# quadram-institute-bioscience/uvaia

Hardware: AMD Instinct MI355X
Metric: ref-seqs scored/sec (higher is better)
Workload: dtype u32 bit-planes / int32 counts

## Files before the change

include/uvaia_gpu.h:

```cpp
#ifndef UVAIA_GPU_H
#define UVAIA_GPU_H

#include <stddef.h>
#include <stdint.h>

#ifdef __cplusplus
extern "C" {
#endif

#define UVAIA_GPU_NSCORE 6

enum {
  UVAIA_GPU_OK         =  0,
  UVAIA_GPU_EINVAL     = -1,
  UVAIA_GPU_ENODEV     = -2,
  UVAIA_GPU_ENOMEM     = -3,
  UVAIA_GPU_EHIP       = -4,
  UVAIA_GPU_EALPHABET  = -5,
  UVAIA_GPU_ESTATE     = -6
};

typedef struct uvaia_gpu_ctx uvaia_gpu_ctx;

typedef struct {
  int n_query;
  int nchar;
  const char *const *seq;
  const char *consensus;
  const size_t *idx_c, *idx_m, *idx;
  int n_idx_c, n_idx_m, n_idx;
  size_t trim;
  int acgt;
} uvaia_gpu_query;

int uvaia_gpu_open (uvaia_gpu_ctx **ctx, const uvaia_gpu_query *query, int heap_size, int device, size_t max_pool);

enum { UVAIA_GPU_SCAN_AUTO = 0,
       UVAIA_GPU_SCAN_PACKED = 1,
       UVAIA_GPU_SCAN_COMPRESSED = 2,
       UVAIA_GPU_SCAN_WIDE = 3 };
typedef struct {
  size_t subslice_refs;
  int rare_max;
  int scan;
  int serial;
  int scan_tiles_per_wave;
  int scan_waves_per_block;
  int rederive_streams;
  int ball_gather;
  int query_tables;
  int replay_extras;
  int replay_cus;
  int scan_streams;
  int pipeline;
  int head_scan;
  int derive_waves;
} uvaia_gpu_tuning;
int uvaia_gpu_export_query_table (uvaia_gpu_ctx *ctx, int which, void *out, size_t cap, size_t *n_bytes);
int uvaia_gpu_open_tuned (uvaia_gpu_ctx **ctx, const uvaia_gpu_query *query, int heap_size, int device, size_t max_pool, const uvaia_gpu_tuning *tuning );
void uvaia_gpu_close (uvaia_gpu_ctx *ctx);
const char *uvaia_gpu_last_error (const uvaia_gpu_ctx *ctx);

int uvaia_gpu_push (uvaia_gpu_ctx *ctx, const char *const *seq, const int *non_n, int n_ref, int64_t ordinal0,
                    uint8_t *entered);

int uvaia_gpu_drain (uvaia_gpu_ctx *ctx, int *n_items, int *max_incompatible, int *scores, int64_t *ordinals);
int uvaia_gpu_heap_slots (const uvaia_gpu_ctx *ctx);
int uvaia_gpu_n_query (const uvaia_gpu_ctx *ctx);
int uvaia_gpu_reset (uvaia_gpu_ctx *ctx);

int uvaia_gpu_db_reserve (uvaia_gpu_ctx *ctx, size_t n_ref_capacity);
int uvaia_gpu_db_append (uvaia_gpu_ctx *ctx, const char *const *seq, const int *non_n, int n_ref);
int uvaia_gpu_db_append_block (uvaia_gpu_ctx *ctx, const char *rows, size_t pitch, const int *non_n, int n_ref);
size_t uvaia_gpu_db_size (const uvaia_gpu_ctx *ctx);
int uvaia_gpu_search_resident (uvaia_gpu_ctx *ctx, size_t pool, int64_t ordinal0, uint8_t *entered);
int uvaia_gpu_sync (uvaia_gpu_ctx *ctx);

size_t uvaia_gpu_state_bytes (const uvaia_gpu_ctx *ctx);
int uvaia_gpu_state_export (uvaia_gpu_ctx *ctx, void *dst);
int uvaia_gpu_state_import (uvaia_gpu_ctx *ctx, const void *src);
int uvaia_gpu_slice_scan (uvaia_gpu_ctx *ctx, size_t first, size_t n, int buf);
int uvaia_gpu_slice_replay (uvaia_gpu_ctx *ctx, int buf, int64_t ordinal0, int stripe_start);
int uvaia_gpu_slice_buffers (void);
size_t uvaia_gpu_state_range_bytes (const uvaia_gpu_ctx *ctx, int q0, int q1);
int uvaia_gpu_state_export_range (uvaia_gpu_ctx *ctx, void *dst, int q0, int q1);
int uvaia_gpu_state_import_range (uvaia_gpu_ctx *ctx, const void *src, int q0, int q1);
int uvaia_gpu_slice_replay_range (uvaia_gpu_ctx *ctx, int buf, int64_t ordinal0, int q0, int q1, int take_snapshot);
int uvaia_gpu_entered_flags (uvaia_gpu_ctx *ctx, uint8_t *out, int clear);

int uvaia_gpu_ball (uvaia_gpu_ctx *ctx, const char *const *seq, int n_ref, int radius, int *mindist);
int uvaia_gpu_ball_resident (uvaia_gpu_ctx *ctx, size_t first, size_t n, int radius, int *mindist);
int uvaia_gpu_ball_packed (uvaia_gpu_ctx *ctx, const void *planes, int n_ref, int radius, int *mindist);
int uvaia_gpu_unpack_rows (uvaia_gpu_ctx *ctx, const int *index, int n, char *rows, size_t pitch);
unsigned long long uvaia_gpu_ball_asked (uvaia_gpu_ctx *ctx, int reset);
void uvaia_gpu_ball_kernel_ms (uvaia_gpu_ctx *ctx, double out[3], int reset);

int uvaia_gpu_agree_on_polymorphic (uvaia_gpu_ctx *ctx, const char *const *seq, int n_seq, uint8_t *out);

int uvaia_gpu_query_columns (const char *const *seq, int n_query, int nchar, size_t trim, int acgt, int device, char *consensus, unsigned char *some_missing);

int uvaia_gpu_last_batch_scores (uvaia_gpu_ctx *ctx, int *out, int n_ref);
int uvaia_gpu_scan_stats (uvaia_gpu_ctx *ctx, double *ms, long long *launches, double *algorithmic_bytes, int reset);
int uvaia_gpu_replay_stats (uvaia_gpu_ctx *ctx, unsigned long long out[3], int reset);
int uvaia_gpu_replay_tiles_opened (uvaia_gpu_ctx *ctx, unsigned long long *out, int reset);
int uvaia_gpu_replay_timing (uvaia_gpu_ctx *ctx, unsigned long long out[12], int reset);
int uvaia_gpu_set_query_tile (uvaia_gpu_ctx *ctx, int qt);
int uvaia_gpu_set_active_queries (uvaia_gpu_ctx *ctx, int q0, int q1);
int uvaia_gpu_max_tolerance (uvaia_gpu_ctx *ctx, int *out);
int uvaia_gpu_search_resident_pool (uvaia_gpu_ctx *ctx, size_t first, size_t n, int64_t ordinal0, int snapshot);

int uvaia_gpu_db_set_shard (uvaia_gpu_ctx *ctx, int rank, int world, size_t piece_refs);
int uvaia_gpu_shard_rows (const uvaia_gpu_ctx *ctx);
size_t uvaia_gpu_shard_aux_bytes (const uvaia_gpu_ctx *ctx, size_t n_tiles);
int uvaia_gpu_shard_scan (uvaia_gpu_ctx *ctx, size_t first, size_t n, void *cnt, void *tmin, void *aux);
int uvaia_gpu_db_skip (uvaia_gpu_ctx *ctx, size_t n_ref);
int uvaia_gpu_shard_set_peer (uvaia_gpu_ctx *ctx, int rank, const void *planes, const void *side_rows);
const void *uvaia_gpu_shard_planes (const uvaia_gpu_ctx *ctx);
const void *uvaia_gpu_shard_side_rows (const uvaia_gpu_ctx *ctx);
int uvaia_gpu_shard_ipc_handle_bytes (void);
int uvaia_gpu_shard_ipc_handles (uvaia_gpu_ctx *ctx, void *out );
int uvaia_gpu_shard_ipc_open (uvaia_gpu_ctx *ctx, int rank, const void *handles);
int uvaia_gpu_shard_ipc_close (uvaia_gpu_ctx *ctx);
int uvaia_gpu_scan_wait (uvaia_gpu_ctx *ctx);
int uvaia_gpu_replay_wait (uvaia_gpu_ctx *ctx);
int uvaia_gpu_set_snapshot (uvaia_gpu_ctx *ctx, int snapshot);
enum { UVAIA_GPU_SCANS = 0, UVAIA_GPU_REPLAYS = 1 };
int uvaia_gpu_mark (uvaia_gpu_ctx *ctx, int what, int slot);
int uvaia_gpu_stream_wait_mark (uvaia_gpu_ctx *ctx, void *stream, int slot);
int uvaia_gpu_wait_stream (uvaia_gpu_ctx *ctx, int what, void *stream);
int uvaia_gpu_shard_replay (uvaia_gpu_ctx *ctx, const void *cnt, const void *tmin, const void *aux, int owner, size_t first, size_t n, int64_t ordinal0, int q0, int q1);

typedef struct uvaia_gpu_group uvaia_gpu_group;
int  uvaia_gpu_group_open (uvaia_gpu_group **group, const uvaia_gpu_query *query, int heap_size, const int *devices, int n_devices, size_t max_pool, size_t piece_refs);
void uvaia_gpu_group_close (uvaia_gpu_group *group);
const char *uvaia_gpu_group_last_error (const uvaia_gpu_group *group);
int  uvaia_gpu_group_size (const uvaia_gpu_group *group);
uvaia_gpu_ctx *uvaia_gpu_group_member (uvaia_gpu_group *group, int i);
int  uvaia_gpu_group_query_shard (const uvaia_gpu_group *group, int i, int *q0, int *q1);
int  uvaia_gpu_group_db_reserve (uvaia_gpu_group *group, size_t n_ref_capacity);
int  uvaia_gpu_group_db_append (uvaia_gpu_group *group, const char *const *seq, const int *non_n, int n_ref);
int  uvaia_gpu_group_db_append_packed (uvaia_gpu_group *group, const void *planes, const int *non_n, const int *side_rows, int n_ref);
int  uvaia_gpu_group_db_clear (uvaia_gpu_group *group);
int  uvaia_gpu_group_db_rederive (uvaia_gpu_group *group);
size_t uvaia_gpu_group_db_size (const uvaia_gpu_group *group);
int  uvaia_gpu_group_reset (uvaia_gpu_group *group);
int  uvaia_gpu_group_search_resident (uvaia_gpu_group *group, size_t pool, int64_t ordinal0, uint8_t *entered);
int  uvaia_gpu_group_push (uvaia_gpu_group *group, const char *const *seq, const int *non_n, int n_ref, int64_t ordinal0, uint8_t *entered);
int  uvaia_gpu_group_drain (uvaia_gpu_group *group, int *n_items, int *max_incompatible, int *scores, int64_t *ordinals);
int  uvaia_gpu_group_sync (uvaia_gpu_group *group);

size_t uvaia_gpu_db_tile_bytes (const uvaia_gpu_ctx *ctx);
int    uvaia_gpu_db_clear (uvaia_gpu_ctx *ctx);
int    uvaia_gpu_db_rederive (uvaia_gpu_ctx *ctx);
int    uvaia_gpu_db_derived_export (uvaia_gpu_ctx *ctx, size_t n_tiles, void *e, uint32_t *grp, void *poly, int *tot);
int    uvaia_gpu_db_side_row_ints (void);
int    uvaia_gpu_db_export (uvaia_gpu_ctx *ctx, size_t first_tile, size_t n_tiles, void *planes, int *non_n, int *side_rows);
int    uvaia_gpu_db_append_packed (uvaia_gpu_ctx *ctx, const void *planes, const int *non_n, const int *side_rows, int n_ref);

int uvaia_gpu_db_stage_reserve (uvaia_gpu_ctx *ctx, size_t n_tiles);
int uvaia_gpu_db_stage_packed (uvaia_gpu_ctx *ctx, int slot, const void *planes, const int *non_n, const int *side_rows, int n_tiles);
int uvaia_gpu_db_load_staged (uvaia_gpu_ctx *ctx, int slot, const int *sel, int n_ref);
int uvaia_gpu_db_stage_packed_at (uvaia_gpu_ctx *ctx, int slot, size_t tile_offset, const void *planes, const int *non_n, const int *side_rows, int n_tiles);
int uvaia_gpu_db_append_staged (uvaia_gpu_ctx *ctx, int slot, const int *sel, int n_ref);
int uvaia_gpu_db_stage_compact_at (uvaia_gpu_ctx *ctx, int slot, size_t tile_offset, const void *base, const uint64_t *head_idx, const uint32_t *heads,
                                   const uint64_t *lit_idx, const void *lits, const int *non_n, int n_tiles);
void uvaia_gpu_compact_ms (uvaia_gpu_ctx *ctx, double out[2], int reset);
int uvaia_gpu_db_unpack_rows (uvaia_gpu_ctx *ctx, const int *index, int n, char *rows, size_t pitch);
void uvaia_gpu_window_ms (uvaia_gpu_ctx *ctx, double out[3], int reset);
size_t uvaia_gpu_free_bytes (uvaia_gpu_ctx *ctx);

int uvaia_gpu_rows_census (uvaia_gpu_ctx *ctx, const void *d_rows, size_t pitch, int n, int *non_n, int *n_exc);
int uvaia_gpu_db_append_device (uvaia_gpu_ctx *ctx, const void *d_rows, size_t pitch, const int *row_index, int n_sel, const int *non_n);
int uvaia_gpu_rows_exceptions (uvaia_gpu_ctx *ctx, const void *d_rows, size_t pitch, const int *row_index, int n_sel, const uint64_t *offsets, void *exc_out);
int uvaia_gpu_db_drop_tiles (uvaia_gpu_ctx *ctx, size_t n_tiles);
void uvaia_gpu_rows_kernel_ms (uvaia_gpu_ctx *ctx, double out[3], int reset);
int uvaia_gpu_rows_set_run_cut (uvaia_gpu_ctx *ctx, unsigned cut);

size_t uvaia_gpu_scan_bytes_per_ref (const uvaia_gpu_ctx *ctx);
int uvaia_gpu_scan_variant (const uvaia_gpu_ctx *ctx);
size_t uvaia_gpu_derived_bytes_per_ref (const uvaia_gpu_ctx *ctx);
size_t uvaia_gpu_packed_bytes_per_ref (const uvaia_gpu_ctx *ctx);

#ifdef __cplusplus
}
#endif
#endif
```

uvaia_amd/capi.py:

```python
import ctypes as C
import os
import subprocess

import numpy as np

_HERE = os.path.dirname(os.path.abspath(__file__))
ROOT = os.path.dirname(_HERE)
_LIB = os.path.join(_HERE, "lib", "libuvaia_gpu.so")
NSCORE = 6

SYMBOLS = [
    "uvaia_gpu_open", "uvaia_gpu_open_tuned", "uvaia_gpu_close", "uvaia_gpu_last_error", "uvaia_gpu_push", "uvaia_gpu_drain",
    "uvaia_gpu_heap_slots", "uvaia_gpu_n_query", "uvaia_gpu_reset", "uvaia_gpu_db_reserve", "uvaia_gpu_db_append",
    "uvaia_gpu_db_append_block", "uvaia_gpu_db_size", "uvaia_gpu_search_resident", "uvaia_gpu_sync", "uvaia_gpu_ball", "uvaia_gpu_ball_resident", "uvaia_gpu_ball_packed", "uvaia_gpu_unpack_rows", "uvaia_gpu_ball_asked", "uvaia_gpu_ball_kernel_ms", "uvaia_gpu_export_query_table", "uvaia_gpu_agree_on_polymorphic", "uvaia_gpu_query_columns",
    "uvaia_gpu_last_batch_scores", "uvaia_gpu_scan_stats", "uvaia_gpu_replay_stats", "uvaia_gpu_replay_tiles_opened", "uvaia_gpu_replay_timing",
    "uvaia_gpu_state_bytes", "uvaia_gpu_state_export", "uvaia_gpu_state_import", "uvaia_gpu_slice_scan", "uvaia_gpu_slice_replay",
    "uvaia_gpu_entered_flags", "uvaia_gpu_state_range_bytes", "uvaia_gpu_state_export_range", "uvaia_gpu_state_import_range",
    "uvaia_gpu_slice_replay_range", "uvaia_gpu_slice_buffers", "uvaia_gpu_scan_bytes_per_ref", "uvaia_gpu_derived_bytes_per_ref", "uvaia_gpu_scan_variant", "uvaia_gpu_set_query_tile", "uvaia_gpu_packed_bytes_per_ref",
    "uvaia_gpu_db_tile_bytes", "uvaia_gpu_db_side_row_ints", "uvaia_gpu_db_export", "uvaia_gpu_db_append_packed", "uvaia_gpu_db_clear", "uvaia_gpu_db_rederive", "uvaia_gpu_db_derived_export",
    "uvaia_gpu_set_active_queries", "uvaia_gpu_max_tolerance", "uvaia_gpu_search_resident_pool",
    "uvaia_gpu_db_set_shard", "uvaia_gpu_shard_rows", "uvaia_gpu_shard_scan", "uvaia_gpu_scan_wait", "uvaia_gpu_replay_wait", "uvaia_gpu_set_snapshot", "uvaia_gpu_shard_replay",
    "uvaia_gpu_mark", "uvaia_gpu_stream_wait_mark", "uvaia_gpu_wait_stream",
    "uvaia_gpu_shard_aux_bytes", "uvaia_gpu_db_skip", "uvaia_gpu_shard_set_peer", "uvaia_gpu_shard_planes", "uvaia_gpu_shard_side_rows",
    "uvaia_gpu_shard_ipc_handle_bytes", "uvaia_gpu_shard_ipc_handles", "uvaia_gpu_shard_ipc_open", "uvaia_gpu_shard_ipc_close",
    "uvaia_gpu_group_open", "uvaia_gpu_group_close", "uvaia_gpu_group_last_error", "uvaia_gpu_group_size", "uvaia_gpu_group_member", "uvaia_gpu_group_query_shard",
    "uvaia_gpu_group_db_reserve", "uvaia_gpu_group_db_append", "uvaia_gpu_group_db_append_packed", "uvaia_gpu_group_db_clear", "uvaia_gpu_group_db_rederive",
    "uvaia_gpu_group_db_size", "uvaia_gpu_group_reset", "uvaia_gpu_group_search_resident", "uvaia_gpu_group_push", "uvaia_gpu_group_drain", "uvaia_gpu_group_sync",
    "uvaia_gpu_rows_census", "uvaia_gpu_db_append_device", "uvaia_gpu_rows_exceptions", "uvaia_gpu_db_drop_tiles", "uvaia_gpu_rows_kernel_ms", "uvaia_gpu_rows_set_run_cut",
    "uvaia_gpu_db_stage_reserve", "uvaia_gpu_db_stage_packed", "uvaia_gpu_db_load_staged", "uvaia_gpu_db_unpack_rows", "uvaia_gpu_window_ms", "uvaia_gpu_free_bytes",
    "uvaia_gpu_db_stage_packed_at", "uvaia_gpu_db_append_staged", "uvaia_gpu_db_stage_compact_at", "uvaia_gpu_compact_ms",
]


class GpuError(RuntimeError):
    def __init__(self, code, msg):
        super().__init__("uvaia_gpu error %d: %s" % (code, msg))
        self.code = code


class Tuning(C.Structure):
    _fields_ = [("subslice_refs", C.c_size_t), ("rare_max", C.c_int), ("scan", C.c_int), ("serial", C.c_int),
                ("scan_tiles_per_wave", C.c_int), ("scan_waves_per_block", C.c_int), ("rederive_streams", C.c_int), ("ball_gather", C.c_int), ("query_tables", C.c_int), ("replay_extras", C.c_int), ("replay_cus", C.c_int), ("scan_streams", C.c_int), ("pipeline", C.c_int), ("head_scan", C.c_int), ("derive_waves", C.c_int)]

    SCAN = {"auto": 0, "packed": 1, "compressed": 2, "wide": 3}

    @classmethod
    def make(cls, tuning):
        if tuning is None or isinstance(tuning, cls):
            return tuning
        t = cls()
        for k, v in tuning.items():
            setattr(t, k, cls.SCAN[v] if k == "scan" and isinstance(v, str) else int(v))
        return t


class _Query(C.Structure):
    _fields_ = [
        ("n_query", C.c_int), ("nchar", C.c_int),
        ("seq", C.POINTER(C.c_char_p)), ("consensus", C.c_char_p),
        ("idx_c", C.POINTER(C.c_size_t)), ("idx_m", C.POINTER(C.c_size_t)), ("idx", C.POINTER(C.c_size_t)),
        ("n_idx_c", C.c_int), ("n_idx_m", C.c_int), ("n_idx", C.c_int),
        ("trim", C.c_size_t), ("acgt", C.c_int),
    ]


def library_path():
    return _LIB


def build_library(force=False):
    csrc = os.path.join(_HERE, "csrc")
    srcs = [os.path.join(csrc, f) for f in os.listdir(csrc) if f.endswith((".hip", ".inc"))] + [os.path.join(ROOT, "include", "uvaia_gpu.h")]
    if not force and os.path.exists(_LIB) and os.path.getmtime(_LIB) >= max(os.path.getmtime(f) for f in srcs):
        return _LIB
    subprocess.check_call(["make", "-C", os.path.join(_HERE, "csrc"), "-s"])
    return _LIB


_lib = None


def load_library():
    global _lib
    if _lib is not None:
        return _lib
    if not os.path.exists(_LIB):
        raise GpuError(-2, "HIP library %s is missing: run __graft_entry__.build() (no CPU fallback exists)" % _LIB)
    L = C.CDLL(_LIB)
    vp = C.c_void_p
    pp = C.POINTER(C.c_char_p)
    pi = C.POINTER(C.c_int)
    sig = {
        "uvaia_gpu_open": (C.c_int, [C.POINTER(vp), C.POINTER(_Query), C.c_int, C.c_int, C.c_size_t]),
        "uvaia_gpu_open_tuned": (C.c_int, [C.POINTER(vp), C.POINTER(_Query), C.c_int, C.c_int, C.c_size_t, C.POINTER(Tuning)]),
        "uvaia_gpu_close": (None, [vp]),
        "uvaia_gpu_last_error": (C.c_char_p, [vp]),
        "uvaia_gpu_push": (C.c_int, [vp, pp, pi, C.c_int, C.c_int64, C.POINTER(C.c_uint8)]),
        "uvaia_gpu_drain": (C.c_int, [vp, pi, pi, pi, C.POINTER(C.c_int64)]),
        "uvaia_gpu_heap_slots": (C.c_int, [vp]),
        "uvaia_gpu_n_query": (C.c_int, [vp]),
        "uvaia_gpu_reset": (C.c_int, [vp]),
        "uvaia_gpu_db_reserve": (C.c_int, [vp, C.c_size_t]),
        "uvaia_gpu_db_append": (C.c_int, [vp, pp, pi, C.c_int]),
        "uvaia_gpu_db_append_block": (C.c_int, [vp, C.c_void_p, C.c_size_t, pi, C.c_int]),
        "uvaia_gpu_db_size": (C.c_size_t, [vp]),
        "uvaia_gpu_search_resident": (C.c_int, [vp, C.c_size_t, C.c_int64, C.POINTER(C.c_uint8)]),
        "uvaia_gpu_sync": (C.c_int, [vp]),
        "uvaia_gpu_ball": (C.c_int, [vp, pp, C.c_int, C.c_int, pi]),
        "uvaia_gpu_ball_resident": (C.c_int, [vp, C.c_size_t, C.c_size_t, C.c_int, pi]),
        "uvaia_gpu_ball_packed": (C.c_int, [vp, C.c_void_p, C.c_int, C.c_int, pi]),
        "uvaia_gpu_unpack_rows": (C.c_int, [vp, pi, C.c_int, C.c_void_p, C.c_size_t]),
        "uvaia_gpu_ball_asked": (C.c_ulonglong, [vp, C.c_int]),
        "uvaia_gpu_ball_kernel_ms": (None, [vp, C.POINTER(C.c_double), C.c_int]),
        "uvaia_gpu_export_query_table": (C.c_int, [vp, C.c_int, vp, C.c_size_t, C.POINTER(C.c_size_t)]),
        "uvaia_gpu_agree_on_polymorphic": (C.c_int, [vp, pp, C.c_int, C.POINTER(C.c_uint8)]),
        "uvaia_gpu_query_columns": (C.c_int, [pp, C.c_int, C.c_int, C.c_size_t, C.c_int, C.c_int, C.c_char_p, C.POINTER(C.c_uint8)]),
        "uvaia_gpu_last_batch_scores": (C.c_int, [vp, pi, C.c_int]),
        "uvaia_gpu_scan_stats": (C.c_int, [vp, C.POINTER(C.c_double), C.POINTER(C.c_longlong), C.POINTER(C.c_double), C.c_int]),
        "uvaia_gpu_replay_stats": (C.c_int, [vp, C.POINTER(C.c_ulonglong), C.c_int]),
        "uvaia_gpu_replay_tiles_opened": (C.c_int, [vp, C.POINTER(C.c_ulonglong), C.c_int]),
        "uvaia_gpu_replay_timing": (C.c_int, [vp, C.POINTER(C.c_ulonglong), C.c_int]),
        "uvaia_gpu_state_bytes": (C.c_size_t, [vp]),
        "uvaia_gpu_state_export": (C.c_int, [vp, C.c_void_p]),
        "uvaia_gpu_state_import": (C.c_int, [vp, C.c_void_p]),
        "uvaia_gpu_slice_scan": (C.c_int, [vp, C.c_size_t, C.c_size_t, C.c_int]),
        "uvaia_gpu_slice_replay": (C.c_int, [vp, C.c_int, C.c_int64, C.c_int]),
        "uvaia_gpu_entered_flags": (C.c_int, [vp, C.POINTER(C.c_uint8), C.c_int]),
        "uvaia_gpu_state_range_bytes": (C.c_size_t, [vp, C.c_int, C.c_int]),
        "uvaia_gpu_state_export_range": (C.c_int, [vp, C.c_void_p, C.c_int, C.c_int]),
        "uvaia_gpu_state_import_range": (C.c_int, [vp, C.c_void_p, C.c_int, C.c_int]),
        "uvaia_gpu_slice_replay_range": (C.c_int, [vp, C.c_int, C.c_int64, C.c_int, C.c_int, C.c_int]),
        "uvaia_gpu_slice_buffers": (C.c_int, []),
        "uvaia_gpu_scan_bytes_per_ref": (C.c_size_t, [vp]),
        "uvaia_gpu_derived_bytes_per_ref": (C.c_size_t, [vp]),
        "uvaia_gpu_scan_variant": (C.c_int, [vp]),
        "uvaia_gpu_set_query_tile": (C.c_int, [vp, C.c_int]),
        "uvaia_gpu_packed_bytes_per_ref": (C.c_size_t, [vp]),
        "uvaia_gpu_set_active_queries": (C.c_int, [vp, C.c_int, C.c_int]),
        "uvaia_gpu_max_tolerance": (C.c_int, [vp, pi]),
        "uvaia_gpu_search_resident_pool": (C.c_int, [vp, C.c_size_t, C.c_size_t, C.c_int64, C.c_int]),
        "uvaia_gpu_db_tile_bytes": (C.c_size_t, [vp]),
        "uvaia_gpu_db_clear": (C.c_int, [vp]),
        "uvaia_gpu_db_rederive": (C.c_int, [vp]),
        "uvaia_gpu_db_derived_export": (C.c_int, [vp, C.c_size_t, C.c_void_p, C.c_void_p, C.c_void_p, C.c_void_p]),
        "uvaia_gpu_db_side_row_ints": (C.c_int, []),
        "uvaia_gpu_db_export": (C.c_int, [vp, C.c_size_t, C.c_size_t, C.c_void_p, pi, pi]),
        "uvaia_gpu_db_append_packed": (C.c_int, [vp, C.c_void_p, pi, pi, C.c_int]),
        "uvaia_gpu_db_set_shard": (C.c_int, [vp, C.c_int, C.c_int, C.c_size_t]),
        "uvaia_gpu_shard_rows": (C.c_int, [vp]),
        "uvaia_gpu_shard_scan": (C.c_int, [vp, C.c_size_t, C.c_size_t, C.c_void_p, C.c_void_p, C.c_void_p]),
        "uvaia_gpu_shard_aux_bytes": (C.c_size_t, [vp, C.c_size_t]), "uvaia_gpu_db_skip": (C.c_int, [vp, C.c_size_t]),
        "uvaia_gpu_shard_set_peer": (C.c_int, [vp, C.c_int, C.c_void_p, C.c_void_p]),
        "uvaia_gpu_shard_planes": (C.c_void_p, [vp]), "uvaia_gpu_shard_side_rows": (C.c_void_p, [vp]),
        "uvaia_gpu_shard_ipc_handle_bytes": (C.c_int, []), "uvaia_gpu_shard_ipc_handles": (C.c_int, [vp, C.c_void_p]),
        "uvaia_gpu_shard_ipc_open": (C.c_int, [vp, C.c_int, C.c_void_p]), "uvaia_gpu_shard_ipc_close": (C.c_int, [vp]),
        "uvaia_gpu_scan_wait": (C.c_int, [vp]),
        "uvaia_gpu_replay_wait": (C.c_int, [vp]),
        "uvaia_gpu_set_snapshot": (C.c_int, [vp, C.c_int]),
        "uvaia_gpu_shard_replay": (C.c_int, [vp, C.c_void_p, C.c_void_p, C.c_void_p, C.c_int, C.c_size_t, C.c_size_t, C.c_int64, C.c_int, C.c_int]),
        "uvaia_gpu_mark": (C.c_int, [vp, C.c_int, C.c_int]), "uvaia_gpu_stream_wait_mark": (C.c_int, [vp, C.c_void_p, C.c_int]),
        "uvaia_gpu_wait_stream": (C.c_int, [vp, C.c_int, C.c_void_p]),
        "uvaia_gpu_group_open": (C.c_int, [C.POINTER(vp), C.POINTER(_Query), C.c_int, pi, C.c_int, C.c_size_t, C.c_size_t]),
        "uvaia_gpu_group_close": (None, [vp]),
        "uvaia_gpu_group_last_error": (C.c_char_p, [vp]),
        "uvaia_gpu_group_size": (C.c_int, [vp]),
        "uvaia_gpu_group_member": (vp, [vp, C.c_int]),
        "uvaia_gpu_group_query_shard": (C.c_int, [vp, C.c_int, pi, pi]),
        "uvaia_gpu_group_db_reserve": (C.c_int, [vp, C.c_size_t]),
        "uvaia_gpu_group_db_append": (C.c_int, [vp, pp, pi, C.c_int]),
        "uvaia_gpu_group_db_append_packed": (C.c_int, [vp, C.c_void_p, pi, pi, C.c_int]),
        "uvaia_gpu_group_db_clear": (C.c_int, [vp]),
        "uvaia_gpu_group_db_rederive": (C.c_int, [vp]),
        "uvaia_gpu_group_db_size": (C.c_size_t, [vp]),
        "uvaia_gpu_group_reset": (C.c_int, [vp]),
        "uvaia_gpu_group_search_resident": (C.c_int, [vp, C.c_size_t, C.c_int64, C.POINTER(C.c_uint8)]),
        "uvaia_gpu_group_push": (C.c_int, [vp, pp, pi, C.c_int, C.c_int64, C.POINTER(C.c_uint8)]),
        "uvaia_gpu_group_drain": (C.c_int, [vp, pi, pi, pi, C.POINTER(C.c_int64)]),
        "uvaia_gpu_group_sync": (C.c_int, [vp]),
        "uvaia_gpu_rows_census": (C.c_int, [vp, C.c_void_p, C.c_size_t, C.c_int, pi, pi]),
        "uvaia_gpu_db_append_device": (C.c_int, [vp, C.c_void_p, C.c_size_t, pi, C.c_int, pi]),
        "uvaia_gpu_rows_exceptions": (C.c_int, [vp, C.c_void_p, C.c_size_t, pi, C.c_int, C.POINTER(C.c_uint64), C.c_void_p]),
        "uvaia_gpu_db_drop_tiles": (C.c_int, [vp, C.c_size_t]),
        "uvaia_gpu_rows_kernel_ms": (None, [vp, C.POINTER(C.c_double), C.c_int]),
        "uvaia_gpu_rows_set_run_cut": (C.c_int, [vp, C.c_uint]),
        "uvaia_gpu_db_stage_reserve": (C.c_int, [vp, C.c_size_t]),
        "uvaia_gpu_db_stage_packed": (C.c_int, [vp, C.c_int, C.c_void_p, pi, pi, C.c_int]),
        "uvaia_gpu_db_load_staged": (C.c_int, [vp, C.c_int, pi, C.c_int]),
        "uvaia_gpu_db_stage_packed_at": (C.c_int, [vp, C.c_int, C.c_size_t, C.c_void_p, pi, pi, C.c_int]),
        "uvaia_gpu_db_append_staged": (C.c_int, [vp, C.c_int, pi, C.c_int]),
        "uvaia_gpu_db_stage_compact_at": (C.c_int, [vp, C.c_int, C.c_size_t, C.c_void_p, C.c_void_p, C.c_void_p, C.c_void_p, C.c_void_p, pi, C.c_int]),
        "uvaia_gpu_compact_ms": (None, [vp, C.POINTER(C.c_double), C.c_int]),
        "uvaia_gpu_db_unpack_rows": (C.c_int, [vp, pi, C.c_int, C.c_void_p, C.c_size_t]),
        "uvaia_gpu_window_ms": (None, [vp, C.POINTER(C.c_double), C.c_int]),
        "uvaia_gpu_free_bytes": (C.c_size_t, [vp]),
    }
    for name, (res, args) in sig.items():
        fn = getattr(L, name)
        fn.restype, fn.argtypes = res, args
    _lib = L
    return L


def _cstrs(strs):
    arr = (C.c_char_p * len(strs))()
    for i, s in enumerate(strs):
        arr[i] = s
    return arr


def _int_ptr(a):
    if a is None:
        return None, None
    arr = np.ascontiguousarray(a, dtype=np.int32)
    return arr, arr.ctypes.data_as(C.POINTER(C.c_int))


class Engine:

    def __init__(self, seqs, consensus, idx_c, idx_m, idx, trim=0, acgt=False, nbest=100, max_pool=4096, device=-1, tuning=None):
        self.L = load_library()
        self.nq, self.nchar = len(seqs), len(consensus)
        self._keep = [_cstrs(seqs), consensus,
                      (C.c_size_t * len(idx_c))(*[int(x) for x in idx_c]),
                      (C.c_size_t * len(idx_m))(*[int(x) for x in idx_m]),
                      (C.c_size_t * len(idx))(*[int(x) for x in idx])]
        q = _Query(self.nq, self.nchar, self._keep[0], consensus, self._keep[2], self._keep[3], self._keep[4],
                   len(idx_c), len(idx_m), len(idx), int(trim), int(bool(acgt)))
        self.ctx = C.c_void_p()
        tn = Tuning.make(tuning)
        rc = self.L.uvaia_gpu_open_tuned(C.byref(self.ctx), C.byref(q), int(nbest), int(device), int(max_pool), C.byref(tn) if tn is not None else None)
        if rc != 0:
            msg = self.L.uvaia_gpu_last_error(None)
            self.ctx = None
            raise GpuError(rc, msg.decode() if msg else "?")
        self.slots = self.L.uvaia_gpu_heap_slots(self.ctx)
        self.ordinal = 0

    @classmethod
    def from_query(cls, q, **kw):
        return cls(q.seqs, q.consensus, q.idx_c, q.idx_m, q.idx, trim=q.trim, acgt=q.acgt, **kw)

    def _chk(self, rc):
        if rc != 0:
            msg = self.L.uvaia_gpu_last_error(self.ctx)
            raise GpuError(rc, msg.decode() if msg else "?")

    def close(self):
        if getattr(self, "ctx", None):
            self.L.uvaia_gpu_close(self.ctx)
            self.ctx = None

    def __del__(self):
        try:
            self.close()
        except Exception:
            pass

    def __enter__(self):
        return self

    def __exit__(self, *a):
        self.close()

    def push(self, refs, non_n=None, ordinal0=None):
        n = len(refs)
        if ordinal0 is None:
            ordinal0 = self.ordinal
        self.ordinal = ordinal0 + n
        entered = np.zeros(n, dtype=np.uint8)
        if n == 0:
            return entered
        _k, nn = _int_ptr(non_n)
        self._chk(self.L.uvaia_gpu_push(self.ctx, _cstrs(refs), nn, n, ordinal0, entered.ctypes.data_as(C.POINTER(C.c_uint8))))
        return entered

    def last_batch_scores(self, n):
        out = np.zeros((n, self.nq, NSCORE), dtype=np.int32)
        self._chk(self.L.uvaia_gpu_last_batch_scores(self.ctx, out.ctypes.data_as(C.POINTER(C.c_int)), n))
        return out

    def drain(self):
        n = np.zeros(self.nq, dtype=np.int32)
        T = np.zeros(self.nq, dtype=np.int32)
        sc = np.zeros((self.nq, self.slots + 1, NSCORE), dtype=np.int32)
        od = np.zeros((self.nq, self.slots + 1), dtype=np.int64)
        pi = C.POINTER(C.c_int)
        self._chk(self.L.uvaia_gpu_drain(self.ctx, n.ctypes.data_as(pi), T.ctypes.data_as(pi), sc.ctypes.data_as(pi),
                                         od.ctypes.data_as(C.POINTER(C.c_int64))))
        return n, T, sc, od

    def reset(self):
        self.ordinal = 0
        self._chk(self.L.uvaia_gpu_reset(self.ctx))

    def db_reserve(self, n):
        self._chk(self.L.uvaia_gpu_db_reserve(self.ctx, int(n)))

    def db_append(self, refs, non_n=None):
        _k, nn = _int_ptr(non_n)
        self._chk(self.L.uvaia_gpu_db_append(self.ctx, _cstrs(refs), nn, len(refs)))

    def db_append_block(self, block, non_n=None):
        block = np.ascontiguousarray(block, dtype=np.uint8)
        _k, nn = _int_ptr(non_n)
        self._chk(self.L.uvaia_gpu_db_append_block(self.ctx, block.ctypes.data, block.shape[1], nn, block.shape[0]))

    def db_size(self):
        return self.L.uvaia_gpu_db_size(self.ctx)

    @staticmethod
    def _device_block(rows, pitch=None, n=None):
        if hasattr(rows, "data_ptr"):
            import torch
            if rows.dtype != torch.uint8 or rows.dim() != 2 or not rows.is_cuda or (rows.shape[0] > 0 and rows.shape[1] > 1 and rows.stride(1) != 1):
                raise GpuError(-1, "rows must be a 2-d torch.uint8 tensor in device memory with contiguous rows")
            torch.cuda.current_stream(rows.device).synchronize()
            return rows.data_ptr(), (rows.stride(0) if rows.shape[0] > 1 else rows.shape[1]), rows.shape[0], rows
        if pitch is None:
            raise GpuError(-1, "a raw device pointer needs its pitch")
        return int(rows), int(pitch), n, None

    def rows_census(self, rows, pitch=None, n=None):
        ptr, pitch, n, _keep = self._device_block(rows, pitch, n)
        non_n, n_exc = np.zeros(n, dtype=np.int32), np.zeros(n, dtype=np.int32)
        self._chk(self.L.uvaia_gpu_rows_census(self.ctx, ptr, pitch, n, non_n.ctypes.data_as(C.POINTER(C.c_int)), n_exc.ctypes.data_as(C.POINTER(C.c_int))))
        return non_n, n_exc

    def db_append_device(self, rows, row_index=None, non_n=None, pitch=None, n=None):
        ptr, pitch, n, _keep = self._device_block(rows, pitch, n)
        _k1, ri = _int_ptr(row_index)
        _k2, nn = _int_ptr(non_n)
        self._chk(self.L.uvaia_gpu_db_append_device(self.ctx, ptr, pitch, ri, n if row_index is None else len(row_index), nn))

    def rows_exceptions(self, rows, n_exc, row_index=None, pitch=None, n=None):
        ptr, pitch, n, _keep = self._device_block(rows, pitch, n)
        n_sel = n if row_index is None else len(row_index)
        off = np.zeros(n_sel + 1, dtype=np.uint64)
        off[1:] = np.cumsum(np.asarray(n_exc, dtype=np.uint64))
        out = np.zeros((int(off[-1]), 2), dtype=np.uint32)
        _k1, ri = _int_ptr(row_index)
        self._chk(self.L.uvaia_gpu_rows_exceptions(self.ctx, ptr, pitch, ri, n_sel, off.ctypes.data_as(C.POINTER(C.c_uint64)), out.ctypes.data))
        return off, out

    def db_drop_tiles(self, n_tiles):
        self._chk(self.L.uvaia_gpu_db_drop_tiles(self.ctx, int(n_tiles)))

    def rows_kernel_ms(self, reset=False):
        out = (C.c_double * 3)()
        self.L.uvaia_gpu_rows_kernel_ms(self.ctx, out, int(reset))
        return {"census": out[0], "gather": out[1], "exceptions": out[2]}

    def rows_set_run_cut(self, cut):
        self._chk(self.L.uvaia_gpu_rows_set_run_cut(self.ctx, int(cut)))

    def set_active_queries(self, q0, q1):
        self._chk(self.L.uvaia_gpu_set_active_queries(self.ctx, int(q0), int(q1)))

    def max_tolerance(self):
        v = C.c_int(0)
        self._chk(self.L.uvaia_gpu_max_tolerance(self.ctx, C.byref(v)))
        return v.value

    def search_resident_pool(self, first, n, ordinal0, snapshot=-1):
        self._chk(self.L.uvaia_gpu_search_resident_pool(self.ctx, int(first), int(n), int(ordinal0), int(snapshot)))

    def db_clear(self):
        self._chk(self.L.uvaia_gpu_db_clear(self.ctx))

    def db_set_shard(self, rank, world, piece_refs):
        self._chk(self.L.uvaia_gpu_db_set_shard(self.ctx, int(rank), int(world), int(piece_refs)))

    def shard_rows(self):
        return self.L.uvaia_gpu_shard_rows(self.ctx)

    def shard_scan(self, first, n, cnt_ptr, tmin_ptr, aux_ptr):
        self._chk(self.L.uvaia_gpu_shard_scan(self.ctx, int(first), int(n), C.c_void_p(cnt_ptr), C.c_void_p(tmin_ptr), C.c_void_p(aux_ptr)))

    def shard_aux_bytes(self, n_tiles):
        return int(self.L.uvaia_gpu_shard_aux_bytes(self.ctx, int(n_tiles)))

    def db_skip(self, n_ref):
        self._chk(self.L.uvaia_gpu_db_skip(self.ctx, int(n_ref)))

    def shard_ipc_handles(self):
        buf = C.create_string_buffer(self.L.uvaia_gpu_shard_ipc_handle_bytes())
        self._chk(self.L.uvaia_gpu_shard_ipc_handles(self.ctx, buf))
        return buf.raw

    def shard_ipc_close(self):
        self._chk(self.L.uvaia_gpu_shard_ipc_close(self.ctx))

    def shard_ipc_open(self, rank, handles):
        self._chk(self.L.uvaia_gpu_shard_ipc_open(self.ctx, int(rank), C.c_char_p(bytes(handles))))

    def scan_wait(self):
        self._chk(self.L.uvaia_gpu_scan_wait(self.ctx))

    def replay_wait(self):
        self._chk(self.L.uvaia_gpu_replay_wait(self.ctx))

    def set_snapshot(self, v):
        self._chk(self.L.uvaia_gpu_set_snapshot(self.ctx, int(v)))

    SCANS, REPLAYS = 0, 1

    def mark(self, what, slot):
        self._chk(self.L.uvaia_gpu_mark(self.ctx, int(what), int(slot)))

    def stream_wait_mark(self, stream, slot):
        self._chk(self.L.uvaia_gpu_stream_wait_mark(self.ctx, C.c_void_p(stream), int(slot)))

    def wait_stream(self, what, stream):
        self._chk(self.L.uvaia_gpu_wait_stream(self.ctx, int(what), C.c_void_p(stream)))

    def shard_replay(self, cnt_ptr, tmin_ptr, aux_ptr, owner, first, n, ordinal0, q0, q1):
        self._chk(self.L.uvaia_gpu_shard_replay(self.ctx, C.c_void_p(cnt_ptr), C.c_void_p(tmin_ptr), C.c_void_p(aux_ptr), int(owner), int(first), int(n), int(ordinal0), int(q0), int(q1)))

    def db_rederive(self):
        self._chk(self.L.uvaia_gpu_db_rederive(self.ctx))

    def db_export(self, first_tile=0, n_tiles=None):
        if n_tiles is None:
            n_tiles = (self.db_size() + 63) // 64 - first_tile
        tb, ri = self.L.uvaia_gpu_db_tile_bytes(self.ctx), self.L.uvaia_gpu_db_side_row_ints()
        planes = np.zeros((n_tiles, tb), dtype=np.uint8)
        non_n = np.zeros(n_tiles * 64, dtype=np.int32)
        side = np.zeros((n_tiles * 64, ri), dtype=np.int32)
        self._chk(self.L.uvaia_gpu_db_export(self.ctx, first_tile, n_tiles, planes.ctypes.data, non_n.ctypes.data_as(C.POINTER(C.c_int)),
                                             side.ctypes.data_as(C.POINTER(C.c_int))))
        return planes, non_n, side

    def db_append_packed(self, planes, non_n, side_rows, n_ref):
        planes = np.ascontiguousarray(planes, dtype=np.uint8)
        non_n = np.ascontiguousarray(non_n, dtype=np.int32)
        side_rows = np.ascontiguousarray(side_rows, dtype=np.int32)
        self._chk(self.L.uvaia_gpu_db_append_packed(self.ctx, planes.ctypes.data, non_n.ctypes.data_as(C.POINTER(C.c_int)),
                                                    side_rows.ctypes.data_as(C.POINTER(C.c_int)), int(n_ref)))

    def search_resident(self, pool, ordinal0=0, want_entered=True):
        ent, p = None, None
        if want_entered:
            ent = np.zeros(self.db_size(), dtype=np.uint8)
            p = ent.ctypes.data_as(C.POINTER(C.c_uint8))
        self._chk(self.L.uvaia_gpu_search_resident(self.ctx, int(pool), int(ordinal0), p))
        return ent

    def sync(self):
        self._chk(self.L.uvaia_gpu_sync(self.ctx))

    def scan_stats(self, reset=False):
        ms, n, b = C.c_double(), C.c_longlong(), C.c_double()
        self._chk(self.L.uvaia_gpu_scan_stats(self.ctx, C.byref(ms), C.byref(n), C.byref(b), int(reset)))
        return ms.value, n.value, b.value

    def state_bytes(self):
        return self.L.uvaia_gpu_state_bytes(self.ctx)

    def state_export(self, ptr):
        self._chk(self.L.uvaia_gpu_state_export(self.ctx, C.c_void_p(ptr)))

    def state_import(self, ptr):
        self._chk(self.L.uvaia_gpu_state_import(self.ctx, C.c_void_p(ptr)))

    def slice_scan(self, first, n, buf):
        self._chk(self.L.uvaia_gpu_slice_scan(self.ctx, int(first), int(n), int(buf)))

    def slice_replay(self, buf, ordinal0, stripe_start):
        self._chk(self.L.uvaia_gpu_slice_replay(self.ctx, int(buf), int(ordinal0), int(bool(stripe_start))))

    def state_range_bytes(self, q0, q1):
        return self.L.uvaia_gpu_state_range_bytes(self.ctx, int(q0), int(q1))

    def state_export_range(self, ptr, q0, q1):
        self._chk(self.L.uvaia_gpu_state_export_range(self.ctx, C.c_void_p(ptr), int(q0), int(q1)))

    def state_import_range(self, ptr, q0, q1):
        self._chk(self.L.uvaia_gpu_state_import_range(self.ctx, C.c_void_p(ptr), int(q0), int(q1)))

    def slice_replay_range(self, buf, ordinal0, q0, q1, take_snapshot):
        self._chk(self.L.uvaia_gpu_slice_replay_range(self.ctx, int(buf), int(ordinal0), int(q0), int(q1), int(bool(take_snapshot))))

    def entered_flags(self, clear=False):
        ent = np.zeros(self.db_size(), dtype=np.uint8)
        self._chk(self.L.uvaia_gpu_entered_flags(self.ctx, ent.ctypes.data_as(C.POINTER(C.c_uint8)), int(clear)))
        return ent

    def replay_stats(self, reset=False):
        out = (C.c_ulonglong * 3)()
        self._chk(self.L.uvaia_gpu_replay_stats(self.ctx, out, int(reset)))
        return int(out[0]), int(out[1]), int(out[2])

    def replay_timing(self, reset=False):
        out = (C.c_ulonglong * 12)()
        self._chk(self.L.uvaia_gpu_replay_timing(self.ctx, out, int(reset)))
        return [int(x) for x in out]

    def replay_tiles_opened(self, reset=False):
        out = C.c_ulonglong(0)
        self._chk(self.L.uvaia_gpu_replay_tiles_opened(self.ctx, C.byref(out), int(reset)))
        return int(out.value)

    def set_query_tile(self, qt):
        self._chk(self.L.uvaia_gpu_set_query_tile(self.ctx, int(qt)))

    def scan_bytes_per_ref(self):
        return self.L.uvaia_gpu_scan_bytes_per_ref(self.ctx)

    def derived_bytes_per_ref(self):
        return self.L.uvaia_gpu_derived_bytes_per_ref(self.ctx)

    def scan_variant(self):
        return self.L.uvaia_gpu_scan_variant(self.ctx)

    def packed_bytes_per_ref(self):
        return self.L.uvaia_gpu_packed_bytes_per_ref(self.ctx)

    def agree_on_polymorphic(self, seqs):
        out = np.zeros((len(seqs), self.nq), dtype=np.uint8)
        self._chk(self.L.uvaia_gpu_agree_on_polymorphic(self.ctx, _cstrs(seqs), len(seqs), out.ctypes.data_as(C.POINTER(C.c_uint8))))
        return out

    def ball(self, refs, radius):
        md = np.zeros(len(refs), dtype=np.int32)
        self._chk(self.L.uvaia_gpu_ball(self.ctx, _cstrs(refs), len(refs), int(radius), md.ctypes.data_as(C.POINTER(C.c_int))))
        return md

    def ball_resident(self, radius, first=0, n=None, want=True):
        n = self.db_size() - first if n is None else n
        md = np.zeros(n, dtype=np.int32) if want else None
        self._chk(self.L.uvaia_gpu_ball_resident(self.ctx, int(first), int(n), int(radius), md.ctypes.data_as(C.POINTER(C.c_int)) if want else None))
        return md

    def ball_packed(self, planes, n_ref, radius):
        planes = np.ascontiguousarray(planes, dtype=np.uint8)
        tb = self.L.uvaia_gpu_db_tile_bytes(self.ctx)
        if planes.size < (int(n_ref) + 63) // 64 * tb:
            raise ValueError("%d references need %d bytes of tiles, got %d" % (n_ref, (int(n_ref) + 63) // 64 * tb, planes.size))
        md = np.zeros(int(n_ref), dtype=np.int32)
        self._chk(self.L.uvaia_gpu_ball_packed(self.ctx, planes.ctypes.data, int(n_ref), int(radius), md.ctypes.data_as(C.POINTER(C.c_int))))
        return md

    def unpack_rows(self, index):
        idx = np.ascontiguousarray(index, dtype=np.int32)
        pitch = (self.nchar + 15) // 16 * 16
        rows = np.zeros((max(len(idx), 1), pitch), dtype=np.uint8)
        self._chk(self.L.uvaia_gpu_unpack_rows(self.ctx, idx.ctypes.data_as(C.POINTER(C.c_int)), len(idx), rows.ctypes.data, pitch))
        return [rows[k, :self.nchar].tobytes() for k in range(len(idx))]

    def db_stage_reserve(self, n_tiles):
        self._chk(self.L.uvaia_gpu_db_stage_reserve(self.ctx, int(n_tiles)))

    def db_stage_packed(self, slot, planes, non_n, side_rows, n_tiles):
        planes = np.ascontiguousarray(planes, dtype=np.uint8)
        non_n = np.ascontiguousarray(non_n, dtype=np.int32)
        side_rows = np.ascontiguousarray(side_rows, dtype=np.int32)
        tb = self.L.uvaia_gpu_db_tile_bytes(self.ctx)
        if planes.size < int(n_tiles) * tb or non_n.size < int(n_tiles) * 64 or side_rows.size < int(n_tiles) * 64 * self.L.uvaia_gpu_db_side_row_ints():
            raise ValueError("arrays shorter than %d tiles" % n_tiles)
        if not hasattr(self, "_staged"):
            self._staged = {}
        self._staged[int(slot)] = (planes, non_n, side_rows)
        self._chk(self.L.uvaia_gpu_db_stage_packed(self.ctx, int(slot), planes.ctypes.data, non_n.ctypes.data_as(C.POINTER(C.c_int)),
                                                   side_rows.ctypes.data_as(C.POINTER(C.c_int)), int(n_tiles)))

    def db_load_staged(self, slot, sel, n_ref):
        _k, sp = _int_ptr(sel)
        self._chk(self.L.uvaia_gpu_db_load_staged(self.ctx, int(slot), sp, int(n_ref)))

    def db_stage_packed_at(self, slot, tile_offset, planes, non_n, side_rows, n_tiles):
        planes = np.ascontiguousarray(planes, dtype=np.uint8)
        non_n = np.ascontiguousarray(non_n, dtype=np.int32)
        side_rows = np.ascontiguousarray(side_rows, dtype=np.int32)
        tb = self.L.uvaia_gpu_db_tile_bytes(self.ctx)
        if planes.size < int(n_tiles) * tb or non_n.size < int(n_tiles) * 64 or side_rows.size < int(n_tiles) * 64 * self.L.uvaia_gpu_db_side_row_ints():
            raise ValueError("arrays shorter than %d tiles" % n_tiles)
        if not hasattr(self, "_staged_at"):
            self._staged_at = {}
        if int(tile_offset) == 0:
            self._staged_at[int(slot)] = []
        self._staged_at.setdefault(int(slot), []).append((planes, non_n, side_rows))
        self._chk(self.L.uvaia_gpu_db_stage_packed_at(self.ctx, int(slot), int(tile_offset), planes.ctypes.data, non_n.ctypes.data_as(C.POINTER(C.c_int)),
                                                      side_rows.ctypes.data_as(C.POINTER(C.c_int)), int(n_tiles)))

    def db_stage_compact_at(self, slot, tile_offset, base, head_idx, heads, lit_idx, lits, non_n, n_tiles):
        base = np.ascontiguousarray(base, dtype=np.uint32)
        head_idx = np.ascontiguousarray(head_idx, dtype=np.uint64)
        lit_idx = np.ascontiguousarray(lit_idx, dtype=np.uint64)
        heads = np.ascontiguousarray(heads, dtype=np.uint32)
        lits = np.ascontiguousarray(lits, dtype=np.uint32)
        non_n = np.ascontiguousarray(non_n, dtype=np.int32)
        lanes = int(n_tiles) * 64
        if base.size * 4 * 64 != self.L.uvaia_gpu_db_tile_bytes(self.ctx) or head_idx.size < lanes + 1 or lit_idx.size < lanes + 1 or non_n.size < lanes:
            raise ValueError("arrays shorter than %d tiles" % n_tiles)
        if lanes and (heads.size < int(head_idx[lanes]) or lits.size < int(lit_idx[lanes]) * 4):
            raise ValueError("records shorter than the index says")
        if not hasattr(self, "_staged_at"):
            self._staged_at = {}
        if int(tile_offset) == 0:
            self._staged_at[int(slot)] = []
        self._staged_at.setdefault(int(slot), []).append((base, head_idx, heads, lit_idx, lits, non_n))
        self._chk(self.L.uvaia_gpu_db_stage_compact_at(self.ctx, int(slot), int(tile_offset), base.ctypes.data, head_idx.ctypes.data, heads.ctypes.data,
                                                       lit_idx.ctypes.data, lits.ctypes.data, non_n.ctypes.data_as(C.POINTER(C.c_int)), int(n_tiles)))

    def compact_ms(self, reset=False):
        out = (C.c_double * 2)()
        self.L.uvaia_gpu_compact_ms(self.ctx, out, int(reset))
        return tuple(out)

    def db_append_staged(self, slot, sel, n_ref):
        _k, sp = _int_ptr(sel)
        self._chk(self.L.uvaia_gpu_db_append_staged(self.ctx, int(slot), sp, int(n_ref)))

    def db_unpack_rows(self, index, pitch=None):
        idx = np.ascontiguousarray(index, dtype=np.int32)
        pitch = (self.nchar + 15) // 16 * 16 if pitch is None else int(pitch)
        rows = np.zeros((max(len(idx), 1), pitch), dtype=np.uint8)
        self._chk(self.L.uvaia_gpu_db_unpack_rows(self.ctx, idx.ctypes.data_as(C.POINTER(C.c_int)), len(idx), rows.ctypes.data, pitch))
        return [rows[k, :self.nchar].tobytes() for k in range(len(idx))]

    def window_ms(self, reset=False):
        out = (C.c_double * 3)()
        self.L.uvaia_gpu_window_ms(self.ctx, out, int(reset))
        return tuple(out)

    def free_bytes(self):
        return int(self.L.uvaia_gpu_free_bytes(self.ctx))

    def ball_asked(self, reset=False):
        return int(self.L.uvaia_gpu_ball_asked(self.ctx, int(reset)))

    def query_table(self, which):
        n = C.c_size_t(0)
        self._chk(self.L.uvaia_gpu_export_query_table(self.ctx, int(which), None, 0, C.byref(n)))
        out = np.zeros(n.value, dtype=np.uint8)
        if n.value:
            self._chk(self.L.uvaia_gpu_export_query_table(self.ctx, int(which), out.ctypes.data_as(C.c_void_p), n.value, C.byref(n)))
        return out

    def db_derived(self, n_tiles):
        W4 = ((self.nchar + 31) // 32 + 3) // 4
        counts = self.query_table(10).view(np.int32)
        NG = int(counts[2]) + int(counts[3])
        e = np.zeros((n_tiles, W4, 64, 4), dtype=np.uint32)
        grp = np.zeros((n_tiles, W4, 64), dtype=np.uint32)
        poly = np.zeros((n_tiles, NG, 3, 64, 4), dtype=np.uint32)
        tot = np.zeros(n_tiles * 64, dtype=np.int32)
        self._chk(self.L.uvaia_gpu_db_derived_export(self.ctx, int(n_tiles), e.ctypes.data, grp.ctypes.data, poly.ctypes.data, tot.ctypes.data))
        return e, grp, poly, tot

    def ball_kernel_ms(self, reset=False):
        out = (C.c_double * 3)()
        self.L.uvaia_gpu_ball_kernel_ms(self.ctx, out, int(reset))
        return tuple(out)


def finalise_heaps(n, scores, ordinals):
    out = []
    for q in range(len(n)):
        k = int(n[q])
        order = ([k] + list(range(1, k))) if k else []
        rows = [(tuple(int(x) for x in scores[q, s]), int(ordinals[q, s])) for s in order]
        rows.sort(key=lambda r: tuple(-v for v in r[0]))
        out.append(rows)
    return out


class Group:

    def __init__(self, q, devices, nbest=100, max_pool=4096, piece_refs=0):
        self.L = load_library()
        self.nq, self.nchar = len(q.seqs), len(q.consensus)
        self._keep = [_cstrs(q.seqs), q.consensus,
                      (C.c_size_t * len(q.idx_c))(*[int(x) for x in q.idx_c]),
                      (C.c_size_t * len(q.idx_m))(*[int(x) for x in q.idx_m]),
                      (C.c_size_t * len(q.idx))(*[int(x) for x in q.idx])]
        qq = _Query(self.nq, self.nchar, self._keep[0], q.consensus, self._keep[2], self._keep[3], self._keep[4],
                    len(q.idx_c), len(q.idx_m), len(q.idx), int(q.trim), int(bool(q.acgt)))
        self.g = C.c_void_p()
        dev = (C.c_int * len(devices))(*[int(d) for d in devices])
        rc = self.L.uvaia_gpu_group_open(C.byref(self.g), C.byref(qq), int(nbest), dev, len(devices), int(max_pool), int(piece_refs))
        if rc != 0:
            msg = self.L.uvaia_gpu_group_last_error(None)
            self.g = None
            raise GpuError(rc, msg.decode() if msg else "?")
        self.slots = self.L.uvaia_gpu_heap_slots(self.L.uvaia_gpu_group_member(self.g, 0))

    def _chk(self, rc):
        if rc != 0:
            msg = self.L.uvaia_gpu_group_last_error(self.g)
            raise GpuError(rc, msg.decode() if msg else "?")

    def close(self):
        if getattr(self, "g", None):
            self.L.uvaia_gpu_group_close(self.g)
            self.g = None

    def __enter__(self):
        return self

    def __exit__(self, *a):
        self.close()

    def __del__(self):
        try:
            self.close()
        except Exception:
            pass

    def query_shard(self, i):
        a, b = C.c_int(), C.c_int()
        self._chk(self.L.uvaia_gpu_group_query_shard(self.g, i, C.byref(a), C.byref(b)))
        return a.value, b.value

    def member_bytes_per_ref(self):
        self.L.uvaia_gpu_packed_bytes_per_ref.restype = C.c_size_t
        self.L.uvaia_gpu_derived_bytes_per_ref.restype = C.c_size_t
        m0 = C.c_void_p(self.L.uvaia_gpu_group_member(self.g, 0))
        return int(self.L.uvaia_gpu_packed_bytes_per_ref(m0)), int(self.L.uvaia_gpu_derived_bytes_per_ref(m0))

    def db_reserve(self, n):
        self._chk(self.L.uvaia_gpu_group_db_reserve(self.g, int(n)))

    def db_append(self, refs, non_n=None):
        _k, nn = _int_ptr(non_n)
        self._chk(self.L.uvaia_gpu_group_db_append(self.g, _cstrs(refs), nn, len(refs)))

    def db_rederive(self):
        self._chk(self.L.uvaia_gpu_group_db_rederive(self.g))

    def reset(self):
        self._chk(self.L.uvaia_gpu_group_reset(self.g))

    def sync(self):
        self._chk(self.L.uvaia_gpu_group_sync(self.g))

    def search_resident(self, pool, ordinal0=0, want_entered=True):
        ent, p = None, None
        if want_entered:
            ent = np.zeros(self.L.uvaia_gpu_group_db_size(self.g), dtype=np.uint8)
            p = ent.ctypes.data_as(C.POINTER(C.c_uint8))
        self._chk(self.L.uvaia_gpu_group_search_resident(self.g, int(pool), int(ordinal0), p))
        return ent

    def push(self, refs, non_n=None, ordinal0=0):
        entered = np.zeros(len(refs), dtype=np.uint8)
        _k, nn = _int_ptr(non_n)
        self._chk(self.L.uvaia_gpu_group_push(self.g, _cstrs(refs), nn, len(refs), int(ordinal0), entered.ctypes.data_as(C.POINTER(C.c_uint8))))
        return entered

    def drain(self):
        n = np.zeros(self.nq, dtype=np.int32)
        T = np.zeros(self.nq, dtype=np.int32)
        sc = np.zeros((self.nq, self.slots + 1, NSCORE), dtype=np.int32)
        od = np.zeros((self.nq, self.slots + 1), dtype=np.int64)
        pi = C.POINTER(C.c_int)
        self._chk(self.L.uvaia_gpu_group_drain(self.g, n.ctypes.data_as(pi), T.ctypes.data_as(pi), sc.ctypes.data_as(pi), od.ctypes.data_as(C.POINTER(C.c_int64))))
        return n, T, sc, od


def query_columns(seqs, trim=0, acgt=False, device=-1):
    L = load_library()
    n, nchar = len(seqs), len(seqs[0])
    arr = (C.c_char_p * n)(*seqs)
    cons = C.create_string_buffer(nchar)
    miss = np.zeros(nchar, dtype=np.uint8)
    rc = L.uvaia_gpu_query_columns(arr, n, nchar, int(trim), int(bool(acgt)), int(device), cons, miss.ctypes.data_as(C.POINTER(C.c_uint8)))
    if rc:
        raise GpuError(rc, (L.uvaia_gpu_last_error(None) or b"").decode())
    return cons.raw[:nchar], miss
```

uvaia_amd/csrc/host_ctx.inc:

```

struct uvaia_gpu_ctx;

namespace {

thread_local std::string g_open_error;

int fail(uvaia_gpu_ctx *c, int code, const char *fmt, ...);

#define HIP_TRY(call, on_fail) do { hipError_t e_ = (call); if (e_ != hipSuccess) { const int code_ = e_ == hipErrorOutOfMemory ? UVAIA_GPU_ENOMEM : UVAIA_GPU_EHIP; (void)code_; on_fail; } } while (0)
#define HIPCHK(c, call) HIP_TRY(call, return fail((c), code_, "%s failed: %s (%s:%d)", #call, hipGetErrorString(e_), __FILE__, __LINE__))

template <class T> struct DevBuf {
  T *p = nullptr; size_t cap = 0;
  DevBuf() = default;
  DevBuf(const DevBuf &) = delete; DevBuf &operator=(const DevBuf &) = delete;
  DevBuf(DevBuf &&o) noexcept : p(o.p), cap(o.cap) { o.p = nullptr; o.cap = 0; }
  DevBuf &operator=(DevBuf &&o) noexcept { if (this != &o) { release(); p = o.p; cap = o.cap; o.p = nullptr; o.cap = 0; } return *this; }
  ~DevBuf() { release(); }
  void release() { if (p) hipFree(p); p = nullptr; cap = 0; }
  int reserve(uvaia_gpu_ctx *c, size_t n)
  {
    if (n <= cap) return 0;
    release();
    HIPCHK(c, hipMalloc(&p, n * sizeof(T)));
    cap = n;
    return 0;
  }
  operator T *() const { return p; }
};

struct PinnedBuf {
  uint8_t *p = nullptr;
  PinnedBuf() = default;
  PinnedBuf(const PinnedBuf &) = delete; PinnedBuf &operator=(const PinnedBuf &) = delete;
  ~PinnedBuf() { if (p) hipHostFree(p); }
  int alloc(uvaia_gpu_ctx *c, size_t bytes) { HIPCHK(c, hipHostMalloc(&p, bytes, hipHostMallocDefault)); return 0; }
  operator uint8_t *() const { return p; }
};

struct Event {
  hipEvent_t e = nullptr;
  Event() = default;
  Event(const Event &) = delete; Event &operator=(const Event &) = delete;
  Event(Event &&o) noexcept : e(o.e) { o.e = nullptr; }
  Event &operator=(Event &&o) noexcept { if (this != &o) { if (e) hipEventDestroy(e); e = o.e; o.e = nullptr; } return *this; }
  ~Event() { if (e) hipEventDestroy(e); }
  int make(uvaia_gpu_ctx *c, unsigned flags = 0)
  {
    if (e) return 0;
    if (flags) HIPCHK(c, hipEventCreateWithFlags(&e, flags)); else HIPCHK(c, hipEventCreate(&e));
    return 0;
  }
  operator hipEvent_t() const { return e; }
};

struct Stream {
  hipStream_t s = nullptr;
  Stream() = default;
  Stream(const Stream &) = delete; Stream &operator=(const Stream &) = delete;
  ~Stream() { if (s) hipStreamDestroy(s); }
  operator hipStream_t() const { return s; }
};

struct ScanEvt { Event a, b; double bytes = 0; };

struct TileStore {
  DevBuf<uint4> planes;
  DevBuf<int> nonn;
  DevBuf<int> amb;
  DevBuf<int> tot;
  DevBuf<uint4> ev, poly;
  DevBuf<uint32_t> grp;
  DevBuf<int> tote;
};

struct SliceBuf {
  DevBuf<uint32_t> cnt;
  DevBuf<int2> tmin;
  DevBuf<uint32_t> ext;
  DevBuf<uint32_t> rtp;
  DevBuf<uint4> tb8;
  DevBuf<int4> rt;
  int tiles = 0, rb = 0, re = 0; long long tf = 0;
  bool scanned = false, cons_done = false;
  Event scan_done, replay_done;
  bool replay_recorded = false;
};

}

struct uvaia_gpu_ctx {
  int device = 0;
  struct Streams {
    Stream stream;
    Stream scan_streams[3];
    unsigned scan_rr = 0;
    int scan_nstreams = 1;
    int scan_nstreams_forced = 0;
    struct DeriveChunk { long long t0, t1; Event done; };
    Stream derive_streams[3];
    int derive_nstreams = 3; bool derive_forced = false;
    std::vector<DeriveChunk> derive_chunks;
    Event derive_fence[4];
    size_t derive_pending = 0;
    bool planes_busy[4] = {}; hipEvent_t planes_ev[4] = {};
    Stream rep_stream; Event rep_ev[2];
    Event order_ev[16]; unsigned order_rr = 0;
    Event mark_ev[8][3]; bool mark_set[8][3] = {};
  } st;
  SliceBuf slice[NBUF];
  bool use_ext = false;
  size_t subslice = 25088;
  bool subslice_forced = false;
  int first_slice_pct = 70;
  int nq = 0, nq_pad = 0, nchar = 0, W = 0, W4 = 0, P = 4, NQ = 6, acgt = 0, k = 2, qt = 16, n_idx_c = 0, n_idx_m = 0;
  size_t trim = 0;
  size_t max_pool = 0, pool_pad = 0;
  int scan_variant = 2;
  int derive_waves = 0;
  int act_q0 = 0, act_q1 = 0;
  bool serial = false;
  int replay_lq = -1;
  int replay_prio = 1;
  int replay_half = 32;
  int replay_cus = 0;
  int scan_R = 2;
  int scan_NW = 8;
  bool fullscan = false;
  struct QueryTables {
    DevBuf<uint32_t> d_qp;
    DevBuf<uint32_t> d_qp2;
    DevBuf<uint32_t> d_cls;
    DevBuf<uint32_t> d_qpl;
    DevBuf<uint32_t> d_stream;
    DevBuf<uint32_t> d_sdir;
    int NP = 0, NP4 = 0;
    int NR = 0, NR4 = 0, rare_max = -1;
    DevBuf<uint32_t> d_rmask;
    DevBuf<int> d_split;
    DevBuf<uint32_t> d_qrare;
    int need_e_groups = 0, need_v_groups = 0, need_g_groups = 0, need_r_groups = 0;
    DevBuf<int> d_amb_q;
    struct { const void *p; size_t n; } qtab[10] = {};
    DevBuf<uint32_t> d_cp;
    DevBuf<uint32_t> d_cpm;
    DevBuf<uint32_t> d_qpoly;
    DevBuf<uint32_t> d_pmask;
  } tab;
  struct SearchState {
    DevBuf<int> d_heap, d_n, d_T, d_snap, d_err;
    DevBuf<int4> d_cnt;
    DevBuf<int4> d_rt, d_tr;
    DevBuf<uint8_t> d_entered;
    size_t entered_clean = 0;
  } state;
  struct Ball {
    DevBuf<int> d_mindist, d_list, d_cdist, d_n;
    DevBuf<uint4> d_tiles; unsigned long long asked = 0;
    bool fused = true; DevBuf<uint4> d_ga;
    Event ev[4]; double ms[3] = {0., 0., 0.};
    DevBuf<int> d_idx_cols; int n_idx = 0, NG4 = 0;
    std::vector<int> idx_cols; DevBuf<uint32_t> d_masks; int NH4 = 0;
    DevBuf<uint32_t> d_qg;
    DevBuf<unsigned long long> d_key;
    DevBuf<uint4> d_pk; int pk_n = 0;
    DevBuf<uint8_t> d_rows;
    DevBuf<int> d_row_idx;
  } ball;
  struct Rows {
    DevBuf<int> d_sel, d_cnt; DevBuf<unsigned long long> d_off; DevBuf<uint2> d_exc;
    std::vector<int> host; std::vector<uint2> exc_host;
    uint32_t run_cut = 0xFFFFFFu;
    std::vector<Event> evs; double ms[3] = {0., 0., 0.};
  } rows;
  struct Window {
    Stream copy_stream;
    struct StageSlot { DevBuf<uint4> planes; DevBuf<int> nonn, side; int n_tiles = 0; Event copied, read; bool read_recorded = false; };
    StageSlot stage[2];
    DevBuf<int> d_sel;
    DevBuf<uint4> d_four; int n = 0;
    Event ev[5]; double ms[3] = {0., 0., 0.};
    struct Compact { DevBuf<uint4> base; DevBuf<unsigned long long> hidx, lidx; DevBuf<uint32_t> heads, lits; Event ev[3]; bool timed = false; double ms[2] = {0., 0.}; } compact;
  } win;
  struct Shard {
    int rank = 0, world = 1; long long pt = 0;
    const uint4 *peer_db[64] = {}; const int *peer_amb[64] = {};
    void *ipc_opened[64][2] = {};
  } shard;
  TileStore batch;
  DevBuf<uint8_t> d_stage;
  PinnedBuf h_stage;
  Event stage_free[2]; bool stage_busy[2] = {};
  size_t pitch = 0;
  TileStore db;
  size_t db_cap = 0, db_n = 0, db_local_tiles = 0;
  struct { const TileStore *store = nullptr; long long tile_first = 0; int n_tiles = 0, n = 0, rbegin = 0, ppad = 0; const int4 *rt = nullptr; } last;
  struct Stats {
    DevBuf<unsigned long long> d_stats;
    std::vector<ScanEvt> evts;
    std::vector<Event> ev_pool;
    double scan_ms = 0, scan_bytes = 0; long long scan_launches = 0;
    bool profile = true;
  } stats;
  std::string err;
};

namespace {

int fail(uvaia_gpu_ctx *c, int code, const char *fmt, ...)
{
  char buf[512];
  va_list ap; va_start(ap, fmt); vsnprintf(buf, sizeof buf, fmt, ap); va_end(ap);
  if (c) c->err = buf; else g_open_error = buf;
  return code;
}

inline bool owns_tile(const uvaia_gpu_ctx *c, long long t) { return c->shard.world == 1 || (t / c->shard.pt) % c->shard.world == c->shard.rank; }
inline long long dtile_of(const uvaia_gpu_ctx *c, long long t)
{ return c->shard.world == 1 ? t : (t / (c->shard.pt * c->shard.world)) * c->shard.pt + t % c->shard.pt; }
template <class F> inline int for_owned_tiles(const uvaia_gpu_ctx *c, long long gt0, long long gt1, F f)
{
  if (c->shard.world == 1) return gt1 > gt0 ? f(gt0, gt0, gt1 - gt0) : 0;
  for (long long a = gt0; a < gt1;) {
    const long long b = std::min(gt1, (a / c->shard.pt + 1) * c->shard.pt);
    if (owns_tile(c, a)) { const int rc = f(a, dtile_of(c, a), b - a); if (rc) return rc; }
    a = b;
  }
  return 0;
}
inline size_t derived_tiles(const uvaia_gpu_ctx *c, size_t tiles)
{ return c->shard.world == 1 ? tiles : (size_t)((tiles + (size_t)(c->shard.pt * c->shard.world) - 1) / (size_t)(c->shard.pt * c->shard.world)) * (size_t)c->shard.pt; }

void fill_code_table(uint8_t *t)
{
  memset(t, 0xFF, 256);
  const char *inv = "NnXx-?Oo.";
  for (const char *p = inv; *p; p++) t[(unsigned char)*p] = 0;
  static const struct { char c; uint8_t m; } iu[] = {
    {'A',1},{'C',2},{'G',4},{'T',8},{'M',3},{'R',5},{'W',9},{'S',6},{'Y',10},{'K',12},{'V',7},{'H',11},{'D',13},{'B',14}};
  for (auto &e : iu) { t[(unsigned char)e.c] = e.m; t[(unsigned char)(e.c + 32)] = e.m; }
}

}
```

uvaia_amd/csrc/host_launch.inc:

```

namespace {

template <class F>
static void parallel_for(int n, F f)
{
  const unsigned nt = std::min<unsigned>(std::max(1u, std::thread::hardware_concurrency()), 64u);
  if (n < 32 || nt < 2) { for (int i = 0; i < n; i++) f(i); return; }
  std::atomic<int> next(0);
  std::vector<std::thread> th;
  for (unsigned t = 0; t < nt; t++) th.emplace_back([&]() { for (;;) { const int a = next.fetch_add(4); if (a >= n) break; for (int i = a; i < std::min(n, a + 4); i++) f(i); } });
  for (auto &x : th) x.join();
}

__global__ void mask_query_planes_kernel(const uint32_t *__restrict__ qp, const uint32_t *__restrict__ pmask, uint32_t *__restrict__ out, size_t n_words_total, int words_per_row, int nq_planes)
{
  const size_t i = (size_t)blockIdx.x * blockDim.x + threadIdx.x;
  if (i >= n_words_total) return;
  const int w = (int)((i / (size_t)nq_planes) % (size_t)words_per_row);
  out[i] = qp[i] & pmask[w];
}

int ensure_qpoly(uvaia_gpu_ctx *c)
{
  if (c->tab.d_qpoly) return 0;
  HIPCHK(c, hipSetDevice(c->device));
  const size_t n = (size_t)c->nq_pad * c->W4 * 4 * c->NQ;
  DevBuf<uint32_t> d;
  if (int rc = d.reserve(c, n)) return rc;
  hipLaunchKernelGGL(mask_query_planes_kernel, dim3((unsigned)((n + 255) / 256)), dim3(256), 0, c->st.stream, c->tab.d_qp, c->tab.d_pmask, d, n, c->W4 * 4, c->NQ);
  hipError_t e = hipGetLastError();
  if (e == hipSuccess) e = hipStreamSynchronize(c->st.stream);
  if (e != hipSuccess) return fail(c, UVAIA_GPU_EHIP, "query planes on the polymorphic columns: %s", hipGetErrorString(e));
  c->tab.d_qpoly = std::move(d);
  return 0;
}

int ensure_qgather(uvaia_gpu_ctx *c)
{
  if (c->ball.d_qg) return 0;
  HIPCHK(c, hipSetDevice(c->device));
  const int NG = c->acgt ? 3 : 5, W = c->W4 * 4, n_idx = c->ball.n_idx;
  constexpr int BALL_HOT_COLS = 256;
  std::vector<int> cols(c->ball.idx_cols.begin(), c->ball.idx_cols.begin() + n_idx), order;
  std::vector<uint32_t> masks((size_t)2 * W, 0u);
  int n_hot = 0;
  if (n_idx >= 2 * BALL_HOT_COLS) {
    DevBuf<int> d_score;
    std::vector<int> score((size_t)n_idx);
    if (int rc = d_score.reserve(c, (size_t)n_idx)) return rc;
    if (c->acgt) hipLaunchKernelGGL((ball_column_diversity_kernel<true>), dim3((n_idx + 63) / 64), dim3(64), 0, c->st.stream, c->tab.d_qp, c->nq, c->W4, c->ball.d_idx_cols, n_idx, d_score);
    else         hipLaunchKernelGGL((ball_column_diversity_kernel<false>), dim3((n_idx + 63) / 64), dim3(64), 0, c->st.stream, c->tab.d_qp, c->nq, c->W4, c->ball.d_idx_cols, n_idx, d_score);
    hipError_t e = hipGetLastError();
    if (e == hipSuccess) e = hipMemcpyAsync(score.data(), d_score, (size_t)n_idx * sizeof(int), hipMemcpyDeviceToHost, c->st.stream);
    if (e == hipSuccess) e = hipStreamSynchronize(c->st.stream);
    if (e != hipSuccess) return fail(c, UVAIA_GPU_EHIP, "diversity of the polymorphic columns: %s", hipGetErrorString(e));
    std::vector<int> by_score((size_t)n_idx);
    for (int i = 0; i < n_idx; i++) by_score[(size_t)i] = i;
    std::stable_sort(by_score.begin(), by_score.end(), [&](int a, int b) { return score[(size_t)a] > score[(size_t)b]; });
    n_hot = BALL_HOT_COLS;
    std::vector<uint8_t> is_hot((size_t)n_idx, 0);
    for (int i = 0; i < n_hot; i++) is_hot[(size_t)by_score[(size_t)i]] = 1;
    for (int i = 0; i < n_idx; i++) if (is_hot[(size_t)i]) order.push_back(cols[(size_t)i]);
    for (int i = 0; i < n_idx; i++) if (!is_hot[(size_t)i]) order.push_back(cols[(size_t)i]);
  } else order = cols;
  c->ball.NH4 = n_hot / 128;
  c->ball.NG4 = std::max(1, c->ball.NH4 + (n_idx - n_hot + 127) / 128);
  for (int i = 0; i < n_idx; i++) { const int col = order[(size_t)i]; masks[(size_t)(col >> 7) * 8 + (i < n_hot ? 0 : 4) + ((col >> 5) & 3)] |= 1u << (col & 31); }
  order.resize(order.size() + 1, 0);
  DevBuf<uint32_t> d, dm; DevBuf<int> dc;
  const size_t n = (size_t)c->nq_pad * c->ball.NG4 * 4 * NG;
  if (int rc = d.reserve(c, n)) return rc;
  if (int rc = dm.reserve(c, masks.size())) return rc;
  if (int rc = dc.reserve(c, order.size())) return rc;
  hipError_t e = hipMemcpyAsync(dm, masks.data(), masks.size() * 4, hipMemcpyHostToDevice, c->st.stream);
  if (e == hipSuccess) e = hipMemcpyAsync(dc, order.data(), order.size() * sizeof(int), hipMemcpyHostToDevice, c->st.stream);
  if (e == hipSuccess) e = hipMemsetAsync(d, 0, n * 4, c->st.stream);
  dim3 grid((unsigned)((c->ball.NG4 * 4 + 63) / 64), (unsigned)c->nq);
  if (e == hipSuccess) {
    if (c->acgt) hipLaunchKernelGGL((ball_gather_queries_kernel<true>), grid, dim3(64), 0, c->st.stream, c->tab.d_qp, c->nq, c->W4, dc, n_idx, c->ball.NG4, d);
    else         hipLaunchKernelGGL((ball_gather_queries_kernel<false>), grid, dim3(64), 0, c->st.stream, c->tab.d_qp, c->nq, c->W4, dc, n_idx, c->ball.NG4, d);
    e = hipGetLastError();
  }
  if (e == hipSuccess) e = hipStreamSynchronize(c->st.stream);
  if (e != hipSuccess) return fail(c, UVAIA_GPU_EHIP, "query planes on the polymorphic columns: %s", hipGetErrorString(e));
  c->ball.d_qg = std::move(d); c->ball.d_masks = std::move(dm);
  return 0;
}

int store_alloc(uvaia_gpu_ctx *c, TileStore &s, size_t tiles)
{
  s = TileStore();
  DevBuf<uint4> planes;
  const size_t refs = tiles * 64, tile_u4 = (size_t)c->W4 * c->P * 64;
  if (int rc = s.nonn.reserve(c, refs)) return rc;
  HIPCHK(c, hipMemset(s.nonn, 0, refs * sizeof(int)));
  if (int rc = s.ev.reserve(c, tiles * (size_t)c->W4 * 2 * 64)) return rc;
  if (int rc = s.grp.reserve(c, tiles * (size_t)c->W4 * 64)) return rc;
  if (int rc = s.poly.reserve(c, tiles * (size_t)std::max(c->tab.NP4 + c->tab.NR4, 1) * 3 * 64)) return rc;
  if (int rc = s.tote.reserve(c, refs)) return rc;
  if (int rc = s.tot.reserve(c, refs)) return rc;
  HIPCHK(c, hipMemset(s.tot, 0, refs * sizeof(int)));
  if (int rc = s.amb.reserve(c, refs * AMB_ROW)) return rc;
  HIPCHK(c, hipMemset(s.amb, 0, refs * AMB_ROW * sizeof(int)));
  if (int rc = planes.reserve(c, tiles * tile_u4)) return rc;
  HIPCHK(c, hipMemset(planes, 0, tiles * tile_u4 * sizeof(uint4)));
  s.planes = std::move(planes);
  return 0;
}

int ensure_batch_buffers(uvaia_gpu_ctx *c)
{
  if (c->batch.planes) return 0;
  HIPCHK(c, hipSetDevice(c->device));
  return store_alloc(c, c->batch, c->pool_pad / 64);
}

int pack_query_row(const uint8_t *code_tab, const char *row, int nchar, int lo, int hi, const uint8_t *keep, const uint8_t *is_poly,
                   bool acgt, int NQ, uint32_t *dst, int *bad_byte)
{
  for (int s = lo; s < hi; s++) {
    if (keep && !keep[s]) continue;
    const uint8_t code = code_tab[(unsigned char)row[s]];
    if (code == 0xFF) { *bad_byte = (unsigned char)row[s]; return -1; }
    if (!code) continue;
    const int w = s >> 5, b = s & 31;
    uint32_t *d = dst + (size_t)w * NQ;
    const bool one = (code & (code - 1)) == 0;
    if (acgt) {
      if (!one) continue;
      const uint32_t two = code == 2 ? 1u : code == 4 ? 2u : code == 8 ? 3u : 0u;
      d[0] |= (two & 1u) << b; d[1] |= (two >> 1) << b; d[2] |= 1u << b;
      if (is_poly && is_poly[s]) d[3] |= 1u << b;
    } else {
      for (int p = 0; p < 4; p++) d[p] |= (uint32_t)((code >> p) & 1u) << b;
      d[4] |= 1u << b;
      if (one) d[5] |= 1u << b;
    }
  }
  return 0;
}

constexpr int DERIVE_SPLIT_INTS = 3 * (5 + 9 + 17);
inline int derive_split_offset(int nwv) { return nwv == 4 ? 0 : nwv == 8 ? 3 * 5 : 3 * (5 + 9); }
inline void build_derive_split(const uint32_t *cls, const uint32_t *rmask, int W4, int *split)
{
  for (int nwv : {4, 8, 16}) {
    int *s = split + derive_split_offset(nwv);
    for (int v = 0; v <= nwv; v++) s[v] = (int)((long long)W4 * v / nwv);
    int nd = 0, nr = 0, w = 0;
    for (int v = 0; v <= nwv; v++) {
      for (; w < s[v] * 4; w++) { nd += __builtin_popcount(cls[(size_t)w * 4 + 3]); nr += __builtin_popcount(rmask[(size_t)w]); }
      s[nwv + 1 + v] = nd; s[2 * (nwv + 1) + v] = nr;
    }
  }
}

inline int planes_slot(const uvaia_gpu_ctx *c, hipStream_t st) { for (int i = 0; i < 3; i++) if (st && st == c->st.scan_streams[i]) return 1 + i; return 0; }
inline void planes_touch(uvaia_gpu_ctx *c, hipStream_t st) { const int i = planes_slot(c, st); c->st.planes_busy[i] = true; c->st.planes_ev[i] = nullptr; }
inline void planes_fenced(uvaia_gpu_ctx *c, hipStream_t st, hipEvent_t ev)
{
  const int i = planes_slot(c, st);
  for (int j = 0; j < 4; j++) if (j != i && c->st.planes_ev[j] == ev) c->st.planes_ev[j] = nullptr;
  if (c->st.planes_busy[i]) c->st.planes_ev[i] = ev;
}
inline void planes_idle(uvaia_gpu_ctx *c, bool main, bool scans)
{ for (int i = 0; i < 4; i++) if (i == 0 ? main : scans) { c->st.planes_busy[i] = false; c->st.planes_ev[i] = nullptr; } }

int take_scan_events(uvaia_gpu_ctx *c, ScanEvt &ev)
{
  for (Event *e : {&ev.a, &ev.b}) {
    if (!c->stats.ev_pool.empty()) { *e = std::move(c->stats.ev_pool.back()); c->stats.ev_pool.pop_back(); }
    else if (int rc = e->make(c)) return rc;
  }
  return 0;
}

int launch_scan(uvaia_gpu_ctx *c, const TileStore &s, long long tile_first, int n_tiles, const uint32_t *qp, int n_rows, int4 *out, int ppad, double bytes)
{
  if (n_tiles <= 0) return 0;
  dim3 grid((unsigned)((n_rows + c->qt - 1) / c->qt), (unsigned)((n_tiles + 3) / 4)), block(256);
  ScanEvt ev{};
  if (c->stats.profile) {
    { int rc_ = take_scan_events(c, ev); if (rc_) return rc_; }
    HIPCHK(c, hipEventRecord(ev.a, c->st.stream));
  }
#define LAUNCH(K, QT) hipLaunchKernelGGL((K<QT>), grid, block, 0, c->st.stream, s.planes, tile_first, n_tiles, c->W4, qp, out, ppad)
  if (c->acgt) { switch (c->qt) { case 8: LAUNCH(scan_acgt_kernel, 8); break; case 32: LAUNCH(scan_acgt_kernel, 32); break; default: LAUNCH(scan_acgt_kernel, 16); } }
  else         { switch (c->qt) { case 8: LAUNCH(scan_iupac_kernel, 8); break; case 32: LAUNCH(scan_iupac_kernel, 32); break; default: LAUNCH(scan_iupac_kernel, 16); } }
#undef LAUNCH
  HIPCHK(c, hipGetLastError());
  if (c->stats.profile) { HIPCHK(c, hipEventRecord(ev.b, c->st.stream)); ev.bytes = bytes; c->stats.evts.push_back(std::move(ev)); }
  return 0;
}

int launch_pair_extras(uvaia_gpu_ctx *c, const TileStore &s, long long tile_first, int n_tiles, uint32_t *ext, int ppad, hipStream_t stream)
{
  if (n_tiles <= 0) return 0;
  hipLaunchKernelGGL(pair_extras_kernel, dim3((unsigned)n_tiles, (unsigned)((c->nq + 15) / 16)), dim3(256), 0, stream, s.planes, tile_first, n_tiles, c->W4,
                     s.amb, c->tab.d_qp, c->tab.d_amb_q, c->nq, ext, ppad);
  HIPCHK(c, hipGetLastError());
  return 0;
}

int launch_scan2(uvaia_gpu_ctx *c, const TileStore &s, long long tile_first, int n_tiles, uint32_t *out, int ppad, double bytes, hipStream_t stream,
                 int2 *tmin, int r_lo, int r_hi, int4 *rt, uint32_t *ext = nullptr , uint32_t *rtp = nullptr, uint4 *tb8 = nullptr)
{
  if (n_tiles <= 0) return 0;
  if (!stream) stream = c->st.stream;
  const bool cons = c->n_idx_c > 0;
  if (cons && !rt) return fail(c, UVAIA_GPU_ESTATE, "no buffer for the consensus pre-score");
  const uint4 *tiles = s.planes; const int *tot_tile0 = s.tot + tile_first * 64;
  const long long ptile_first = tile_first;
  auto consensus_rt = [&]() {
    if (!cons) return;
    if (c->acgt) hipLaunchKernelGGL((consensus_rt_kernel<true>), dim3((n_tiles + 3) / 4), dim3(256), 0, stream, tiles, ptile_first, n_tiles, c->W4, c->tab.d_cp, rt);
    else         hipLaunchKernelGGL((consensus_rt_kernel<false>), dim3((n_tiles + 3) / 4), dim3(256), 0, stream, tiles, ptile_first, n_tiles, c->W4, c->tab.d_cp, rt);
  };
  const int qt2 = c->qt != 8 ? 16 : c->nq <= 1 ? 1 : c->nq <= 2 ? 2 : c->nq <= 4 ? 4 : 8;
  const int n_qtiles = (c->nq + qt2 - 1) / qt2;
  dim3 grid(scan_grid_size(n_qtiles, n_tiles)), block(256);
  ScanEvt ev_{};
  if (c->stats.profile) {
    { int rc_ = take_scan_events(c, ev_); if (rc_) return rc_; }
    HIPCHK(c, hipEventRecord(ev_.a, stream));
  }
  const uint32_t *qp = c->acgt ? c->tab.d_qp : c->tab.d_qp2;
  if (c->scan_variant == 2) {
    planes_touch(c, stream);
    const int *tote = s.tote + tile_first * 64;
    constexpr int QS = 64;
    if (c->act_q0 % QS) return fail(c, UVAIA_GPU_ESTATE, "the scan works on super-tiles of %d queries: active queries start at a multiple of that", QS);
    const int st_first = c->act_q0 / QS, n_st = (c->act_q1 + QS - 1) / QS - st_first;
    const int R = c->scan_R;
    dim3 grid3(scan_grid_size(n_st, (n_tiles + R - 1) / R));
#define SCAN3_LAUNCH(NWW, A, RR) hipLaunchKernelGGL((scan3_kernel<NWW, A, RR>), grid3, dim3(64 * NWW), 0, stream, s.ev, s.poly, tile_first, n_tiles, c->W4, c->tab.NP4, c->tab.NP4 + c->tab.NR4, c->tab.d_qpl, c->tab.d_stream, c->tab.d_sdir, s.grp, tote, tot_tile0, out, ppad, n_st, tmin, r_lo, r_hi, st_first)
#define SCAN3_NW(A, RR) { if (c->scan_NW == 8) SCAN3_LAUNCH(8, A, RR); else SCAN3_LAUNCH(4, A, RR); }
    if (R == 4)      { if (c->acgt) SCAN3_LAUNCH(8, true, 4); else SCAN3_LAUNCH(8, false, 4); }
    else if (R == 2) { if (c->acgt) SCAN3_NW(true, 2) else SCAN3_NW(false, 2) }
    else             { if (c->acgt) SCAN3_NW(true, 1) else SCAN3_NW(false, 1) }
#undef SCAN3_NW
#undef SCAN3_LAUNCH
    HIPCHK(c, hipGetLastError());
    if (c->stats.profile) { HIPCHK(c, hipEventRecord(ev_.b, stream)); ev_.bytes = bytes; c->stats.evts.push_back(std::move(ev_)); }
    consensus_rt();
    HIPCHK(c, hipGetLastError());
    if (tb8 && !c->acgt) {
      hipLaunchKernelGGL(tile_bounds_kernel, dim3((unsigned)n_tiles), dim3(256), 0, stream, out, ppad, n_tiles, c->nq, r_lo, r_hi, tb8, cons ? rt : (const int4 *)nullptr, rtp);
      HIPCHK(c, hipGetLastError());
      if (ext) { int rc_ = launch_pair_extras(c, s, ptile_first, n_tiles, ext, ppad, stream); if (rc_) return rc_; }
    }
    return 0;
  }
  const int *amb0 = s.amb;
#define LAUNCH(K, QT, CN) hipLaunchKernelGGL((K<QT, CN>), grid, block, 0, stream, tiles, tile_first, n_tiles, c->W4, qp, out, ppad, n_qtiles, tot_tile0, tmin, r_lo, r_hi, c->tab.d_cp, rt)
#define LAUNCHX(K, QT, CN) hipLaunchKernelGGL((K<QT, CN>), grid, block, 0, stream, tiles, tile_first, n_tiles, c->W4, qp, out, ppad, n_qtiles, tot_tile0, tmin, r_lo, r_hi, c->tab.d_cp, rt, ext, rtp, tb8, amb0, c->tab.d_qp, c->tab.d_amb_q, c->nq)
#define LAUNCH_QT(L, K, CN) switch (qt2) { case 1: L(K, 1, CN); break; case 2: L(K, 2, CN); break; case 4: L(K, 4, CN); break; case 8: L(K, 8, CN); break; default: L(K, 16, CN); }
  if (c->acgt) { if (cons) { LAUNCH_QT(LAUNCH, scan2_acgt_kernel, true) } else { LAUNCH_QT(LAUNCH, scan2_acgt_kernel, false) } }
  else         { if (cons) { LAUNCH_QT(LAUNCHX, scan2_iupac_kernel, true) } else { LAUNCH_QT(LAUNCHX, scan2_iupac_kernel, false) } }
#undef LAUNCH_QT
#undef LAUNCHX
#undef LAUNCH
  HIPCHK(c, hipGetLastError());
  if (c->stats.profile) { HIPCHK(c, hipEventRecord(ev_.b, stream)); ev_.bytes = bytes; c->stats.evts.push_back(std::move(ev_)); }
  return 0;
}

size_t replay3_lds_bytes(const uvaia_gpu_ctx *c)
{ return (size_t)(c->k + 1) * HEAP_ENTRY * sizeof(int) + 128 + (size_t)16 * 1024 + (size_t)2 * c->replay_half * (c->n_idx_c > 0 ? 4 : 3) * 256; }
int ensure_cnt4(uvaia_gpu_ctx *c, size_t elems) { return c->state.d_cnt.reserve(c, elems); }

int collect_events(uvaia_gpu_ctx *c)
{
  for (auto &e : c->stats.evts) {
    HIPCHK(c, hipEventSynchronize(e.b));
    float ms = 0; HIPCHK(c, hipEventElapsedTime(&ms, e.a, e.b));
    c->stats.scan_ms += ms; c->stats.scan_bytes += e.bytes; c->stats.scan_launches++;
    c->stats.ev_pool.push_back(std::move(e.a)); c->stats.ev_pool.push_back(std::move(e.b));
  }
  c->stats.evts.clear();
  return 0;
}

struct ReplayLaunch {
  hipStream_t stream; int q0, q1;
  const uint32_t *cnt, *ext; int ppad; const int4 *rt; const uint32_t *rtp; const int2 *tmin; const uint4 *tb8;
  const uint4 *planes; long long tile_first; const int *nonn, *amb; uint8_t *entered;
  int rb, re; long long ord_base;
  const uint32_t *qpl; const uint4 *poly; int nr4; const uint32_t *qrare;
  int prefetch;
};
int launch_replay(uvaia_gpu_ctx *c, const ReplayLaunch &L)
{
  const dim3 grid(L.q1 - L.q0), block(64);
  const size_t lds = (size_t)(c->k + 1) * HEAP_ENTRY * sizeof(int);
  c->state.entered_clean = 0;
  if (L.poly) planes_touch(c, L.stream);
  if (c->fullscan) {
#define REPLAY(A) hipLaunchKernelGGL((replay_kernel<A>), grid, block, lds, L.stream, c->state.d_cnt, L.ppad, c->state.d_rt, c->state.d_tr, L.nonn, L.rb, L.re, L.ord_base, c->state.d_heap, c->state.d_n, c->state.d_T, c->state.d_snap, L.entered, c->k)
    if (c->acgt) REPLAY(true); else REPLAY(false);
#undef REPLAY
  } else if (L.ext) {
#define REPLAY3(B, H) hipLaunchKernelGGL((replay3_kernel<B, H>), grid, block, replay3_lds_bytes(c), L.stream, L.cnt, L.ext, L.ppad, L.rt, L.rtp, c->tab.d_cp, L.nonn, L.amb, L.rb, L.re, L.ord_base, \
                                         c->state.d_heap, c->state.d_n, c->state.d_T, c->state.d_snap, L.entered, c->k, L.planes, L.tile_first, c->W4, c->tab.d_qp, c->tab.d_amb_q, c->stats.d_stats, L.q0, L.tb8, c->replay_prio)
#define REPLAY3_HALF(B) { if (c->replay_half == 32) REPLAY3(B, 32); else if (c->replay_half == 16) REPLAY3(B, 16); else REPLAY3(B, 8); }
    if (c->n_idx_c > 0) REPLAY3_HALF(true) else REPLAY3_HALF(false)
#undef REPLAY3_HALF
#undef REPLAY3
  } else {
    const int lq_words = (c->replay_lq && !c->acgt && lds + (size_t)c->W4 * 4 * 6 * 4 + 128 <= 64 * 1024) ? c->W4 * 4 * 6 : 0;
#define REPLAY2(A, B, PF_) hipLaunchKernelGGL((replay2_kernel<A, B, PF_>), grid, block, lds + (size_t)lq_words * 4 + 128, L.stream, L.cnt, L.ppad, L.rt, c->tab.d_cp, L.nonn, L.amb, L.rb, L.re, L.ord_base, \
                                              c->state.d_heap, c->state.d_n, c->state.d_T, c->state.d_snap, L.entered, c->k, L.planes, L.tile_first, c->W4, c->tab.d_qp, c->tab.d_amb_q, c->stats.d_stats, L.q0, L.tmin, L.qpl, lq_words, c->replay_prio, \
                                              L.poly, c->tab.NP4 + c->tab.NR4, c->tab.NP4, L.nr4, L.qrare)
#define REPLAY2_PF(A, B) { if (L.prefetch == 1) REPLAY2(A, B, 1); else if (L.prefetch == 2) REPLAY2(A, B, 2); else REPLAY2(A, B, 3); }
    if (c->acgt) { if (c->n_idx_c > 0) REPLAY2_PF(true, true) else REPLAY2_PF(true, false) }
    else         { if (c->n_idx_c > 0) REPLAY2_PF(false, true) else REPLAY2_PF(false, false) }
#undef REPLAY2_PF
#undef REPLAY2
  }
  HIPCHK(c, hipGetLastError());
  return 0;
}

int run_batch(uvaia_gpu_ctx *c, const TileStore &s, long long tile_first, int n_tiles, int r_begin, int r_end,
              long long ord_base)
{
  if (r_end <= r_begin) return 0;
  const int ppad = n_tiles * 64;
  const SliceBuf &b = c->slice[0];
  hipLaunchKernelGGL(snapshot_kernel, dim3(1), dim3(256), 0, c->st.stream, c->state.d_T, c->nq, c->state.d_snap);
  if (c->n_idx_c > 0 && c->fullscan) {
    if (c->acgt) hipLaunchKernelGGL((consensus_kernel<true>), dim3((n_tiles + 3) / 4), dim3(256), 0, c->st.stream, s.planes, tile_first, n_tiles, c->W4, c->tab.d_cp, c->state.d_snap, c->state.d_rt, c->state.d_tr);
    else         hipLaunchKernelGGL((consensus_kernel<false>), dim3((n_tiles + 3) / 4), dim3(256), 0, c->st.stream, s.planes, tile_first, n_tiles, c->W4, c->tab.d_cp, c->state.d_snap, c->state.d_rt, c->state.d_tr);
  }
  HIPCHK(c, hipGetLastError());
  const double bytes = (double)(r_end - r_begin) * (double)c->W4 * 16.0 * c->P + (double)c->nq * (double)c->W4 * 16.0 * c->P;
  uint32_t *ext = c->use_ext ? b.ext : nullptr;
  int rc = 0;
  if (c->fullscan) {
    rc = ensure_cnt4(c, (size_t)c->nq_pad * c->pool_pad); if (rc) return rc;
    rc = launch_scan(c, s, tile_first, n_tiles, c->tab.d_qp, c->nq, c->state.d_cnt, ppad, bytes);
  } else rc = launch_scan2(c, s, tile_first, n_tiles, b.cnt, ppad, bytes, nullptr, b.tmin, r_begin, r_end, b.rt, ext, b.rtp, b.tb8);
  if (rc) return rc;
  rc = launch_replay(c, {c->st.stream, 0, c->nq, b.cnt, ext, ppad, b.rt, b.rtp, b.tmin, b.tb8,
                             s.planes, tile_first, s.nonn + tile_first * 64, s.amb + tile_first * 64 * AMB_ROW, c->state.d_entered + tile_first * 64, r_begin, r_end, ord_base,
                             c->scan_variant == 2 ? c->tab.d_qpl : nullptr, s.poly, c->tab.NR4, c->tab.d_qrare, 3});
  if (rc) return rc;
  c->last = {&s, tile_first, n_tiles, r_end - r_begin, r_begin, ppad, c->fullscan ? c->state.d_rt : b.rt};
  return 0;
}

int derive_rows(uvaia_gpu_ctx *c, const TileStore &s, long long slot0, int n_ref, hipStream_t st = nullptr, bool v_in_place = false)
{
  if (!st) st = c->st.stream;
  if (c->fullscan || c->scan_variant != 2 || n_ref <= 0 || !c->tab.d_split) return 0;
  if (st == c->st.stream) planes_touch(c, st);
  const long long a = slot0 / 64, t1 = (slot0 + n_ref - 1) / 64;
  const int nblk = (int)(t1 - a + 1);
  const int waves = c->derive_waves ? c->derive_waves : 4;
#define DERIVE_ALL_W(A, V, N) hipLaunchKernelGGL((derive_all_kernel<A, V, N>), dim3(nblk), dim3(64 * N), 0, st, s.planes, a, a, c->W4, c->tab.d_cls, c->tab.d_rmask, c->tab.d_split + derive_split_offset(N), c->tab.NP4, c->tab.NR4, s.ev, s.tote, s.grp, s.poly)
#define DERIVE_ALL(A, V) { if (waves == 8) DERIVE_ALL_W(A, V, 8); else if (waves == 16) DERIVE_ALL_W(A, V, 16); else DERIVE_ALL_W(A, V, 4); }
  if (c->acgt) { if (v_in_place) DERIVE_ALL(true, false) else DERIVE_ALL(true, true) }
  else         { if (v_in_place) DERIVE_ALL(false, false) else DERIVE_ALL(false, true) }
#undef DERIVE_ALL
#undef DERIVE_ALL_W
  HIPCHK(c, hipGetLastError());
  return 0;
}

int sync_scan_streams(uvaia_gpu_ctx *c) { for (hipStream_t st : c->st.scan_streams) if (st) HIPCHK(c, hipStreamSynchronize(st)); planes_idle(c, false, true); return 0; }
int sync_derive_streams(uvaia_gpu_ctx *c) { for (hipStream_t st : c->st.derive_streams) if (st) HIPCHK(c, hipStreamSynchronize(st)); return 0; }

int slice_reserve(uvaia_gpu_ctx *c, SliceBuf &b, size_t need, size_t ppad)
{
  need = std::max(need, b.cnt.cap);
  if (need <= b.cnt.cap && b.tmin) return 0;
  if (int rc = sync_scan_streams(c)) return rc;
  HIPCHK(c, hipStreamSynchronize(c->st.stream));
  const size_t cap = std::max(need, (size_t)c->nq_pad * c->pool_pad), refs = std::max(cap / (size_t)c->nq_pad, ppad) + 64;
  if (int rc = b.cnt.reserve(c, cap)) return rc;
  if (int rc = b.tmin.reserve(c, cap / 64)) return rc;
  if (c->use_ext) {
    if (int rc = b.ext.reserve(c, cap)) return rc;
    if (int rc = b.tb8.reserve(c, cap / 64)) return rc;
    if (int rc = b.rtp.reserve(c, refs)) return rc;
  }
  return b.rt.reserve(c, refs);
}

static int settle_derive(uvaia_gpu_ctx *c)
{
  if (c->st.derive_pending) { if (int rc = sync_derive_streams(c)) return rc; c->st.derive_pending = 0; }
  return 0;
}


int db_refuse_full(uvaia_gpu_ctx *c) { return fail(c, UVAIA_GPU_ESTATE, "database capacity %zu exceeded: call uvaia_gpu_db_reserve first", c->db_cap); }

int db_make_room(uvaia_gpu_ctx *c, size_t n)
{
  if (int rc = settle_derive(c)) return rc;
  if (c->db_n + n <= c->db_cap) return 0;
  return c->db_n ? db_refuse_full(c) : uvaia_gpu_db_reserve(c, n);
}

int launch_pack_chunk(uvaia_gpu_ctx *c, const uint8_t *ds, int m, const TileStore &s, long long s0, const int *non_n)
{
  const long long t0 = s0 / 64, t1 = (s0 + m - 1) / 64;
  const int nblk = (int)(t1 - t0 + 1);
  int *nn_out = non_n ? nullptr : s.nonn.p;
  if (c->acgt) hipLaunchKernelGGL((pack_refs_kernel<3>), dim3(nblk), dim3(256), 0, c->st.stream, ds, c->pitch, c->nchar, s0, m, c->W4, s.planes, t0, nn_out, (int *)nullptr, s.tot, c->state.d_err);
  else         hipLaunchKernelGGL((pack_refs_kernel<4>), dim3(nblk), dim3(256), 0, c->st.stream, ds, c->pitch, c->nchar, s0, m, c->W4, s.planes, t0, nn_out, s.amb, s.tot, c->state.d_err);
  HIPCHK(c, hipGetLastError());
  if (non_n) HIPCHK(c, hipMemcpyAsync(s.nonn + s0, non_n, (size_t)m * sizeof(int), hipMemcpyHostToDevice, c->st.stream));
  return 0;
}

int take_pack_error(uvaia_gpu_ctx *c)
{
  int bad = 0;
  HIPCHK(c, hipMemcpy(&bad, c->state.d_err, sizeof(int), hipMemcpyDeviceToHost));
  if (!bad) return 0;
  HIPCHK(c, hipMemset(c->state.d_err, 0, sizeof(int)));
  return fail(c, UVAIA_GPU_EALPHABET, "a reference sequence holds a byte outside ACGT / MRWSYKVHDB / NX-?O.");
}

int db_import_tiles(uvaia_gpu_ctx *c, const uint4 *four, long long t0, size_t n_tiles)
{
  if (c->acgt) hipLaunchKernelGGL((import_tiles_kernel<3>), dim3((unsigned)n_tiles), dim3(256), 0, c->st.stream, four, c->W4, c->db.planes, t0, c->db.tot);
  else         hipLaunchKernelGGL((import_tiles_kernel<4>), dim3((unsigned)n_tiles), dim3(256), 0, c->st.stream, c->db.planes + (size_t)t0 * c->W4 * 4 * 64, c->W4, (uint4 *)nullptr, t0, c->db.tot);
  HIPCHK(c, hipGetLastError());
  return 0;
}

int db_sanitise_import(uvaia_gpu_ctx *c, size_t slot0, size_t n)
{
  hipLaunchKernelGGL(sanitise_import_kernel, dim3((unsigned)((n + 255) / 256)), dim3(256), 0, c->st.stream, c->acgt ? (int *)nullptr : c->db.amb + slot0 * AMB_ROW, c->db.nonn + slot0,
                     (long long)n, c->W4 * 4, c->nchar);
  HIPCHK(c, hipGetLastError());
  return 0;
}

int db_canonical_side_rows(uvaia_gpu_ctx *c, long long slot0, int n_ref, bool wait)
{
  if (c->acgt || n_ref <= 0 || !c->db.amb) return 0;
  const long long t0 = slot0 / 64, t1 = (slot0 + n_ref - 1) / 64;
  hipLaunchKernelGGL(side_rows_canonical_kernel, dim3((unsigned)(t1 - t0 + 1)), dim3(64), 0, c->st.stream, c->db.planes, c->W4, t0, slot0, n_ref, c->db.amb);
  HIPCHK(c, hipGetLastError());
  if (wait) HIPCHK(c, hipStreamSynchronize(c->st.stream));
  return 0;
}

int win_image_room(uvaia_gpu_ctx *c, size_t tiles, bool *grown)
{
  const size_t tile_u4 = (size_t)c->W4 * 4 * 64;
  if (!c->acgt || c->win.d_four.cap >= tiles * tile_u4) return 0;
  *grown = true;
  return c->win.d_four.reserve(c, std::max(tiles, c->db_cap / 64 + 1) * tile_u4);
}

void db_commit(uvaia_gpu_ctx *c, size_t db_n, int win_n) { c->db_n = db_n; c->win.n = win_n; }

int pack_rows(uvaia_gpu_ctx *c, const char *const *seq, const char *rows, size_t rows_pitch, const int *non_n, int n_ref, const TileStore &s, long long slot0)
{
  for (int done = 0, k = 0; done < n_ref; done += PACK_CHUNK, k ^= 1) {
    const int m = std::min(PACK_CHUNK, n_ref - done);
    if (c->stage_busy[k]) { HIPCHK(c, hipEventSynchronize(c->stage_free[k])); c->stage_busy[k] = false; }
    uint8_t *hs = c->h_stage + (size_t)k * PACK_CHUNK * c->pitch, *ds = c->d_stage + (size_t)k * PACK_CHUNK * c->pitch;
    for (int i = 0; i < m; i++) if (!(seq ? seq[done + i] : rows)) return fail(c, UVAIA_GPU_EINVAL, "NULL sequence at position %d", done + i);
    parallel_for(m, [&](int i) {
      const char *src = seq ? seq[done + i] : rows + (size_t)(done + i) * rows_pitch;
      memcpy(hs + (size_t)i * c->pitch, src, (size_t)c->nchar);
    });
    HIPCHK(c, hipMemcpyAsync(ds, hs, (size_t)m * c->pitch, hipMemcpyHostToDevice, c->st.stream));
    if (int rc = launch_pack_chunk(c, ds, m, s, slot0 + done, non_n ? non_n + done : nullptr)) return rc;
    HIPCHK(c, hipEventRecord(c->stage_free[k], c->st.stream)); c->stage_busy[k] = true;
  }
  { int rc = derive_rows(c, s, slot0, n_ref); if (rc) return rc; }
  HIPCHK(c, hipStreamSynchronize(c->st.stream));
  planes_idle(c, true, false);
  return take_pack_error(c);
}

}
```

uvaia_amd/csrc/host_open.inc:

```

extern "C" {

const char *uvaia_gpu_last_error(const uvaia_gpu_ctx *ctx) { return ctx ? ctx->err.c_str() : g_open_error.c_str(); }

void uvaia_gpu_close(uvaia_gpu_ctx *c)
{
  if (!c) return;
  if (c->st.stream) hipStreamSynchronize(c->st.stream);
  if (c->win.copy_stream) hipStreamSynchronize(c->win.copy_stream);
  for (hipStream_t st : c->st.derive_streams) if (st) hipStreamSynchronize(st);
  if (c->st.rep_stream) hipStreamSynchronize(c->st.rep_stream);
  for (auto &rank : c->shard.ipc_opened) for (void *p : rank) if (p) hipIpcCloseMemHandle(p);
  delete c;
}

int uvaia_gpu_open(uvaia_gpu_ctx **out, const uvaia_gpu_query *q, int heap_size, int device, size_t max_pool)
{ return uvaia_gpu_open_tuned(out, q, heap_size, device, max_pool, nullptr); }

int uvaia_gpu_open_tuned(uvaia_gpu_ctx **out, const uvaia_gpu_query *q, int heap_size, int device, size_t max_pool, const uvaia_gpu_tuning *tune)
{
  uvaia_gpu_tuning tn;
  memset(&tn, 0, sizeof tn);
  if (tune) tn = *tune;
  if (tn.scan < 0 || tn.scan > UVAIA_GPU_SCAN_WIDE || tn.query_tables < 0 || tn.query_tables > 2 || (tn.scan_tiles_per_wave != 0 && tn.scan_tiles_per_wave != 1 && tn.scan_tiles_per_wave != 2 && tn.scan_tiles_per_wave != 4) ||
      (tn.scan_waves_per_block != 0 && tn.scan_waves_per_block != 4 && tn.scan_waves_per_block != 8) || (tn.subslice_refs != 0 && tn.subslice_refs < 64) ||
      (tn.derive_waves != 0 && tn.derive_waves != 4 && tn.derive_waves != 8 && tn.derive_waves != 16))
    return fail(nullptr, UVAIA_GPU_EINVAL, "bad tuning values");
  if (!out) return fail(nullptr, UVAIA_GPU_EINVAL, "ctx is NULL");
  *out = nullptr;
  if (!q || q->n_query < 1 || q->nchar < 1 || !q->seq || !q->consensus) return fail(nullptr, UVAIA_GPU_EINVAL, "empty or incomplete query set");
  if ((q->n_idx_c && !q->idx_c) || (q->n_idx_m && !q->idx_m) || (q->n_idx && !q->idx)) return fail(nullptr, UVAIA_GPU_EINVAL, "index arrays missing");
  if (max_pool < 1) return fail(nullptr, UVAIA_GPU_EINVAL, "max_pool must be >= 1");
  int ndev = 0;
  if (hipGetDeviceCount(&ndev) != hipSuccess || ndev < 1) return fail(nullptr, UVAIA_GPU_ENODEV, "no HIP device available: the MI355X engine has no CPU fallback");
  if (device < 0) { if (hipGetDevice(&device) != hipSuccess) device = 0; }
  if (device >= ndev) return fail(nullptr, UVAIA_GPU_ENODEV, "device %d out of range (%d devices)", device, ndev);
  if (hipSetDevice(device) != hipSuccess) return fail(nullptr, UVAIA_GPU_ENODEV, "hipSetDevice(%d) failed", device);

  uvaia_gpu_ctx *c = new uvaia_gpu_ctx();
  c->device = device;
  c->nq = q->n_query; c->act_q0 = 0; c->act_q1 = q->n_query; c->nchar = q->nchar; c->acgt = q->acgt ? 1 : 0; c->trim = q->trim; c->n_idx_c = q->n_idx_c; c->n_idx_m = q->n_idx_m;
  c->P = c->acgt ? 3 : 4; c->NQ = c->acgt ? 4 : 6;
  c->W = (c->nchar + 31) / 32; c->W4 = (c->W + 3) / 4;
  c->k = heap_size < 2 ? 2 : heap_size;
  c->qt = c->nq <= 8 ? 8 : 16;
  c->scan_variant = tn.scan == UVAIA_GPU_SCAN_PACKED ? 0 : tn.scan == UVAIA_GPU_SCAN_COMPRESSED ? 2 : (c->nq <= 32 ? 0 : 2);
  c->fullscan = tn.scan == UVAIA_GPU_SCAN_WIDE;
  c->serial = tn.serial != 0;
  if (tn.scan_tiles_per_wave) c->scan_R = tn.scan_tiles_per_wave;
  if (tn.scan_waves_per_block) c->scan_NW = tn.scan_waves_per_block;
  if (c->scan_R == 4 && c->scan_NW != 8) { delete c; return fail(nullptr, UVAIA_GPU_EINVAL, "four reference tiles per wave go with eight waves per block"); }
  if (tn.subslice_refs) { c->subslice = tn.subslice_refs; c->subslice_forced = true; }
  if (tn.scan_streams >= 1 && tn.scan_streams <= 3) c->st.scan_nstreams_forced = tn.scan_streams;
  if (tn.scan_streams > 100 && tn.scan_streams < 200) c->first_slice_pct = tn.scan_streams == 199 ? 0 : tn.scan_streams - 100;
  c->derive_waves = tn.derive_waves;
  if (tn.ball_gather == 1 || tn.ball_gather == 2) c->ball.fused = tn.ball_gather == 2;
  if (tn.rederive_streams >= 1 && tn.rederive_streams <= 3) { c->st.derive_nstreams = tn.rederive_streams; c->st.derive_forced = true; }
  if (c->nchar > 49000) c->fullscan = true;
  c->nq_pad = ((c->nq + 127) / 128) * 128;
  c->max_pool = max_pool; c->pool_pad = ((max_pool + 63) / 64) * 64 + 64;
  c->pitch = ((size_t)c->nchar + 63) / 64 * 64;
  if ((size_t)(c->k + 1) * HEAP_ENTRY * sizeof(int) + 128 > 160 * 1024) { delete c; return fail(nullptr, UVAIA_GPU_EINVAL, "nbest=%d does not fit the per-query LDS heap (max 5115)", heap_size); }

#define OPENCHK(call) HIP_TRY(call, { const int rc_ = fail(nullptr, code_, "%s failed: %s", #call, hipGetErrorString(e_)); uvaia_gpu_close(c); return rc_; })
#define OPENBUF(buf, n) do { if (const int rc_ = (buf).reserve(nullptr, (n))) { uvaia_gpu_close(c); return rc_; } } while (0)
  c->use_ext = !c->fullscan && !c->acgt && tn.replay_extras != 1 && (c->scan_variant == 0 || (c->scan_variant == 2 && c->nq <= 128 && tn.replay_extras == 2));
  {
    int prio_least = 0, prio_greatest = 0;
    OPENCHK(hipDeviceGetStreamPriorityRange(&prio_least, &prio_greatest));
    bool split = false;
    const int want_half = tn.replay_cus >= 1000 ? tn.replay_cus / 1000 : 0, want_cus = tn.replay_cus >= 1000 ? tn.replay_cus % 1000 : tn.replay_cus;
    c->replay_half = (want_half == 32 || want_half == 16 || want_half == 8) ? want_half : c->nq <= 8 ? 32 : c->nq <= 24 ? 16 : 8;
    int per_cu = (int)std::min<size_t>(4, (size_t)160 * 1024 / replay3_lds_bytes(c));
    while (c->use_ext && c->replay_half > 8 && per_cu * 8 < std::min(c->nq, 32)) { c->replay_half /= 2; per_cu = (int)std::min<size_t>(4, (size_t)160 * 1024 / replay3_lds_bytes(c)); }
    if (c->use_ext && replay3_lds_bytes(c) > (size_t)160 * 1024) c->use_ext = false;
    const int rep_cus = want_cus < 0 ? 0 : want_cus > 0 ? want_cus : (c->use_ext && per_cu > 0 ? std::max(8, ((c->nq + per_cu - 1) / per_cu + 7) / 8 * 8) : 0);
    hipDeviceProp_t prop;
    if (rep_cus > 0 && hipGetDeviceProperties(&prop, device) == hipSuccess && prop.multiProcessorCount >= 4 * rep_cus) {
      const int ncu = prop.multiProcessorCount, words = (ncu + 31) / 32;
      std::vector<uint32_t> m_rep((size_t)words, 0u), m_scan((size_t)words, 0u);
      for (int b = 0; b < ncu; b++) (b < rep_cus ? m_rep : m_scan)[(size_t)b >> 5] |= 1u << (b & 31);
      hipStream_t st[7] = {};
      bool ok = hipExtStreamCreateWithCUMask(&st[0], (uint32_t)words, m_rep.data()) == hipSuccess;
      for (int i = 1; i < 7 && ok; i++) ok = hipExtStreamCreateWithCUMask(&st[i], (uint32_t)words, m_scan.data()) == hipSuccess;
      if (ok) ok = hipEventCreateWithFlags(&c->st.rep_ev[0].e, hipEventDisableTiming) == hipSuccess && hipEventCreateWithFlags(&c->st.rep_ev[1].e, hipEventDisableTiming) == hipSuccess;
      if (ok) {
        c->st.rep_stream.s = st[0];
        for (int i = 0; i < 3; i++) { c->st.scan_streams[i].s = st[1 + i]; c->st.derive_streams[i].s = st[4 + i]; }
        split = true; c->replay_cus = rep_cus;
      } else { (void)hipGetLastError(); for (int i = 0; i < 7; i++) if (st[i]) hipStreamDestroy(st[i]); }
    }
    OPENCHK(hipStreamCreateWithPriority(&c->st.stream.s, hipStreamNonBlocking, prio_greatest));
    if (!split) {
      for (int i = 0; i < 3; i++) OPENCHK(hipStreamCreateWithPriority(&c->st.scan_streams[i].s, hipStreamNonBlocking, prio_least));
      for (int i = 0; i < 3; i++) OPENCHK(hipStreamCreateWithPriority(&c->st.derive_streams[i].s, hipStreamNonBlocking, (prio_least + prio_greatest) / 2));
    }
    for (SliceBuf &b : c->slice) { OPENCHK(hipEventCreateWithFlags(&b.scan_done.e, hipEventDisableTiming)); OPENCHK(hipEventCreateWithFlags(&b.replay_done.e, hipEventDisableTiming)); }
  }
  uint8_t code_tab[256]; fill_code_table(code_tab);
  OPENCHK(hipMemcpyToSymbol(HIP_SYMBOL(c_code), code_tab, 256));

  const int lo = (int)std::min<size_t>(c->trim, (size_t)c->nchar), hi = std::max(lo, c->nchar - (int)c->trim);
  const size_t row_words = (size_t)c->W4 * 4 * c->NQ;
  std::vector<uint8_t> in_c(c->nchar, 0), in_m(c->nchar, 0), in_p(c->nchar, 0);
  for (int i = 0; i < q->n_idx_c; i++) if (q->idx_c[i] < (size_t)c->nchar) in_c[q->idx_c[i]] = 1;
  for (int i = 0; i < q->n_idx_m; i++) if (q->idx_m[i] < (size_t)c->nchar) in_m[q->idx_m[i]] = 1;
  for (int i = 0; i < q->n_idx; i++)   if (q->idx[i]   < (size_t)c->nchar) in_p[q->idx[i]] = 1;
  std::vector<uint32_t> cp(row_words, 0u), cpm(row_words, 0u);
  int bad = 0;
  for (int i = 0; i < c->nq; i++) if (!q->seq[i]) { uvaia_gpu_close(c); return fail(nullptr, UVAIA_GPU_EINVAL, "query %d is NULL", i); }
  if (pack_query_row(code_tab, q->consensus, c->nchar, 0, c->nchar, in_c.data(), nullptr, c->acgt, c->NQ, cp.data(), &bad) ||
      pack_query_row(code_tab, q->consensus, c->nchar, 0, c->nchar, in_m.data(), nullptr, c->acgt, c->NQ, cpm.data(), &bad)) {
    uvaia_gpu_close(c); return fail(nullptr, UVAIA_GPU_EALPHABET, "consensus holds byte 0x%02x outside the supported alphabet", bad);
  }
  {
    std::vector<uint32_t> pmask((size_t)c->W4 * 4, 0u);
    for (int sidx = lo; sidx < hi; sidx++) if (in_p[(size_t)sidx]) pmask[(size_t)sidx >> 5] |= 1u << (sidx & 31);
    OPENBUF(c->tab.d_pmask, pmask.size()); OPENCHK(hipMemcpy(c->tab.d_pmask, pmask.data(), pmask.size() * 4, hipMemcpyHostToDevice));
    std::vector<int> cols;
    for (int sidx = lo; sidx < hi; sidx++) if (in_p[(size_t)sidx]) cols.push_back(sidx);
    c->ball.n_idx = (int)cols.size(); c->ball.NG4 = std::max(1, ((c->ball.n_idx + 31) / 32 + 3) / 4);
    c->ball.idx_cols = cols;
    cols.resize(cols.size() + 1, 0);
    OPENBUF(c->ball.d_idx_cols, cols.size()); OPENCHK(hipMemcpy(c->ball.d_idx_cols, cols.data(), cols.size() * sizeof(int), hipMemcpyHostToDevice));
  }
  OPENBUF(c->d_stage, (size_t)2 * PACK_CHUNK * c->pitch);
  if (const int rc_ = c->h_stage.alloc(nullptr, (size_t)2 * PACK_CHUNK * c->pitch)) { uvaia_gpu_close(c); return rc_; }
  memset(c->h_stage, 'N', (size_t)2 * PACK_CHUNK * c->pitch);
  for (int i = 0; i < 2; i++) OPENCHK(hipEventCreateWithFlags(&c->stage_free[i].e, hipEventDisableTiming));
  if (tn.query_tables == 1) { const int rc_ = build_query_tables_host(c, q, tn, code_tab, lo, hi, in_p); if (rc_) { uvaia_gpu_close(c); return rc_; } }
  else                      { const int rc_ = build_query_tables_device(c, q, tn, lo, hi);               if (rc_) { uvaia_gpu_close(c); return rc_; } }
  OPENBUF(c->tab.d_cp, cp.size()); OPENCHK(hipMemcpy(c->tab.d_cp, cp.data(), cp.size() * 4, hipMemcpyHostToDevice));
  OPENBUF(c->tab.d_cpm, cpm.size()); OPENCHK(hipMemcpy(c->tab.d_cpm, cpm.data(), cpm.size() * 4, hipMemcpyHostToDevice));

  OPENBUF(c->state.d_heap, (size_t)c->nq * (c->k + 1) * HEAP_ENTRY);
  OPENBUF(c->state.d_n, (size_t)c->nq);
  OPENBUF(c->state.d_T, (size_t)c->nq);
  OPENBUF(c->state.d_snap, 1);
  OPENBUF(c->state.d_err, 1);
  OPENCHK(hipMemset(c->state.d_err, 0, sizeof(int)));
  SliceBuf &b0 = c->slice[0];
  if (!c->fullscan) OPENBUF(b0.cnt, (size_t)c->nq_pad * c->pool_pad);
  if (c->use_ext) {
    OPENBUF(b0.ext, (size_t)c->nq_pad * c->pool_pad);
    OPENBUF(b0.tb8, (size_t)c->nq_pad * (c->pool_pad / 64));
    OPENBUF(b0.rtp, c->pool_pad);
    OPENCHK(hipMemset(b0.rtp, 0, c->pool_pad * sizeof(uint32_t)));
    const size_t l3 = replay3_lds_bytes(c);
#define BIGLDS(K, N) OPENCHK(hipFuncSetAttribute(reinterpret_cast<const void *>(&K), hipFuncAttributeMaxDynamicSharedMemorySize, (int)(N)))
    BIGLDS((replay3_kernel<true, 32>), l3); BIGLDS((replay3_kernel<false, 32>), l3); BIGLDS((replay3_kernel<true, 16>), l3);
    BIGLDS((replay3_kernel<false, 16>), l3); BIGLDS((replay3_kernel<true, 8>), l3); BIGLDS((replay3_kernel<false, 8>), l3);
  }
  OPENBUF(b0.tmin, (size_t)c->nq_pad * (c->pool_pad / 64));
  OPENBUF(b0.rt, c->pool_pad);
  OPENCHK(hipMemset(b0.rt, 0, c->pool_pad * sizeof(int4)));
  OPENBUF(c->stats.d_stats, 16);
  OPENCHK(hipMemset(c->stats.d_stats, 0, 16 * sizeof(unsigned long long)));
  OPENBUF(c->state.d_rt, c->pool_pad);
  OPENBUF(c->state.d_tr, c->pool_pad);
  OPENCHK(hipMemset(c->state.d_rt, 0, c->pool_pad * sizeof(int4)));
  OPENCHK(hipMemset(c->state.d_tr, 0, c->pool_pad * sizeof(int4)));
  OPENBUF(c->state.d_entered, c->pool_pad);
  OPENCHK(hipMemset(c->state.d_entered, 0, c->pool_pad));
  const size_t lds = (size_t)(c->k + 1) * HEAP_ENTRY * sizeof(int) + 128;
  if (lds > 64 * 1024) {
    BIGLDS(replay_kernel<true>, lds); BIGLDS(replay_kernel<false>, lds);
#define BIGHEAP(PF_) BIGLDS((replay2_kernel<true, true, PF_>), lds); BIGLDS((replay2_kernel<true, false, PF_>), lds); BIGLDS((replay2_kernel<false, true, PF_>), lds); BIGLDS((replay2_kernel<false, false, PF_>), lds)
    BIGHEAP(1); BIGHEAP(2); BIGHEAP(3);
#undef BIGHEAP
  }
#undef BIGLDS
#undef OPENBUF
#undef OPENCHK
  int rc = uvaia_gpu_reset(c);
  if (rc) { g_open_error = c->err; uvaia_gpu_close(c); return rc; }
  *out = c;
  return UVAIA_GPU_OK;
}

int uvaia_gpu_export_query_table(uvaia_gpu_ctx *c, int which, void *out, size_t cap, size_t *n_bytes)
{
  if (!c || !n_bytes || which < 0 || which > 10) return UVAIA_GPU_EINVAL;
  if (which == 10) {
    const int v[11] = {c->tab.NP, c->tab.NR, c->tab.NP4, c->tab.NR4, c->tab.rare_max, c->scan_variant, c->tab.need_e_groups, c->tab.need_v_groups, c->tab.need_g_groups, c->tab.need_r_groups, c->replay_lq};
    *n_bytes = sizeof v;
    if (out && cap >= sizeof v) memcpy(out, v, sizeof v);
    return UVAIA_GPU_OK;
  }
  *n_bytes = c->tab.qtab[which].p ? c->tab.qtab[which].n : 0;
  if (out && *n_bytes && cap >= *n_bytes) {
    HIPCHK(c, hipSetDevice(c->device));
    HIPCHK(c, hipStreamSynchronize(c->st.stream));
    HIPCHK(c, hipMemcpy(out, c->tab.qtab[which].p, *n_bytes, hipMemcpyDeviceToHost));
  }
  return UVAIA_GPU_OK;
}

int uvaia_gpu_reset(uvaia_gpu_ctx *c)
{
  if (!c) return UVAIA_GPU_EINVAL;
  const size_t heap16 = (size_t)c->nq * (c->k + 1) * HEAP_ENTRY * sizeof(int) / 16;
  const size_t ent = (c->state.d_entered && c->db_n) ? std::min(c->state.d_entered.cap / 64 * 64, ((c->db_n + 63) / 64) * 64) : 0;
  const size_t work = std::max(std::max(heap16, ent / 16), (size_t)c->nq);
  hipLaunchKernelGGL(reset_state_kernel, dim3((unsigned)std::min<size_t>(1024, (work + 255) / 256)), dim3(256), 0, c->st.stream,
                     reinterpret_cast<uint4 *>(c->state.d_heap.p), heap16, c->state.d_T, c->state.d_n, c->nq, c->nchar, c->state.d_snap, reinterpret_cast<uint4 *>(c->state.d_entered.p), ent / 16);
  HIPCHK(c, hipGetLastError());
  c->state.entered_clean = ent;
  return 0;
}

int uvaia_gpu_heap_slots(const uvaia_gpu_ctx *c) { return c ? c->k : 0; }
int uvaia_gpu_n_query(const uvaia_gpu_ctx *c) { return c ? c->nq : 0; }
size_t uvaia_gpu_packed_bytes_per_ref(const uvaia_gpu_ctx *c) { return c ? (size_t)c->W4 * 16 * c->P : 0; }
size_t uvaia_gpu_scan_bytes_per_ref(const uvaia_gpu_ctx *c)
{
  if (!c) return 0;
  return (c->fullscan || c->scan_variant != 2) ? (size_t)c->W4 * 16 * c->P
                                                : (size_t)(c->tab.need_e_groups + c->tab.need_v_groups) * 16 + (size_t)c->tab.need_g_groups * 4 + (size_t)(c->tab.NP4 + c->tab.need_r_groups) * 16 * 3;
}

int uvaia_gpu_scan_variant(const uvaia_gpu_ctx *c)
{
  return !c ? -2 : c->fullscan ? -1 : c->scan_variant;
}

size_t uvaia_gpu_derived_bytes_per_ref(const uvaia_gpu_ctx *c)
{
  if (!c || c->fullscan || c->scan_variant != 2) return 0;
  return (size_t)c->W4 * 16 + (size_t)c->W4 * 4 + (size_t)(c->tab.NP4 + c->tab.NR4) * 48 + 4;
}

int uvaia_gpu_set_query_tile(uvaia_gpu_ctx *c, int qt)
{
  if (!c) return UVAIA_GPU_EINVAL;
  if (qt == 0) qt = 16;
  if (qt != 8 && qt != 16 && qt != 32) return fail(c, UVAIA_GPU_EINVAL, "query tile must be 8, 16 or 32");
  c->qt = qt;
  return 0;
}


}
```

uvaia_amd/csrc/host_resident.inc:

```

extern "C" {

int uvaia_gpu_db_reserve(uvaia_gpu_ctx *c, size_t cap)
{
  if (!c) return UVAIA_GPU_EINVAL;
  if (cap <= c->db_cap) return 0;
  if (c->db_n) return fail(c, UVAIA_GPU_ESTATE, "reserve the database before appending to it");
  const size_t tiles = (cap + 63) / 64 + 1;
  const size_t dtiles = derived_tiles(c, tiles) + (c->shard.world > 1 ? 1 : 0);
  if (int rc = store_alloc(c, c->db, dtiles)) return rc;
  c->db_local_tiles = dtiles;
  c->shard.peer_db[c->shard.rank] = c->db.planes; c->shard.peer_amb[c->shard.rank] = c->db.amb;
  c->db_cap = tiles * 64 - 64;
  c->state.entered_clean = 0;
  if (int rc = c->state.d_entered.reserve(c, tiles * 64)) return rc;
  HIPCHK(c, hipMemset(c->state.d_entered, 0, c->state.d_entered.cap));
  return 0;
}

static int db_append_common(uvaia_gpu_ctx *c, const char *const *seq, const char *rows, size_t pitch, const int *non_n, int n_ref)
{
  if (!c) return UVAIA_GPU_EINVAL;
  if (n_ref < 0) return fail(c, UVAIA_GPU_EINVAL, "negative count");
  if (n_ref == 0) return 0;
  if (int rc = db_make_room(c, (size_t)n_ref)) return rc;
  const long long s0 = (long long)c->db_n, s1 = s0 + n_ref;
  for (long long a = s0; a < s1;) {
    const long long pe = c->shard.world == 1 ? s1 : std::min(s1, (a / (c->shard.pt * 64) + 1) * c->shard.pt * 64);
    if (owns_tile(c, a / 64)) {
      const long long off = a - s0, local = dtile_of(c, a / 64) * 64 + a % 64;
      int rc = pack_rows(c, seq ? seq + off : nullptr, rows ? rows + (size_t)off * pitch : nullptr, pitch, non_n ? non_n + off : nullptr, (int)(pe - a), c->db, local);
      if (rc) return rc;
      rc = db_canonical_side_rows(c, local, (int)(pe - a), true);
      if (rc) return rc;
    }
    a = pe;
  }
  db_commit(c, c->db_n + (size_t)n_ref, 0);
  return 0;
}

int uvaia_gpu_db_skip(uvaia_gpu_ctx *c, size_t n_ref)
{
  if (!c) return UVAIA_GPU_EINVAL;
  if (!n_ref) return 0;
  if (c->db_n + n_ref > c->db_cap) return db_refuse_full(c);
  for (size_t a = c->db_n; a < c->db_n + n_ref; a = (a / 64 + 1) * 64)
    if (owns_tile(c, (long long)(a / 64))) return fail(c, UVAIA_GPU_EINVAL, "reference %zu belongs to a piece of this context: it cannot be skipped", a);
  c->db_n += n_ref;
  return 0;
}

int uvaia_gpu_db_append(uvaia_gpu_ctx *c, const char *const *seq, const int *non_n, int n_ref)
{ if (c && n_ref > 0 && !seq) return fail(c, UVAIA_GPU_EINVAL, "NULL seq"); return db_append_common(c, seq, nullptr, 0, non_n, n_ref); }

int uvaia_gpu_db_append_block(uvaia_gpu_ctx *c, const char *rows, size_t pitch, const int *non_n, int n_ref)
{
  if (c && n_ref > 0 && (!rows || pitch < (size_t)c->nchar)) return fail(c, UVAIA_GPU_EINVAL, "bad block");
  return db_append_common(c, nullptr, rows, pitch, non_n, n_ref);
}

size_t uvaia_gpu_db_size(const uvaia_gpu_ctx *c) { return c ? c->db_n : 0; }

int uvaia_gpu_db_clear(uvaia_gpu_ctx *c)
{
  if (!c) return UVAIA_GPU_EINVAL;
  c->win.n = 0;
  if (!c->db.planes || !c->db_n) { c->db_n = 0; return 0; }
  { int rc = settle_derive(c); if (rc) return rc; }
  HIPCHK(c, hipStreamSynchronize(c->st.stream));
  if (int rc = sync_scan_streams(c)) return rc;
  const size_t tiles = c->shard.world == 1 ? (c->db_n + 63) / 64 : c->db_local_tiles;
  HIPCHK(c, hipMemsetAsync(c->db.planes, 0, tiles * (size_t)c->W4 * c->P * 64 * sizeof(uint4), c->st.stream));
  HIPCHK(c, hipMemsetAsync(c->db.nonn, 0, tiles * 64 * sizeof(int), c->st.stream));
  HIPCHK(c, hipMemsetAsync(c->db.tot, 0, tiles * 64 * sizeof(int), c->st.stream));
  HIPCHK(c, hipMemsetAsync(c->db.amb, 0, tiles * 64 * AMB_ROW * sizeof(int), c->st.stream));
  HIPCHK(c, hipStreamSynchronize(c->st.stream));
  c->db_n = 0;
  return 0;
}

size_t uvaia_gpu_db_tile_bytes(const uvaia_gpu_ctx *c) { return c ? (size_t)c->W4 * 4 * 64 * sizeof(uint4) : 0; }
int uvaia_gpu_db_side_row_ints(void) { return AMB_ROW; }

int uvaia_gpu_db_export(uvaia_gpu_ctx *c, size_t first_tile, size_t n_tiles, void *planes, int *non_n, int *side_rows)
{
  if (!c || !planes || !non_n || !side_rows) return UVAIA_GPU_EINVAL;
  if (c->acgt) return fail(c, UVAIA_GPU_ESTATE, "the interchange form is the four IUPAC planes: export from a default-mode context");
  if (c->shard.world > 1) return fail(c, UVAIA_GPU_ESTATE, "a context of a reference shard holds its own pieces only: export from a plain context");
  if ((first_tile + n_tiles) * 64 > ((c->db_n + 63) / 64) * 64) return fail(c, UVAIA_GPU_EINVAL, "tiles %zu..%zu lie outside the database", first_tile, first_tile + n_tiles);
  if (!n_tiles) return 0;
  HIPCHK(c, hipStreamSynchronize(c->st.stream));
  const size_t tb = uvaia_gpu_db_tile_bytes(c);
  HIPCHK(c, hipMemcpy(planes, reinterpret_cast<const char *>(c->db.planes.p) + first_tile * tb, n_tiles * tb, hipMemcpyDeviceToHost));
  HIPCHK(c, hipMemcpy(non_n, c->db.nonn + first_tile * 64, n_tiles * 64 * sizeof(int), hipMemcpyDeviceToHost));
  HIPCHK(c, hipMemcpy(side_rows, c->db.amb + first_tile * 64 * AMB_ROW, n_tiles * 64 * AMB_ROW * sizeof(int), hipMemcpyDeviceToHost));
  return 0;
}

int uvaia_gpu_db_derived_export(uvaia_gpu_ctx *c, size_t n_tiles, void *e, uint32_t *grp, void *poly, int *tot)
{
  if (!c || !e || !grp || !poly || !tot) return UVAIA_GPU_EINVAL;
  if (c->fullscan || c->scan_variant != 2 || !c->db.ev) return fail(c, UVAIA_GPU_ESTATE, "only the column-compressed scan keeps planes derived for the query set");
  if (c->shard.world > 1) return fail(c, UVAIA_GPU_ESTATE, "a context of a reference shard numbers its derived tiles by piece: read them from a plain context");
  if (n_tiles * 64 > ((c->db_n + 63) / 64) * 64) return fail(c, UVAIA_GPU_EINVAL, "tiles 0..%zu lie outside the database", n_tiles);
  if (!n_tiles) return 0;
  { int rc = settle_derive(c); if (rc) return rc; }
  HIPCHK(c, hipStreamSynchronize(c->st.stream));
  const size_t W4 = (size_t)c->W4, NG = (size_t)(c->tab.NP4 + c->tab.NR4);
  HIPCHK(c, hipMemcpy2D(e, 1024, c->db.ev, 2048, 1024, n_tiles * W4, hipMemcpyDeviceToHost));
  HIPCHK(c, hipMemcpy(grp, c->db.grp, n_tiles * W4 * 64 * sizeof(uint32_t), hipMemcpyDeviceToHost));
  if (NG) HIPCHK(c, hipMemcpy(poly, c->db.poly, n_tiles * NG * 3 * 64 * sizeof(uint4), hipMemcpyDeviceToHost));
  HIPCHK(c, hipMemcpy(tot, c->db.tote, n_tiles * 64 * sizeof(int), hipMemcpyDeviceToHost));
  return 0;
}

int uvaia_gpu_db_append_packed(uvaia_gpu_ctx *c, const void *planes, const int *non_n, const int *side_rows, int n_ref)
{
  if (!c) return UVAIA_GPU_EINVAL;
  if (n_ref < 0) return fail(c, UVAIA_GPU_EINVAL, "negative count");
  if (n_ref == 0) return 0;
  if (!planes || !non_n || (!c->acgt && !side_rows)) return fail(c, UVAIA_GPU_EINVAL, "NULL packed arrays");
  if (c->db_n % 64) return fail(c, UVAIA_GPU_ESTATE, "packed tiles can only follow a whole number of tiles (database holds %zu references)", c->db_n);
  if (int rc = db_make_room(c, (size_t)n_ref)) return rc;
  const size_t tb = uvaia_gpu_db_tile_bytes(c), n_tiles_all = ((size_t)n_ref + 63) / 64;
  const long long t0g = (long long)(c->db_n / 64);
  int rc = for_owned_tiles(c, t0g, t0g + (long long)n_tiles_all, [&](long long gt, long long t0, long long nt) -> int {
    const size_t n_tiles = (size_t)nt, off = (size_t)(gt - t0g);
    const char *pl = reinterpret_cast<const char *>(planes) + off * tb;
    if (!c->acgt) {
      HIPCHK(c, hipMemcpyAsync(reinterpret_cast<char *>(c->db.planes.p) + (size_t)t0 * tb, pl, n_tiles * tb, hipMemcpyHostToDevice, c->st.stream));
      if (int rc = db_import_tiles(c, nullptr, t0, n_tiles)) return rc;
      HIPCHK(c, hipMemcpyAsync(c->db.amb + (size_t)t0 * 64 * AMB_ROW, side_rows + off * 64 * AMB_ROW, n_tiles * 64 * AMB_ROW * sizeof(int), hipMemcpyHostToDevice, c->st.stream));
    } else {
      const size_t chunk = 64;
      DevBuf<uint4> d_tmp;
      if (int rc = d_tmp.reserve(c, chunk * tb / sizeof(uint4))) return rc;
      for (size_t a = 0; a < n_tiles; a += chunk) {
        const size_t m = std::min(chunk, n_tiles - a);
        HIPCHK(c, hipMemcpyAsync(d_tmp, pl + a * tb, m * tb, hipMemcpyHostToDevice, c->st.stream));
        if (int rc = db_import_tiles(c, d_tmp, t0 + (long long)a, m)) return rc;
        HIPCHK(c, hipStreamSynchronize(c->st.stream));
      }
    }
    HIPCHK(c, hipMemcpyAsync(c->db.nonn + (size_t)t0 * 64, non_n + off * 64, n_tiles * 64 * sizeof(int), hipMemcpyHostToDevice, c->st.stream));
    if (int rc = db_sanitise_import(c, (size_t)t0 * 64, n_tiles * 64)) return rc;
    return derive_rows(c, c->db, t0 * 64, (int)(n_tiles * 64));
  });
  if (rc) return rc;
  HIPCHK(c, hipStreamSynchronize(c->st.stream));
  db_commit(c, c->db_n + (size_t)n_ref, 0);
  return 0;
}

struct SubSlice { size_t first, n; bool pool_start; };
#ifndef HEAD_TAIL_NQT
#define HEAD_TAIL_NQT 17
#endif
static std::vector<SubSlice> plan_subslices(const uvaia_gpu_ctx *c, size_t first, size_t n, size_t pool)
{
  std::vector<SubSlice> subs;
  const int nqt = (c->act_q1 + 15) / 16 - c->act_q0 / 16;
  if (c->n_idx_c == 0) pool = std::max<size_t>(n, 1);
  size_t sub = c->subslice;
  if (nqt <= 32) sub /= 2;
  if (nqt < 63) sub = std::min(pool, (sub * 63 / (size_t)std::max(nqt, 1) + 63) / 64 * 64);
  if (nqt < 4) sub = std::min(pool, std::max<size_t>(65536, ((pool + 3) / 4 + 63) / 64 * 64));
  if (c->subslice_forced) sub = std::min(pool, c->subslice);
  for (size_t a = first; a < first + n; a += pool) {
    const size_t pe = std::min(first + n, a + pool);
    if (nqt < HEAD_TAIL_NQT && !c->subslice_forced && pe - a >= 8 * 65536) {
      const size_t head = 65536, tail = 65536, pre = (nqt < 4 && pe - a >= 12 * 65536) ? 131072 : 0, mid = pe - a - head - tail - pre, nm = std::max<size_t>(1, (mid + sub / 2) / sub);
      const size_t each = ((mid + nm - 1) / nm + 63) / 64 * 64;
      subs.push_back({a, head, true});
      for (size_t x = a + head; x < pe - tail - pre; x += each) subs.push_back({x, std::min(each, pe - tail - pre - x), false});
      if (pre) subs.push_back({pe - tail - pre, pre, false});
      subs.push_back({pe - tail, tail, false});
      continue;
    }
    const size_t len = pe - a, ns = std::max<size_t>(1, (len + sub / 2) / sub);
    const size_t each = ((len + ns - 1) / ns + 63) / 64 * 64;
    if (c->first_slice_pct > 0 && c->first_slice_pct < 100 && ns >= 3 && !c->subslice_forced) {
      const size_t first_n = std::max<size_t>(64, each * (size_t)c->first_slice_pct / 100 / 64 * 64), rest = len - first_n;
      const size_t each2 = ((rest + (ns - 1) - 1) / (ns - 1) + 63) / 64 * 64;
      subs.push_back({a, first_n, true});
      for (size_t x = a + first_n; x < pe; x += each2) subs.push_back({x, std::min(each2, pe - x), false});
      continue;
    }
    for (size_t x = a; x < pe; x += each) subs.push_back({x, std::min(each, pe - x), x == a});
  }
  return subs;
}

int uvaia_gpu_db_rederive(uvaia_gpu_ctx *c)
{
  if (!c) return UVAIA_GPU_EINVAL;
  if (!c->db.planes || !c->db_n || c->fullscan || c->scan_variant != 2) return 0;
  HIPCHK(c, hipSetDevice(c->device));
  std::vector<SubSlice> plan;
  if (c->shard.world == 1) plan = plan_subslices(c, 0, c->db_n, c->max_pool);
  else {
    const size_t piece = (size_t)c->shard.pt * 64;
    for (size_t a = (size_t)c->shard.rank * piece; a < c->db_n; a += piece * (size_t)c->shard.world) plan.push_back({a, std::min(piece, c->db_n - a), false});
  }
  const int n_derive_streams = (c->st.derive_forced || plan.size() <= 3) ? c->st.derive_nstreams : 1;
  {
    hipStream_t busy[4] = {c->st.stream, c->st.scan_streams[0], c->st.scan_streams[1], c->st.scan_streams[2]};
    for (int i = 0; i < 4; i++) {
      if (!busy[i] || !c->st.planes_busy[i]) continue;
      hipEvent_t e = c->st.planes_ev[i];
      if (!e) {
        if (int rc = c->st.derive_fence[i].make(c, hipEventDisableTiming)) return rc;
        HIPCHK(c, hipEventRecord(c->st.derive_fence[i], busy[i]));
        planes_fenced(c, busy[i], e = c->st.derive_fence[i]);
      }
      for (int j = 0; j < n_derive_streams; j++) HIPCHK(c, hipStreamWaitEvent(c->st.derive_streams[j], e, 0));
    }
  }
  size_t k = 0;
  long long t_done = 0;
  for (const SubSlice &sl : plan) {
    const long long t0 = std::max(t_done, (long long)(sl.first / 64)), t1 = (long long)((sl.first + sl.n + 63) / 64);
    if (t0 >= t1) continue;
    t_done = t1;
    hipStream_t ds = c->st.derive_streams[k % (size_t)n_derive_streams];
    int rc = for_owned_tiles(c, t0, t1, [&](long long, long long lt, long long nt) -> int { return derive_rows(c, c->db, lt * 64, (int)(nt * 64), ds, true); });
    if (rc) return rc;
    if (k == c->st.derive_chunks.size()) {
      c->st.derive_chunks.emplace_back();
      if (int rc = c->st.derive_chunks.back().done.make(c, hipEventDisableTiming)) { c->st.derive_chunks.pop_back(); return rc; }
    }
    c->st.derive_chunks[k].t0 = t0; c->st.derive_chunks[k].t1 = t1;
    HIPCHK(c, hipEventRecord(c->st.derive_chunks[k].done, ds));
    k++;
  }
  c->st.derive_pending = k;
  return 0;
}

static int run_subslices(uvaia_gpu_ctx *c, const std::vector<SubSlice> &subs, int64_t ordinal_of_db0, int snapshot)
{
  const size_t ns = subs.size();
  size_t issued = 0;
  {
    const int nqt = (c->act_q1 + 15) / 16 - c->act_q0 / 16;
    size_t longest = 0;
    for (const SubSlice &sl : subs) longest = std::max(longest, sl.n);
    const size_t waves = ns ? (size_t)nqt * ((longest + 63) / 64) : 0;
    c->st.scan_nstreams = (waves && waves < 16000 && nqt >= 4 && !c->use_ext) ? 3 : 1;
    if (c->st.scan_nstreams_forced) c->st.scan_nstreams = c->st.scan_nstreams_forced;
  }
  for (size_t i = 0; i < ns; i++) {
    const bool serial_ = c->serial;
    while (issued < ns && issued < i + (serial_ ? 1 : NBUF)) {
      int rc = uvaia_gpu_slice_scan(c, subs[issued].first, subs[issued].n, (int)(issued % NBUF));
      if (rc) return rc;
      issued++;
      if (serial_) (void)sync_scan_streams(c);
    }
    int take = subs[i].pool_start ? 1 : 0;
    if (take && snapshot >= 0) { HIPCHK(c, hipMemcpyAsync(c->state.d_snap, &snapshot, sizeof(int), hipMemcpyHostToDevice, c->st.stream)); HIPCHK(c, hipStreamSynchronize(c->st.stream)); take = 0; }
    int rc = uvaia_gpu_slice_replay(c, (int)(i % NBUF), ordinal_of_db0 + (long long)subs[i].first, take);
    if (rc) return rc;
    if (serial_) hipStreamSynchronize(c->st.stream);
  }
  return 0;
}

int uvaia_gpu_search_resident(uvaia_gpu_ctx *c, size_t pool, int64_t ordinal0, uint8_t *entered)
{
  if (!c) return UVAIA_GPU_EINVAL;
  if (c->shard.world > 1) return fail(c, UVAIA_GPU_ESTATE, "a context of a reference shard keeps its own pieces only: use uvaia_gpu_shard_scan / uvaia_gpu_shard_replay (or a group)");
  if (pool < 1 || pool > c->max_pool) return fail(c, UVAIA_GPU_EINVAL, "pool must be in [1, max_pool=%zu]", c->max_pool);
  if (!c->db_n) return 0;
  if (c->state.entered_clean < ((c->db_n + 63) / 64) * 64) HIPCHK(c, hipMemsetAsync(c->state.d_entered, 0, ((c->db_n + 63) / 64) * 64, c->st.stream));
  c->state.entered_clean = 0;
  if (!c->fullscan) {
    int rc = run_subslices(c, plan_subslices(c, 0, c->db_n, pool), ordinal0, -1);
    if (rc) return rc;
  } else
  for (size_t a = 0; a < c->db_n; a += pool) {
    const size_t b = std::min(c->db_n, a + pool);
    const long long tf = (long long)(a / 64);
    const int n_tiles = (int)((b + 63) / 64 - a / 64);
    const int rb = (int)(a - (size_t)tf * 64), re = (int)(b - (size_t)tf * 64);
    int rc = run_batch(c, c->db, tf, n_tiles, rb, re, ordinal0 + (long long)a);
    if (rc) return rc;
  }
  if (entered) {
    HIPCHK(c, hipMemcpyAsync(entered, c->state.d_entered, c->db_n, hipMemcpyDeviceToHost, c->st.stream));
    HIPCHK(c, hipStreamSynchronize(c->st.stream));
    return collect_events(c);
  }
  return 0;
}

int uvaia_gpu_search_resident_pool(uvaia_gpu_ctx *c, size_t first, size_t n, int64_t ordinal0, int snapshot)
{
  if (!c) return UVAIA_GPU_EINVAL;
  if (c->fullscan) return fail(c, UVAIA_GPU_ESTATE, "per-pool search needs the default scan");
  if (n < 1 || n > c->max_pool || first + n > c->db_n) return fail(c, UVAIA_GPU_EINVAL, "pool [%zu,+%zu) outside the database or above max_pool=%zu", first, n, c->max_pool);
  return run_subslices(c, plan_subslices(c, first, n, n), ordinal0 - (int64_t)first, snapshot);
}

int uvaia_gpu_sync(uvaia_gpu_ctx *c)
{
  if (!c) return UVAIA_GPU_EINVAL;
  if (int rc = sync_derive_streams(c)) return rc;
  c->st.derive_pending = 0;
  if (int rc = sync_scan_streams(c)) return rc;
  HIPCHK(c, hipStreamSynchronize(c->st.stream));
  if (c->st.rep_stream) HIPCHK(c, hipStreamSynchronize(c->st.rep_stream));
  planes_idle(c, true, true);
  return collect_events(c);
}

int uvaia_gpu_last_batch_scores(uvaia_gpu_ctx *c, int *out, int n_ref)
{
  if (!c || !out) return UVAIA_GPU_EINVAL;
  if (n_ref != c->last.n || !c->last.store) return fail(c, UVAIA_GPU_ESTATE, "last batch held %d references, not %d", c->last.n, n_ref);
  const int *nonn = c->last.store->nonn + c->last.tile_first * 64;
  DevBuf<int> d_out;
  const size_t bytes = (size_t)n_ref * c->nq * 6 * sizeof(int);
  if (!c->fullscan) {
    int rc = ensure_cnt4(c, (size_t)c->nq_pad * c->last.ppad); if (rc) return rc;
    const bool prof = c->stats.profile; c->stats.profile = false;
    rc = launch_scan(c, *c->last.store, c->last.tile_first, c->last.n_tiles, c->tab.d_qp, c->nq, c->state.d_cnt, c->last.ppad, 0.0);
    c->stats.profile = prof;
    if (rc) return rc;
  }
  if (int rc = d_out.reserve(c, bytes / sizeof(int))) return rc;
  dim3 grid((n_ref + 255) / 256, c->nq);
  if (c->acgt) hipLaunchKernelGGL((batch_scores_kernel<true>), grid, dim3(256), 0, c->st.stream, c->state.d_cnt, c->last.ppad, c->last.rt, nonn, c->last.rbegin, n_ref, c->nq, d_out);
  else         hipLaunchKernelGGL((batch_scores_kernel<false>), grid, dim3(256), 0, c->st.stream, c->state.d_cnt, c->last.ppad, c->last.rt, nonn, c->last.rbegin, n_ref, c->nq, d_out);
  hipError_t e = hipGetLastError();
  if (e == hipSuccess) e = hipMemcpyAsync(out, d_out, bytes, hipMemcpyDeviceToHost, c->st.stream);
  if (e == hipSuccess) e = hipStreamSynchronize(c->st.stream);
  if (e != hipSuccess) return fail(c, UVAIA_GPU_EHIP, "batch_scores: %s", hipGetErrorString(e));
  return 0;
}

int uvaia_gpu_scan_stats(uvaia_gpu_ctx *c, double *ms, long long *launches, double *bytes, int reset)
{
  if (!c) return UVAIA_GPU_EINVAL;
  int rc = collect_events(c); if (rc) return rc;
  if (ms) *ms = c->stats.scan_ms;
  if (launches) *launches = c->stats.scan_launches;
  if (bytes) *bytes = c->stats.scan_bytes;
  if (reset) { c->stats.scan_ms = 0; c->stats.scan_bytes = 0; c->stats.scan_launches = 0; }
  return 0;
}

int uvaia_gpu_replay_stats(uvaia_gpu_ctx *c, unsigned long long out[3], int reset)
{
  if (!c || !out) return UVAIA_GPU_EINVAL;
  HIPCHK(c, hipStreamSynchronize(c->st.stream));
  unsigned long long h[3] = {0, 0, 0};
  HIPCHK(c, hipMemcpy(h, c->stats.d_stats, sizeof h, hipMemcpyDeviceToHost));
  out[0] = h[0]; out[1] = h[1]; out[2] = h[2];
  if (reset) HIPCHK(c, hipMemset(c->stats.d_stats, 0, sizeof h));
  return 0;
}

int uvaia_gpu_replay_timing(uvaia_gpu_ctx *c, unsigned long long out[12], int reset)
{
  if (!c || !out) return UVAIA_GPU_EINVAL;
  HIPCHK(c, hipStreamSynchronize(c->st.stream));
  HIPCHK(c, hipMemcpy(out, c->stats.d_stats + 4, 12 * sizeof(unsigned long long), hipMemcpyDeviceToHost));
  if (reset) HIPCHK(c, hipMemset(c->stats.d_stats + 4, 0, 12 * sizeof(unsigned long long)));
  return 0;
}

int uvaia_gpu_replay_tiles_opened(uvaia_gpu_ctx *c, unsigned long long *out, int reset)
{
  if (!c || !out) return UVAIA_GPU_EINVAL;
  HIPCHK(c, hipStreamSynchronize(c->st.stream));
  unsigned long long h3 = 0;
  HIPCHK(c, hipMemcpy(&h3, c->stats.d_stats + 3, sizeof h3, hipMemcpyDeviceToHost));
  *out = h3;
  if (reset) HIPCHK(c, hipMemset(c->stats.d_stats + 3, 0, sizeof h3));
  return 0;
}

size_t uvaia_gpu_state_range_bytes(const uvaia_gpu_ctx *c, int q0, int q1)
{
  if (!c || q0 < 0 || q1 > c->nq || q1 < q0) return 0;
  const size_t nqr = (size_t)(q1 - q0);
  return sizeof(int) * (4 + 2 * nqr + nqr * (c->k + 1) * HEAP_ENTRY);
}
size_t uvaia_gpu_state_bytes(const uvaia_gpu_ctx *c) { return c ? uvaia_gpu_state_range_bytes(c, 0, c->nq) : 0; }

int uvaia_gpu_state_export_range(uvaia_gpu_ctx *c, void *dst, int q0, int q1)
{
  if (!c || !dst || q0 < 0 || q1 > c->nq || q1 < q0) return UVAIA_GPU_EINVAL;
  int *d = (int *)dst;
  const size_t nqr = (size_t)(q1 - q0), he = (size_t)(c->k + 1) * HEAP_ENTRY;
  HIPCHK(c, hipMemcpyAsync(d, c->state.d_snap, sizeof(int), hipMemcpyDefault, c->st.stream));
  if (nqr) {
    HIPCHK(c, hipMemcpyAsync(d + 4, c->state.d_n + q0, nqr * sizeof(int), hipMemcpyDefault, c->st.stream));
    HIPCHK(c, hipMemcpyAsync(d + 4 + nqr, c->state.d_T + q0, nqr * sizeof(int), hipMemcpyDefault, c->st.stream));
    HIPCHK(c, hipMemcpyAsync(d + 4 + 2 * nqr, c->state.d_heap + (size_t)q0 * he, nqr * he * sizeof(int), hipMemcpyDefault, c->st.stream));
  }
  HIPCHK(c, hipStreamSynchronize(c->st.stream));
  return 0;
}

int uvaia_gpu_state_import_range(uvaia_gpu_ctx *c, const void *src, int q0, int q1)
{
  if (!c || !src || q0 < 0 || q1 > c->nq || q1 < q0) return UVAIA_GPU_EINVAL;
  const int *d = (const int *)src;
  const size_t nqr = (size_t)(q1 - q0), he = (size_t)(c->k + 1) * HEAP_ENTRY;
  HIPCHK(c, hipMemcpyAsync(c->state.d_snap, d, sizeof(int), hipMemcpyDefault, c->st.stream));
  if (nqr) {
    HIPCHK(c, hipMemcpyAsync(c->state.d_n + q0, d + 4, nqr * sizeof(int), hipMemcpyDefault, c->st.stream));
    HIPCHK(c, hipMemcpyAsync(c->state.d_T + q0, d + 4 + nqr, nqr * sizeof(int), hipMemcpyDefault, c->st.stream));
    HIPCHK(c, hipMemcpyAsync(c->state.d_heap + (size_t)q0 * he, d + 4 + 2 * nqr, nqr * he * sizeof(int), hipMemcpyDefault, c->st.stream));
  }
  HIPCHK(c, hipStreamSynchronize(c->st.stream));
  return 0;
}

int uvaia_gpu_state_export(uvaia_gpu_ctx *c, void *dst) { return c ? uvaia_gpu_state_export_range(c, dst, 0, c->nq) : UVAIA_GPU_EINVAL; }
int uvaia_gpu_state_import(uvaia_gpu_ctx *c, const void *src) { return c ? uvaia_gpu_state_import_range(c, src, 0, c->nq) : UVAIA_GPU_EINVAL; }

int uvaia_gpu_slice_scan(uvaia_gpu_ctx *c, size_t first, size_t n, int buf)
{
  if (!c || buf < 0 || buf >= NBUF) return UVAIA_GPU_EINVAL;
  if (c->fullscan) return fail(c, UVAIA_GPU_ESTATE, "ring mode needs the two-counter scan");
  if (c->shard.world > 1) return fail(c, UVAIA_GPU_ESTATE, "a context of a reference shard keeps its own pieces only: use uvaia_gpu_shard_scan / uvaia_gpu_shard_replay");
  if (first + n > c->db_n) return fail(c, UVAIA_GPU_EINVAL, "slice [%zu,+%zu) outside the database", first, n);
  if (n > c->max_pool && c->n_idx_c > 0) return fail(c, UVAIA_GPU_EINVAL, "slice of %zu references above max_pool %zu", n, c->max_pool);
  SliceBuf &b = c->slice[buf];
  const size_t ppad_ = ((first + n + 63) / 64 - first / 64) * 64;
  const size_t qtile = c->scan_variant == 2 ? 64 : 16;
  const size_t rows = std::min<size_t>((size_t)c->nq_pad, ((size_t)c->act_q1 + qtile - 1) / qtile * qtile);
  if (int rc = slice_reserve(c, b, rows * ppad_, ppad_)) return rc;
  hipStream_t ss = c->st.scan_streams[c->st.scan_nstreams > 1 ? (c->st.scan_rr++ % c->st.scan_nstreams) : 0];
  if (b.replay_recorded) HIPCHK(c, hipStreamWaitEvent(ss, b.replay_done, 0));
  for (size_t k = 0; k < c->st.derive_pending; k++) {
    const auto &d = c->st.derive_chunks[k];
    if (d.t0 < (long long)((first + n + 63) / 64) && d.t1 > (long long)(first / 64)) HIPCHK(c, hipStreamWaitEvent(ss, d.done, 0));
  }
  b.tf = (long long)(first / 64);
  b.tiles = n ? (int)((first + n + 63) / 64 - first / 64) : 0;
  b.rb = (int)(first - (size_t)b.tf * 64); b.re = b.rb + (int)n;
  b.scanned = true; b.cons_done = false;
  const double bytes = (double)n * (double)c->W4 * 16.0 * c->P + (double)c->nq * (double)c->W4 * 16.0 * c->P;
  int rc = launch_scan2(c, c->db, b.tf, b.tiles, b.cnt, b.tiles * 64, bytes, ss, b.tmin, b.rb, b.re, b.rt, c->use_ext ? b.ext : nullptr, b.rtp, b.tb8);
  if (rc) return rc;
  HIPCHK(c, hipEventRecord(b.scan_done, ss));
  planes_fenced(c, ss, b.scan_done);
  return 0;
}

int uvaia_gpu_slice_replay_range(uvaia_gpu_ctx *c, int buf, int64_t ordinal0, int q0, int q1, int take_snapshot)
{
  if (!c || buf < 0 || buf >= NBUF) return UVAIA_GPU_EINVAL;
  SliceBuf &b = c->slice[buf];
  if (!b.scanned) return fail(c, UVAIA_GPU_ESTATE, "slice_replay without slice_scan");
  if (q0 < 0 || q1 > c->nq || q1 < q0) return fail(c, UVAIA_GPU_EINVAL, "bad query range [%d,%d)", q0, q1);
  if (take_snapshot) { hipLaunchKernelGGL(snapshot_kernel, dim3(1), dim3(256), 0, c->st.stream, c->state.d_T + c->act_q0, c->act_q1 - c->act_q0, c->state.d_snap); b.cons_done = false; }
  if (b.re <= b.rb || q1 == q0) return 0;
  HIPCHK(c, hipStreamWaitEvent(c->st.stream, b.scan_done, 0));
  const int ppad = b.tiles * 64;
  const uint32_t *ext = c->use_ext ? b.ext : nullptr;
  hipStream_t rs = (c->st.rep_stream && ext) ? c->st.rep_stream : c->st.stream;
  if (rs != c->st.stream) { HIPCHK(c, hipEventRecord(c->st.rep_ev[0], c->st.stream)); HIPCHK(c, hipStreamWaitEvent(rs, c->st.rep_ev[0], 0)); }
  const int pf = (q1 - q0) <= 64 ? 1 : 2;
  int rc = launch_replay(c, {rs, q0, q1, b.cnt, ext, ppad, b.rt, b.rtp, b.tmin, b.tb8,
                             c->db.planes, b.tf, c->db.nonn + b.tf * 64, c->db.amb + b.tf * 64 * AMB_ROW, c->state.d_entered + b.tf * 64, b.rb, b.re, (long long)ordinal0,
                             (c->scan_variant == 2 && c->shard.world == 1) ? c->tab.d_qpl : nullptr, c->db.poly, c->tab.NR4, c->tab.d_qrare, pf});
  if (rc) return rc;
  if (rs != c->st.stream) { HIPCHK(c, hipEventRecord(c->st.rep_ev[1], rs)); HIPCHK(c, hipStreamWaitEvent(c->st.stream, c->st.rep_ev[1], 0)); }
  HIPCHK(c, hipEventRecord(b.replay_done, c->st.stream));
  planes_fenced(c, c->st.stream, b.replay_done);
  b.replay_recorded = true;
  c->last = {&c->db, b.tf, b.tiles, b.re - b.rb, b.rb, ppad, b.rt};
  return 0;
}

int uvaia_gpu_slice_buffers(void) { return NBUF; }

int uvaia_gpu_slice_replay(uvaia_gpu_ctx *c, int buf, int64_t ordinal0, int stripe_start)
{ return c ? uvaia_gpu_slice_replay_range(c, buf, ordinal0, c->act_q0, c->act_q1, stripe_start) : UVAIA_GPU_EINVAL; }

int uvaia_gpu_set_active_queries(uvaia_gpu_ctx *c, int q0, int q1)
{
  if (!c) return UVAIA_GPU_EINVAL;
  if (q0 < 0 || q1 > c->nq || q1 <= q0 || ((q0 % 64) && c->shard.world == 1))
    return fail(c, UVAIA_GPU_EINVAL, "active queries [%d,%d): need 0 <= q0 < q1 <= %d and q0 a multiple of 64", q0, q1, c->nq);
  if ((c->fullscan || c->scan_variant != 2) && c->shard.world == 1) { if (q0 != 0 || q1 != c->nq) return fail(c, UVAIA_GPU_ESTATE, "query shards need the default scan"); }
  c->act_q0 = q0; c->act_q1 = q1;
  return 0;
}

int uvaia_gpu_max_tolerance(uvaia_gpu_ctx *c, int *out)
{
  if (!c || !out) return UVAIA_GPU_EINVAL;
  DevBuf<int> d_tmp;
  if (int rc = d_tmp.reserve(c, 1)) return rc;
  hipLaunchKernelGGL(snapshot_kernel, dim3(1), dim3(256), 0, c->st.stream, c->state.d_T + c->act_q0, c->act_q1 - c->act_q0, d_tmp);
  hipError_t e = hipGetLastError();
  if (e == hipSuccess) e = hipMemcpyAsync(out, d_tmp, sizeof(int), hipMemcpyDeviceToHost, c->st.stream);
  if (e == hipSuccess) e = hipStreamSynchronize(c->st.stream);
  if (e != hipSuccess) return fail(c, UVAIA_GPU_EHIP, "max_tolerance: %s", hipGetErrorString(e));
  return 0;
}

int uvaia_gpu_entered_flags(uvaia_gpu_ctx *c, uint8_t *out, int clear)
{
  if (!c) return UVAIA_GPU_EINVAL;
  HIPCHK(c, hipStreamSynchronize(c->st.stream));
  if (out && c->db_n) HIPCHK(c, hipMemcpy(out, c->state.d_entered, c->db_n, hipMemcpyDeviceToHost));
  if (clear && c->db_n) HIPCHK(c, hipMemset(c->state.d_entered, 0, ((c->db_n + 63) / 64) * 64));
  return 0;
}


}
```

uvaia_amd/csrc/kernels_scan3.inc:

```


typedef uint32_t u32x4_nt __attribute__((ext_vector_type(4)));
static __device__ __forceinline__ void st_stream(uint4 *p, const uint4 &v)
{
  const u32x4_nt x = {v.x, v.y, v.z, v.w};
  __builtin_nontemporal_store(x, reinterpret_cast<u32x4_nt *>(p));
}
struct GatherStage { uint32_t bL, bH, bI; int fill, ow; };

template <int NWV>
static __device__ __forceinline__ int shared_slot(const int *__restrict__ bit, int word)
{
  for (int k = 1; k < NWV; k++) if ((bit[k] & 31) != 0 && (bit[k] >> 5) == word) return k;
  return 0;
}
static __device__ __forceinline__ uint32_t take_bit(uint32_t x, int b, int at, uint32_t acc)
{
  return (__builtin_amdgcn_ubfe(x, (uint32_t)b, 1u) << at) | acc;
}

template <bool ACGT, bool WRITE_V, int NWV>
__global__ __launch_bounds__(64 * NWV) __attribute__((amdgpu_waves_per_eu(8, 8)))
void derive_all_kernel(const uint4 *__restrict__ tiles, long long tile_base, long long dtile_base, int W4,
                       const uint32_t *__restrict__ cls, const uint32_t *__restrict__ rmask,
                       const int *__restrict__ split, int NP4, int NR4,
                       uint4 *__restrict__ ev, int *__restrict__ tot_e, uint32_t *__restrict__ grp, uint4 *__restrict__ poly)
{
  constexpr int P = ACGT ? 3 : 4;
  __shared__ int partial[NWV][64];
  __shared__ uint32_t shr[2 * (NWV - 1)][3][64];
  for (int i = threadIdx.x; i < 2 * (NWV - 1) * 3 * 64; i += 64 * NWV) (&shr[0][0][0])[i] = 0u;
  __syncthreads();
  const int lane = threadIdx.x & 63, wv = __builtin_amdgcn_readfirstlane(threadIdx.x >> 6);
  const long long ptile = tile_base + blockIdx.x, tile = dtile_base + blockIdx.x;
  const uint4 *t = tiles + (size_t)ptile * W4 * P * 64 + lane;
  uint4 *o = ev + (size_t)tile * W4 * 2 * 64 + lane;
  const int NG = NP4 + NR4;
  uint32_t *po = reinterpret_cast<uint32_t *>(poly + (size_t)tile * NG * 3 * 64 + lane);
  const int lo = split[wv], hi = split[wv + 1];
  const int *dbit = split + (NWV + 1), *rbit = split + 2 * (NWV + 1);

  GatherStage D, R;
  D.bL = D.bH = D.bI = 0u; D.fill = dbit[wv] & 31; D.ow = dbit[wv] >> 5;
  R.bL = R.bH = R.bI = 0u; R.fill = rbit[wv] & 31; R.ow = rbit[wv] >> 5;
  int sw[2][2], sk[2][2];
#pragma unroll
  for (int sec = 0; sec < 2; sec++) {
    const int *bit = sec ? rbit : dbit;
    sw[sec][0] = (bit[wv] & 31) != 0 ? (bit[wv] >> 5) : -1;
    sw[sec][1] = (wv + 1 < NWV && (bit[wv + 1] & 31) != 0) ? (bit[wv + 1] >> 5) : -1;
#pragma unroll
    for (int e = 0; e < 2; e++) sk[sec][e] = sw[sec][e] >= 0 ? shared_slot<NWV>(bit, sw[sec][e]) : 0;
  }
  auto push_word = [&](GatherStage &g, int sec) {
    const int k = (sw[sec][0] == g.ow) ? sk[sec][0] : (sw[sec][1] == g.ow) ? sk[sec][1] : 0;
    if (k) {
      uint32_t (*dst)[64] = shr[sec * (NWV - 1) + k - 1];
      if (g.bL) atomicOr(&dst[0][lane], g.bL);
      if (g.bH) atomicOr(&dst[1][lane], g.bH);
      if (g.bI) atomicOr(&dst[2][lane], g.bI);
    } else {
      uint32_t *d = po + (size_t)((sec ? NP4 : 0) + (g.ow >> 2)) * 3 * 256 + (g.ow & 3);
      d[0] = g.bL; d[256] = g.bH; d[512] = g.bI;
    }
    g.bL = g.bH = g.bI = 0u; g.fill = 0; g.ow++;
  };

  int te = 0;
  uint4 nxt[P];
#pragma unroll
  for (int p = 0; p < P; p++) nxt[p] = lo < hi ? ld_stream(t + (size_t)(lo * P + p) * 64) : make_uint4(0u, 0u, 0u, 0u);
  for (int w4 = lo; w4 < hi; w4++) {
    uint4 pl[P];
#pragma unroll
    for (int p = 0; p < P; p++) pl[p] = nxt[p];
    if (w4 + 1 < hi) {
#pragma unroll
      for (int p = 0; p < P; p++) nxt[p] = ld_stream(t + (size_t)((w4 + 1) * P + p) * 64);
    }
    uint32_t e[4], v[4];
    int ge = 0, gv = 0;
#pragma unroll
    for (int j = 0; j < 4; j++) {
      uint32_t rL, rH, rI, rV;
      if (ACGT) { rL = u4c(pl[0], j); rH = u4c(pl[1], j); rI = u4c(pl[2], j); rV = rI; }
      else {
        const uint32_t a = u4c(pl[0], j), cc = u4c(pl[1], j), g = u4c(pl[2], j), tt = u4c(pl[P - 1], j);
        const uint32_t par = a ^ cc ^ g ^ tt, three = (a & cc & (g | tt)) | (g & tt & (a | cc));
        rI = par & ~three; rL = (cc | tt) & rI; rH = (g | tt) & rI; rV = a | cc | g | tt;
      }
      const uint32_t *c4 = cls + (size_t)(w4 * 4 + j) * 4;
      const uint32_t diff = (rL ^ c4[0]) | (rH ^ c4[1]);
      e[j] = rI & c4[2] & (ACGT ? diff : ~diff);
      v[j] = rV;
      ge += __popc(e[j]); gv += __popc(v[j]);
      for (uint32_t m = c4[3]; m; m &= m - 1) {
        const int b = __ffs(m) - 1;
        D.bL = take_bit(rL, b, D.fill, D.bL); D.bH = take_bit(rH, b, D.fill, D.bH); D.bI = take_bit(rI, b, D.fill, D.bI);
        if (++D.fill == 32) push_word(D, 0);
      }
      for (uint32_t m = rmask[w4 * 4 + j]; m; m &= m - 1) {
        const int b = __ffs(m) - 1;
        R.bL = take_bit(rL, b, R.fill, R.bL); R.bH = take_bit(rH, b, R.fill, R.bH); R.bI = take_bit(rI, b, R.fill, R.bI);
        if (++R.fill == 32) push_word(R, 1);
      }
    }
    te += ge;
    __builtin_nontemporal_store((uint32_t)ge | ((uint32_t)gv << 16), grp + ((size_t)tile * W4 + w4) * 64 + lane);
    st_stream(o + (size_t)(w4 * 2 + 0) * 64, make_uint4(e[0], e[1], e[2], e[3]));
    if (WRITE_V) st_stream(o + (size_t)(w4 * 2 + 1) * 64, make_uint4(v[0], v[1], v[2], v[3]));
  }
  if (NP4 && D.fill > 0) push_word(D, 0);
  if (NR4 && R.fill > 0) push_word(R, 1);
  if (wv == NWV - 1) {
    for (int w = (dbit[NWV] + 31) >> 5; w < NP4 * 4; w++) { uint32_t *d = po + (size_t)(w >> 2) * 3 * 256 + (w & 3); d[0] = 0u; d[256] = 0u; d[512] = 0u; }
    for (int w = (rbit[NWV] + 31) >> 5; w < NR4 * 4; w++) { uint32_t *d = po + (size_t)(NP4 + (w >> 2)) * 3 * 256 + (w & 3); d[0] = 0u; d[256] = 0u; d[512] = 0u; }
  }
  partial[wv][lane] = te;
  __syncthreads();
  if (wv == 0) {
    int t_all = 0;
#pragma unroll
    for (int v = 0; v < NWV; v++) t_all += partial[v][lane];
    tot_e[tile * 64 + lane] = t_all;
  } else {
    for (int sec = 0; sec < 2; sec++) {
      if ((sec ? NR4 : NP4) == 0 || sw[sec][0] < 0 || sk[sec][0] != wv) continue;
      const int w = sw[sec][0];
      const uint32_t (*src)[64] = shr[sec * (NWV - 1) + wv - 1];
      uint32_t *d = po + (size_t)((sec ? NP4 : 0) + (w >> 2)) * 3 * 256 + (w & 3);
      d[0] = src[0][lane]; d[256] = src[1][lane]; d[512] = src[2][lane];
    }
  }
}

template <int R> struct Scan3Acc;
template <> struct Scan3Acc<1> { typedef uint32_t type; };
template <> struct Scan3Acc<2> { typedef unsigned long long type; };
struct Scan3Acc4 { unsigned long long a, b; };
template <> struct Scan3Acc<4> { typedef Scan3Acc4 type; };
static __device__ __forceinline__ uint32_t acc_part(uint32_t v, int) { return v; }
static __device__ __forceinline__ uint32_t acc_part(unsigned long long v, int rr) { return (uint32_t)(v >> (32 * rr)); }
static __device__ __forceinline__ uint32_t acc_part(const Scan3Acc4 &v, int rr) { return (uint32_t)((rr < 2 ? v.a : v.b) >> (32 * (rr & 1))); }
typedef __attribute__((address_space(3))) char scan3_lds_char;
static __device__ __forceinline__ void lds_counter_add(scan3_lds_char *p, uint32_t v)
{ __hip_atomic_fetch_add((__attribute__((address_space(3))) uint32_t *)p, v, __ATOMIC_RELAXED, __HIP_MEMORY_SCOPE_WORKGROUP); }
static __device__ __forceinline__ void lds_counter_add(scan3_lds_char *p, unsigned long long v)
{ __hip_atomic_fetch_add((__attribute__((address_space(3))) unsigned long long *)p, v, __ATOMIC_RELAXED, __HIP_MEMORY_SCOPE_WORKGROUP); }
static __device__ __forceinline__ void lds_counter_add(scan3_lds_char *p, const Scan3Acc4 &v)
{
  __hip_atomic_fetch_add((__attribute__((address_space(3))) unsigned long long *)p, v.a, __ATOMIC_RELAXED, __HIP_MEMORY_SCOPE_WORKGROUP);
  __hip_atomic_fetch_add((__attribute__((address_space(3))) unsigned long long *)(p + 8), v.b, __ATOMIC_RELAXED, __HIP_MEMORY_SCOPE_WORKGROUP);
}
template <class T> static __device__ __forceinline__ void lds_counter_store(scan3_lds_char *p, const T &v) { *(__attribute__((address_space(3))) T *)p = v; }
static __device__ __forceinline__ void lds_counter_store(scan3_lds_char *p, const Scan3Acc4 &v)
{ *(__attribute__((address_space(3))) unsigned long long *)p = v.a; *(__attribute__((address_space(3))) unsigned long long *)(p + 8) = v.b; }
template <class T> static __device__ __forceinline__ void lds_counter_load(scan3_lds_char *p, T &v) { v = *(__attribute__((address_space(3))) T *)p; }
static __device__ __forceinline__ void lds_counter_load(scan3_lds_char *p, Scan3Acc4 &v)
{ v.a = *(__attribute__((address_space(3))) unsigned long long *)p; v.b = *(__attribute__((address_space(3))) unsigned long long *)(p + 8); }
static __device__ __forceinline__ void lds_counter_sub(scan3_lds_char *p, uint32_t v)
{ __hip_atomic_fetch_sub((__attribute__((address_space(3))) uint32_t *)p, v, __ATOMIC_RELAXED, __HIP_MEMORY_SCOPE_WORKGROUP); }
static __device__ __forceinline__ void lds_counter_sub(scan3_lds_char *p, unsigned long long v)
{ __hip_atomic_fetch_sub((__attribute__((address_space(3))) unsigned long long *)p, v, __ATOMIC_RELAXED, __HIP_MEMORY_SCOPE_WORKGROUP); }
static __device__ __forceinline__ void lds_counter_sub(scan3_lds_char *p, const Scan3Acc4 &v)
{
  __hip_atomic_fetch_sub((__attribute__((address_space(3))) unsigned long long *)p, v.a, __ATOMIC_RELAXED, __HIP_MEMORY_SCOPE_WORKGROUP);
  __hip_atomic_fetch_sub((__attribute__((address_space(3))) unsigned long long *)(p + 8), v.b, __ATOMIC_RELAXED, __HIP_MEMORY_SCOPE_WORKGROUP);
}

template <int NW , bool ACGT, int R, int QS = 64 >
__global__ __launch_bounds__(64 * NW) __attribute__((amdgpu_waves_per_eu(4, 8))) void scan3_kernel(const uint4 *__restrict__ ev, const uint4 *__restrict__ poly, long long tile_first, int n_tiles,
                                                     int W4, int NP4, int NPT, const uint32_t *__restrict__ qpl, const uint32_t *__restrict__ stream,
                                                     const uint32_t *__restrict__ sdir, const uint32_t *__restrict__ grp,
                                                     const int *__restrict__ tot_e, const int *__restrict__ tot_v,
                                                     uint32_t *__restrict__ out, int ppad, int n_stiles, int2 *__restrict__ tmin, int r_lo, int r_hi,
                                                     int stile_first)
{
  constexpr int QT = QS / NW;
  static_assert((NW == 4 || NW == 8 || NW == 16) && (QS == 64 || QS == 128) && QT >= 4 && QT <= 16, "waves and queries of a super-tile");
  static_assert(R == 1 || R == 2 || R == 4, "one, two or four reference tiles per wave");
  typedef typename Scan3Acc<R>::type acc_t;
  constexpr uint32_t RARE_BIAS = SCAN3_BIAS;
  __shared__ acc_t lacc[QS + 1][64];
  const int lane = threadIdx.x & 63, wave = __builtin_amdgcn_readfirstlane(threadIdx.x >> 6);
  int stile, group;
  if (!scan_work_item(n_stiles, (n_tiles + R - 1) / R, stile, group)) return;
  const int trel0 = group * R;
  stile += stile_first;
  const int q0 = stile * QS + wave * QT;
  int trel[R]; bool live[R];
#pragma unroll
  for (int rr = 0; rr < R; rr++) { live[rr] = trel0 + rr < n_tiles; trel[rr] = live[rr] ? trel0 + rr : trel0; }
  scan3_lds_char *my = (scan3_lds_char *)&lacc[wave * QT][lane];
  auto pack_acc = [](const uint32_t (&v)[R]) -> acc_t {
    if constexpr (R == 1) return v[0];
    else if constexpr (R == 2) return (acc_t)v[0] | ((acc_t)v[1] << 32);
    else return acc_t{(unsigned long long)v[0] | ((unsigned long long)v[1] << 32), (unsigned long long)v[2] | ((unsigned long long)v[3] << 32)};
  };
  {
    int acc[R][QT];
#pragma unroll
    for (int rr = 0; rr < R; rr++)
#pragma unroll
      for (int q = 0; q < QT; q++) acc[rr][q] = 0;
    {
      const uint4 *t[R];
#pragma unroll
      for (int rr = 0; rr < R; rr++) t[rr] = poly + (size_t)(tile_first + trel[rr]) * NPT * 3 * 64 + lane;
      const size_t qstride = (size_t)NP4 * 16;
      const uint32_t *qb = qpl + (size_t)q0 * qstride;
      for (int p4 = 0; p4 < NP4; p4++) {
        uint4 pL[R], pH[R], pI[R];
#pragma unroll
        for (int rr = 0; rr < R; rr++) { pL[rr] = t[rr][(size_t)(p4 * 3 + 0) * 64]; pH[rr] = t[rr][(size_t)(p4 * 3 + 1) * 64]; pI[rr] = t[rr][(size_t)(p4 * 3 + 2) * 64]; }
        const uint32_t *s0 = qb + (size_t)p4 * 16;
        QWords<12> cur, nxt;
        load_qwords(cur, s0);
#pragma unroll
        for (int q = 0; q < QT; q++) {
          if (q + 1 < QT) load_qwords(nxt, s0 + (size_t)(q + 1) * qstride);
          __builtin_amdgcn_sched_barrier(0);
#pragma unroll
          for (int rr = 0; rr < R; rr++)
#pragma unroll
            for (int j = 0; j < 4; j++) {
              const uint32_t d = u4c(pL[rr], j) ^ cur.v[j];
              const uint32_t y = B3(u4c(pH[rr], j), cur.v[4 + j], d, (TT_A ^ TT_B) | TT_C);
              acc[rr][q] = bcnt_acc(ACGT ? B3(y, u4c(pI[rr], j), cur.v[8 + j], TT_A & TT_B & TT_C) : B3(y, u4c(pI[rr], j), cur.v[8 + j], ~(~TT_A & TT_B & TT_C)), acc[rr][q]);
            }
          __builtin_amdgcn_sched_barrier(0);
          if (q + 1 < QT) cur = nxt;
        }
      }
    }
#pragma unroll
    for (int q = 0; q < QT; q++) {
      uint32_t init[R];
#pragma unroll
      for (int rr = 0; rr < R; rr++) {
        if (ACGT) init[rr] = RARE_BIAS - (uint32_t)acc[rr][q];
        else init[rr] = (uint32_t)acc[rr][q] + RARE_BIAS;
      }
      lds_counter_store(my + (size_t)q * 64 * sizeof(acc_t), pack_acc(init));
    }
  }
  __syncthreads();
  {
    const uint4 *t[R]; const uint32_t *gt[R];
#pragma unroll
    for (int rr = 0; rr < R; rr++) { t[rr] = ev + (size_t)(tile_first + trel[rr]) * W4 * 2 * 64 + lane; gt[rr] = grp + (size_t)(tile_first + trel[rr]) * W4 * 64 + lane; }
    typedef __attribute__((address_space(4))) const uint32_t cst_u32;
    const cst_u32 *dir = (const cst_u32 *)(sdir + (size_t)stile * 4 * NW);
    const cst_u32 *sp = (const cst_u32 *)(stream + dir[2 * wave]);
    scan3_lds_char *myc = (scan3_lds_char *)&lacc[0][lane];
#define LDS_ADD(byte_off, val) lds_counter_add(myc + (byte_off), (val))
#define LDS_SUB(byte_off, val) lds_counter_sub(myc + (byte_off), (val))
#define TOUCH_ITEM(it) asm volatile("" ::"s"(it.v[0]), "s"(it.v[1]), "s"(it.v[2]), "s"(it.v[3]), "s"(it.v[4]), "s"(it.v[5]), "s"(it.v[6]), "s"(it.v[7]), "s"(it.v[8]))
#define TOUCH4(it) asm volatile("" ::"s"(it.v[0]), "s"(it.v[1]), "s"(it.v[2]), "s"(it.v[3]))
    struct Planes { uint4 E[R], V[R]; uint32_t g[R]; };
    Planes PA, PB;
    auto request = [&](Planes &P, uint32_t h0) {
#pragma unroll
      for (int rr = 0; rr < R; rr++) {
        const char *tg = reinterpret_cast<const char *>(t[rr]) + (h0 & ~1023u);
        P.E[rr] = *reinterpret_cast<const uint4 *>(tg);
        P.V[rr] = *reinterpret_cast<const uint4 *>(tg + 1024);
        P.g[rr] = *reinterpret_cast<const uint32_t *>(reinterpret_cast<const char *>(gt[rr]) + ((h0 & ~1023u) >> 3));
      }
    };
    QWords<4> h, hn, hnn;
    load_qwords(h, sp);
    const cst_u32 *sp_n = sp + h.v[3];
    load_qwords(hn, sp_n);
    request(PA, h.v[0]);
    const uint32_t n_rec = dir[2 * wave + 1];
#define RECORD(P, Pn)                                                                                                             \
    {                                                                                                                             \
      const uint32_t n_full4 = h.v[1] & 0xFFFFu, n_gen = h.v[1] >> 16, n_words = h.v[2];                                          \
      const cst_u32 *sp_nn = sp_n + hn.v[3];                                                                                      \
      load_qwords(hnn, sp_nn);                                                                                                    \
      request(Pn, hn.v[0]);                                                                                                       \
      sp += 4;                                                                                                                    \
                                   \
      const cst_u32 *ip = sp + n_full4 * 4u, *wp = ip + n_gen * 12u;                                                              \
      QWords<9> a, b;                                                                                                             \
      QWords<4> it, nx;                                                                                                           \
      load_qwords(a, ip);                                                                                                         \
      load_qwords(it, wp);                                                                                                        \
      if (n_full4) {     \
        const acc_t gg = pack_acc(P.g);                                                                                           \
        _Pragma("unroll 1") for (uint32_t k = 0; k < n_full4; k++, sp += 4) {       \
          QWords<4> o;                                                                                                            \
          load_qwords(o, sp);                                                                                                     \
          LDS_ADD(o.v[0], gg); LDS_ADD(o.v[1], gg); LDS_ADD(o.v[2], gg); LDS_ADD(o.v[3], gg);                                     \
        }                                                                                                                         \
      }                                                                                                                           \
      if (n_gen) {                                                                                                                \
         \
         \
                 \
        TOUCH_ITEM(a);                                                                                                            \
        for (uint32_t k = 0; k < n_gen; k += 2, ip += 24) {                                                                       \
          acc_t va, vb;                                                                                                           \
          load_qwords(b, ip + 12);                              \
          __builtin_amdgcn_sched_barrier(0);                                                                                      \
          ITEM_VALUE(P, a, va);                                                                                                   \
          const uint32_t off_a = a.v[8];                                                                                          \
          __builtin_amdgcn_sched_barrier(0);                                                                                      \
          TOUCH_ITEM(b);                                                                                                          \
          LDS_ADD(off_a, va);                                                                                                     \
          if (k + 1 < n_gen) {                                                                                                    \
            load_qwords(a, ip + 24);                                                                                              \
            __builtin_amdgcn_sched_barrier(0);                                                                                    \
            ITEM_VALUE(P, b, vb);                                                                                                 \
            const uint32_t off_b = b.v[8];                                                                                        \
            __builtin_amdgcn_sched_barrier(0);                                                                                    \
            TOUCH_ITEM(a);                                                                                                        \
            LDS_ADD(off_b, vb);                                                                                                   \
          }                                                                                                                       \
        }                                                                                                                         \
      }                                                                                                                           \
      if (n_words) {     \
                                                   \
        uint32_t wE[R], wV[R];       \
        _Pragma("unroll") for (int rr = 0; rr < R; rr++) { wE[rr] = 0u; wV[rr] = 0u; }                                            \
        if (h.v[0] & 1u) {                                                                                                        \
          _Pragma("unroll") for (int rr = 0; rr < R; rr++) {                                                                      \
            wE[rr] = (uint32_t)bcnt_acc(P.E[rr].x, 0) | (uint32_t)bcnt_acc(P.E[rr].y, 0) << 8 | (uint32_t)bcnt_acc(P.E[rr].z, 0) << 16 | (uint32_t)bcnt_acc(P.E[rr].w, 0) << 24; \
            wV[rr] = (uint32_t)bcnt_acc(P.V[rr].x, 0) | (uint32_t)bcnt_acc(P.V[rr].y, 0) << 8 | (uint32_t)bcnt_acc(P.V[rr].z, 0) << 16 | (uint32_t)bcnt_acc(P.V[rr].w, 0) << 24; \
          }                                                                                                                       \
        }                                                                                                                         \
        TOUCH4(it);                                                                                                               \
        WORD_ITEMS(P, 0) WORD_ITEMS(P, 1) WORD_ITEMS(P, 2) WORD_ITEMS(P, 3)                                                       \
      }                                                                                                                           \
      sp = sp_n; sp_n = sp_nn; h = hn; hn = hnn;                                                                                  \
    }
#define ITEM_VALUE(P, it, dst)                                                                                      \
    {                                                                                                               \
      uint32_t pk_[R];                                                                                              \
      _Pragma("unroll") for (int rr = 0; rr < R; rr++) {                                                            \
        int e_ = 0, v_ = 0;                                                                                         \
        _Pragma("unroll") for (int j = 0; j < 4; j++) e_ = bcnt_acc(u4c(P.E[rr], j) & it.v[j], e_);                 \
        _Pragma("unroll") for (int j = 0; j < 4; j++) v_ = bcnt_acc(u4c(P.V[rr], j) & it.v[4 + j], v_);             \
        pk_[rr] = (uint32_t)e_ | ((uint32_t)v_ << 16);                                                              \
      }                                                                                                             \
      dst = pack_acc(pk_);                                                                                          \
    }
         \
#define WORD_ITEM(P, J, cur, ahead)                                                                                               \
        {                                                                                                                         \
          __builtin_amdgcn_sched_barrier(0);                                                                                      \
          uint32_t pk_[R];                                                                                                        \
          _Pragma("unroll") for (int rr = 0; rr < R; rr++)                                                                        \
            pk_[rr] = (uint32_t)bcnt_acc(u4c(P.E[rr], J) & cur.v[0], 0) | ((uint32_t)bcnt_acc(u4c(P.V[rr], J) & cur.v[1], 0) << 16); \
          if (cur.v[3]) {      \
            _Pragma("unroll") for (int rr = 0; rr < R; rr++)                                                                      \
              pk_[rr] += __builtin_amdgcn_sad_u8(wE[rr] & cur.v[3], 0u, 0u) | (__builtin_amdgcn_sad_u8(wV[rr] & cur.v[3], 0u, 0u) << 16); \
          }                                                                                                                       \
          const uint32_t off_ = cur.v[2];                                                                                         \
          __builtin_amdgcn_sched_barrier(0);                                                                                      \
          TOUCH4(ahead);                                                                                                          \
          LDS_ADD(off_, pack_acc(pk_));                                                                                           \
        }
     \
     \
#define WORD_ITEMS(P, J)                                                                                                          \
        {                                                                                                                         \
          uint32_t k = (n_words >> (8 * J)) & 255u;                                                                               \
          _Pragma("unroll 1") for (; k >= 2; k -= 2) {                                                                            \
            load_qwords(nx, wp + 4);                                                                                              \
            WORD_ITEM(P, J, it, nx)                                                                                               \
            wp += 8;                                                                                                              \
            load_qwords(it, wp);                                                                                                  \
            WORD_ITEM(P, J, nx, it)                                                                                               \
          }                                                                                                                       \
          if (k) {                                                                                                                \
            wp += 4;                                                                                                              \
            load_qwords(nx, wp);                                                                                                  \
            WORD_ITEM(P, J, it, nx)                                                                                               \
            it = nx;                                                                                                              \
          }                                                                                                                       \
        }
    for (uint32_t rec = 0; rec < n_rec; rec += 2) {
      RECORD(PA, PB)
      if (rec + 1 < n_rec) RECORD(PB, PA)
    }
#undef RECORD
#undef ITEM_VALUE
#undef WORD_ITEMS
#undef WORD_ITEM
    {
      const char *tr[R];
#pragma unroll
      for (int rr = 0; rr < R; rr++) tr[rr] = reinterpret_cast<const char *>(poly + (size_t)(tile_first + trel[rr]) * NPT * 3 * 64 + lane);
      sp = (const cst_u32 *)(stream + dir[2 * NW + 2 * wave]);
      for (uint32_t rec = 0; rec < dir[2 * NW + 2 * wave + 1]; rec++) {
        QWords<2> hr;
        load_qwords(hr, sp);
        sp += 4;
        uint4 pL[R], pH[R], pI[R];
#pragma unroll
        for (int rr = 0; rr < R; rr++) {
          pL[rr] = *reinterpret_cast<const uint4 *>(tr[rr] + hr.v[0]); pH[rr] = *reinterpret_cast<const uint4 *>(tr[rr] + hr.v[0] + 1024);
          pI[rr] = *reinterpret_cast<const uint4 *>(tr[rr] + hr.v[0] + 2048);
        }
        const uint32_t n_words = hr.v[1];
        QWords<4> it, nx;
        load_qwords(it, sp);
        TOUCH4(it);
#define RARE_ITEM(J, cur, ahead)                                                                                                  \
        {                                                                                                                         \
          __builtin_amdgcn_sched_barrier(0);                                                                                      \
          uint32_t c_[R];                                                                                                         \
          _Pragma("unroll") for (int rr = 0; rr < R; rr++) {                                                                      \
            const uint32_t d_ = u4c(pL[rr], J) ^ cur.v[1];                                                                        \
            const uint32_t y_ = B3(u4c(pH[rr], J), cur.v[2], d_, (TT_A ^ TT_B) | TT_C);                                           \
            const uint32_t g_ = ACGT ? B3(y_, u4c(pI[rr], J), cur.v[0], TT_A & TT_B & TT_C) : B3(y_, u4c(pI[rr], J), cur.v[0], ~TT_A & TT_B & TT_C); \
            c_[rr] = (uint32_t)bcnt_acc(g_, 0);                                                                                   \
          }                                                                                                                       \
          const uint32_t off_ = cur.v[3];                                                                                         \
          __builtin_amdgcn_sched_barrier(0);                                                                                      \
          TOUCH4(ahead);                                                                                                          \
          LDS_SUB(off_, pack_acc(c_));                             \
        }
#define RARE_ITEMS(J)                                                                                                             \
        {                                                                                                                         \
          uint32_t k = (n_words >> (8 * J)) & 255u;                                                                               \
          _Pragma("unroll 1") for (; k >= 2; k -= 2) {                                                                            \
            load_qwords(nx, sp + 4);                                                                                              \
            RARE_ITEM(J, it, nx)                                                                                                  \
            sp += 8;                                                                                                              \
            load_qwords(it, sp);                                                                                                  \
            RARE_ITEM(J, nx, it)                                                                                                  \
          }                                                                                                                       \
          if (k) {                                                                                                                \
            sp += 4;                                                                                                              \
            load_qwords(nx, sp);                                                                                                  \
            RARE_ITEM(J, it, nx)                                                                                                  \
            it = nx;                                                                                                              \
          }                                                                                                                       \
        }
        RARE_ITEMS(0) RARE_ITEMS(1) RARE_ITEMS(2) RARE_ITEMS(3)
#undef RARE_ITEMS
#undef RARE_ITEM
      }
    }
#undef LDS_ADD
#undef LDS_SUB
#undef TOUCH_ITEM
#undef TOUCH4
  }
  __syncthreads();
  int te[R], tv[R]; bool in_batch[R]; size_t r[R];
#pragma unroll
  for (int rr = 0; rr < R; rr++) {
    r[rr] = (size_t)trel[rr] * 64 + lane;
    te[rr] = tot_e[r[rr]]; tv[rr] = tot_v[r[rr]];
    in_batch[rr] = ((int)r[rr] >= r_lo && (int)r[rr] < r_hi);
  }
#pragma unroll
  for (int q = 0; q < QT; q++) {
    acc_t pkk;
    lds_counter_load(my + (size_t)q * 64 * sizeof(acc_t), pkk);
#pragma unroll
    for (int rr = 0; rr < R; rr++) {
      if (!live[rr]) continue;
      const uint32_t pk = acc_part(pkk, rr);
      const int c0 = (ACGT ? te[rr] : te[rr] + NP4 * 128) - ((int)(pk & 0xFFFFu) - (int)RARE_BIAS), c1 = tv[rr] - (int)(pk >> 16);
      out[(size_t)(q0 + q) * ppad + r[rr]] = (uint32_t)c0 | ((uint32_t)c1 << 16);
      const int mm = ACGT ? c0 : c1 - c0, kk = ACGT ? c1 - c0 : c0;
      const uint32_t mx_m = wave_max_dpp(in_batch[rr] ? 65536u - (uint32_t)mm : 0u), mx_k = wave_max_dpp(in_batch[rr] ? (uint32_t)kk + 1u : 0u);
      const int m = mx_m ? (int)(65536u - mx_m) : 0x7fffffff, k = mx_k ? (int)(mx_k - 1u) : (int)0x80000000;
      if (lane == 0) {
        int2 *tp = tmin + (size_t)(q0 + q) * (ppad >> 6) + trel[rr];
        *tp = make_int2(m, k);
      }
    }
    __builtin_amdgcn_sched_barrier(0);
  }
}
```

uvaia_amd/csrc/uvaia_gpu.hip:

```cpp
#include <hip/hip_runtime.h>

#include <algorithm>
#include <atomic>
#include <cstdarg>
#include <cstdint>
#include <cstdio>
#include <cstdlib>
#include <condition_variable>
#include <cstring>
#include <functional>
#include <mutex>
#include <string>
#include <thread>
#include <vector>

#include "../../include/uvaia_gpu.h"
#include "iupac_decode.h"

#define TT_A 0xF0u
#define TT_B 0xCCu
#define TT_C 0xAAu
#define B3(a, b, c, tt) __builtin_amdgcn_bitop3_b32((a), (b), (c), (tt) & 0xFFu)

static __device__ __forceinline__ uint32_t u4c(const uint4 &v, int j)
{
  return j == 0 ? v.x : j == 1 ? v.y : j == 2 ? v.z : v.w;
}

typedef uint32_t u32x4_ld __attribute__((ext_vector_type(4)));
static __device__ __forceinline__ uint4 ld_stream(const uint4 *p)
{
  const u32x4_ld v = __builtin_nontemporal_load(reinterpret_cast<const u32x4_ld *>(p));
  return make_uint4(v.x, v.y, v.z, v.w);
}

static __device__ __forceinline__ int bcnt_acc(uint32_t x, int acc)
{
  int r;
  asm("v_bcnt_u32_b32 %0, %1, %2" : "=v"(r) : "v"(x), "v"(acc));
  return r;
}

namespace {

constexpr int HEAP_ENTRY = 8;
constexpr int AMB_CAP = 11;
constexpr int AMB_STRIDE = AMB_CAP + 1;
constexpr int AMB_ROW = 64;
constexpr int PACK_CHUNK = 4096;
constexpr uint32_t SCAN3_BIAS = 16384u;
constexpr int NBUF = 4;

}

#include "kernels_pack.inc"
#include "kernels_rows.inc"
#include "kernels_consensus.inc"
#include "kernels_scan2.inc"
#include "kernels_scan3.inc"
#include "kernels_replay.inc"
#include "kernels_ball.inc"
#include "kernels_qprep.inc"
#include "kernels_expand.inc"

#include "host_ctx.inc"
#include "host_launch.inc"
#include "host_qtables.inc"
#include "host_qprep.inc"
#include "host_open.inc"
#include "host_batch.inc"
#include "host_resident.inc"
#include "host_rows.inc"
#include "host_shards.inc"
#include "host_ball.inc"
#include "host_window.inc"
```

Before: 34.97 million.

## Precompute per-word popcounts in derive and skip padded polymorphic words in scan

The derive kernel now stores per-word byte-packed popcounts of the e and v planes (uint2 per group) instead of one summed group count. The scan kernel reads these to avoid recomputing popcounts in the word-item path and rebuilds group sums with sad_u8. The polymorphic pass also processes only the real number of words in the last group of four, and reads query words through the constant address space. In exchange, derived storage per reference grows by 4 bytes per word group, and the old grp export is reconstructed on the host.

```diff
diff --git a/include/uvaia_gpu.h b/include/uvaia_gpu.h
--- a/include/uvaia_gpu.h
+++ b/include/uvaia_gpu.h
@@ -153,6 +153,7 @@
 int    uvaia_gpu_db_clear (uvaia_gpu_ctx *ctx);
 int    uvaia_gpu_db_rederive (uvaia_gpu_ctx *ctx);
 int    uvaia_gpu_db_derived_export (uvaia_gpu_ctx *ctx, size_t n_tiles, void *e, uint32_t *grp, void *poly, int *tot);
+int    uvaia_gpu_db_word_counts_export (uvaia_gpu_ctx *ctx, size_t n_tiles, uint32_t *wcnt);
 int    uvaia_gpu_db_side_row_ints (void);
 int    uvaia_gpu_db_export (uvaia_gpu_ctx *ctx, size_t first_tile, size_t n_tiles, void *planes, int *non_n, int *side_rows);
 int    uvaia_gpu_db_append_packed (uvaia_gpu_ctx *ctx, const void *planes, const int *non_n, const int *side_rows, int n_ref);
diff --git a/uvaia_amd/capi.py b/uvaia_amd/capi.py
--- a/uvaia_amd/capi.py
+++ b/uvaia_amd/capi.py
@@ -17,7 +17,7 @@
     "uvaia_gpu_state_bytes", "uvaia_gpu_state_export", "uvaia_gpu_state_import", "uvaia_gpu_slice_scan", "uvaia_gpu_slice_replay",
     "uvaia_gpu_entered_flags", "uvaia_gpu_state_range_bytes", "uvaia_gpu_state_export_range", "uvaia_gpu_state_import_range",
     "uvaia_gpu_slice_replay_range", "uvaia_gpu_slice_buffers", "uvaia_gpu_scan_bytes_per_ref", "uvaia_gpu_derived_bytes_per_ref", "uvaia_gpu_scan_variant", "uvaia_gpu_set_query_tile", "uvaia_gpu_packed_bytes_per_ref",
-    "uvaia_gpu_db_tile_bytes", "uvaia_gpu_db_side_row_ints", "uvaia_gpu_db_export", "uvaia_gpu_db_append_packed", "uvaia_gpu_db_clear", "uvaia_gpu_db_rederive", "uvaia_gpu_db_derived_export",
+    "uvaia_gpu_db_tile_bytes", "uvaia_gpu_db_side_row_ints", "uvaia_gpu_db_export", "uvaia_gpu_db_append_packed", "uvaia_gpu_db_clear", "uvaia_gpu_db_rederive", "uvaia_gpu_db_derived_export", "uvaia_gpu_db_word_counts_export",
     "uvaia_gpu_set_active_queries", "uvaia_gpu_max_tolerance", "uvaia_gpu_search_resident_pool",
     "uvaia_gpu_db_set_shard", "uvaia_gpu_shard_rows", "uvaia_gpu_shard_scan", "uvaia_gpu_scan_wait", "uvaia_gpu_replay_wait", "uvaia_gpu_set_snapshot", "uvaia_gpu_shard_replay",
     "uvaia_gpu_mark", "uvaia_gpu_stream_wait_mark", "uvaia_gpu_wait_stream",
@@ -143,6 +143,7 @@
         "uvaia_gpu_db_clear": (C.c_int, [vp]),
         "uvaia_gpu_db_rederive": (C.c_int, [vp]),
         "uvaia_gpu_db_derived_export": (C.c_int, [vp, C.c_size_t, C.c_void_p, C.c_void_p, C.c_void_p, C.c_void_p]),
+        "uvaia_gpu_db_word_counts_export": (C.c_int, [vp, C.c_size_t, C.c_void_p]),
         "uvaia_gpu_db_side_row_ints": (C.c_int, []),
         "uvaia_gpu_db_export": (C.c_int, [vp, C.c_size_t, C.c_size_t, C.c_void_p, pi, pi]),
         "uvaia_gpu_db_append_packed": (C.c_int, [vp, C.c_void_p, pi, pi, C.c_int]),
@@ -648,6 +649,12 @@
         self._chk(self.L.uvaia_gpu_db_derived_export(self.ctx, int(n_tiles), e.ctypes.data, grp.ctypes.data, poly.ctypes.data, tot.ctypes.data))
         return e, grp, poly, tot
 
+    def db_word_counts(self, n_tiles):
+        W4 = ((self.nchar + 31) // 32 + 3) // 4
+        wcnt = np.zeros((n_tiles, W4, 64, 2), dtype=np.uint32)
+        self._chk(self.L.uvaia_gpu_db_word_counts_export(self.ctx, int(n_tiles), wcnt.ctypes.data))
+        return wcnt
+
     def ball_kernel_ms(self, reset=False):
         out = (C.c_double * 3)()
         self.L.uvaia_gpu_ball_kernel_ms(self.ctx, out, int(reset))
diff --git a/uvaia_amd/csrc/host_ctx.inc b/uvaia_amd/csrc/host_ctx.inc
--- a/uvaia_amd/csrc/host_ctx.inc
+++ b/uvaia_amd/csrc/host_ctx.inc
@@ -70,7 +70,7 @@
   DevBuf<int> amb;
   DevBuf<int> tot;
   DevBuf<uint4> ev, poly;
-  DevBuf<uint32_t> grp;
+  DevBuf<uint2> wcnt;
   DevBuf<int> tote;
 };
 
diff --git a/uvaia_amd/csrc/host_launch.inc b/uvaia_amd/csrc/host_launch.inc
--- a/uvaia_amd/csrc/host_launch.inc
+++ b/uvaia_amd/csrc/host_launch.inc
@@ -95,7 +95,7 @@
   if (int rc = s.nonn.reserve(c, refs)) return rc;
   HIPCHK(c, hipMemset(s.nonn, 0, refs * sizeof(int)));
   if (int rc = s.ev.reserve(c, tiles * (size_t)c->W4 * 2 * 64)) return rc;
-  if (int rc = s.grp.reserve(c, tiles * (size_t)c->W4 * 64)) return rc;
+  if (int rc = s.wcnt.reserve(c, tiles * (size_t)c->W4 * 64)) return rc;
   if (int rc = s.poly.reserve(c, tiles * (size_t)std::max(c->tab.NP4 + c->tab.NR4, 1) * 3 * 64)) return rc;
   if (int rc = s.tote.reserve(c, refs)) return rc;
   if (int rc = s.tot.reserve(c, refs)) return rc;
@@ -233,7 +233,7 @@
     const int st_first = c->act_q0 / QS, n_st = (c->act_q1 + QS - 1) / QS - st_first;
     const int R = c->scan_R;
     dim3 grid3(scan_grid_size(n_st, (n_tiles + R - 1) / R));
-#define SCAN3_LAUNCH(NWW, A, RR) hipLaunchKernelGGL((scan3_kernel<NWW, A, RR>), grid3, dim3(64 * NWW), 0, stream, s.ev, s.poly, tile_first, n_tiles, c->W4, c->tab.NP4, c->tab.NP4 + c->tab.NR4, c->tab.d_qpl, c->tab.d_stream, c->tab.d_sdir, s.grp, tote, tot_tile0, out, ppad, n_st, tmin, r_lo, r_hi, st_first)
+#define SCAN3_LAUNCH(NWW, A, RR) hipLaunchKernelGGL((scan3_kernel<NWW, A, RR>), grid3, dim3(64 * NWW), 0, stream, s.ev, s.poly, tile_first, n_tiles, c->W4, c->tab.NP4, (c->tab.NP + 31) / 32, c->tab.NP4 + c->tab.NR4, c->tab.d_qpl, c->tab.d_stream, c->tab.d_sdir, s.wcnt, tote, tot_tile0, out, ppad, n_st, tmin, r_lo, r_hi, st_first)
 #define SCAN3_NW(A, RR) { if (c->scan_NW == 8) SCAN3_LAUNCH(8, A, RR); else SCAN3_LAUNCH(4, A, RR); }
     if (R == 4)      { if (c->acgt) SCAN3_LAUNCH(8, true, 4); else SCAN3_LAUNCH(8, false, 4); }
     else if (R == 2) { if (c->acgt) SCAN3_NW(true, 2) else SCAN3_NW(false, 2) }
@@ -357,7 +357,7 @@
   const long long a = slot0 / 64, t1 = (slot0 + n_ref - 1) / 64;
   const int nblk = (int)(t1 - a + 1);
   const int waves = c->derive_waves ? c->derive_waves : 4;
-#define DERIVE_ALL_W(A, V, N) hipLaunchKernelGGL((derive_all_kernel<A, V, N>), dim3(nblk), dim3(64 * N), 0, st, s.planes, a, a, c->W4, c->tab.d_cls, c->tab.d_rmask, c->tab.d_split + derive_split_offset(N), c->tab.NP4, c->tab.NR4, s.ev, s.tote, s.grp, s.poly)
+#define DERIVE_ALL_W(A, V, N) hipLaunchKernelGGL((derive_all_kernel<A, V, N>), dim3(nblk), dim3(64 * N), 0, st, s.planes, a, a, c->W4, c->tab.d_cls, c->tab.d_rmask, c->tab.d_split + derive_split_offset(N), c->tab.NP4, c->tab.NR4, s.ev, s.tote, s.wcnt, s.poly)
 #define DERIVE_ALL(A, V) { if (waves == 8) DERIVE_ALL_W(A, V, 8); else if (waves == 16) DERIVE_ALL_W(A, V, 16); else DERIVE_ALL_W(A, V, 4); }
   if (c->acgt) { if (v_in_place) DERIVE_ALL(true, false) else DERIVE_ALL(true, true) }
   else         { if (v_in_place) DERIVE_ALL(false, false) else DERIVE_ALL(false, true) }
diff --git a/uvaia_amd/csrc/host_open.inc b/uvaia_amd/csrc/host_open.inc
--- a/uvaia_amd/csrc/host_open.inc
+++ b/uvaia_amd/csrc/host_open.inc
@@ -227,7 +227,7 @@
 size_t uvaia_gpu_derived_bytes_per_ref(const uvaia_gpu_ctx *c)
 {
   if (!c || c->fullscan || c->scan_variant != 2) return 0;
-  return (size_t)c->W4 * 16 + (size_t)c->W4 * 4 + (size_t)(c->tab.NP4 + c->tab.NR4) * 48 + 4;
+  return (size_t)c->W4 * 16 + (size_t)c->W4 * 8 + (size_t)(c->tab.NP4 + c->tab.NR4) * 48 + 4;
 }
 
 int uvaia_gpu_set_query_tile(uvaia_gpu_ctx *c, int qt)
diff --git a/uvaia_amd/csrc/host_resident.inc b/uvaia_amd/csrc/host_resident.inc
--- a/uvaia_amd/csrc/host_resident.inc
+++ b/uvaia_amd/csrc/host_resident.inc
@@ -98,18 +98,38 @@
   return 0;
 }
 
-int uvaia_gpu_db_derived_export(uvaia_gpu_ctx *c, size_t n_tiles, void *e, uint32_t *grp, void *poly, int *tot)
-{
-  if (!c || !e || !grp || !poly || !tot) return UVAIA_GPU_EINVAL;
+static int derived_export_ready(uvaia_gpu_ctx *c, size_t n_tiles)
+{
   if (c->fullscan || c->scan_variant != 2 || !c->db.ev) return fail(c, UVAIA_GPU_ESTATE, "only the column-compressed scan keeps planes derived for the query set");
   if (c->shard.world > 1) return fail(c, UVAIA_GPU_ESTATE, "a context of a reference shard numbers its derived tiles by piece: read them from a plain context");
   if (n_tiles * 64 > ((c->db_n + 63) / 64) * 64) return fail(c, UVAIA_GPU_EINVAL, "tiles 0..%zu lie outside the database", n_tiles);
   if (!n_tiles) return 0;
   { int rc = settle_derive(c); if (rc) return rc; }
   HIPCHK(c, hipStreamSynchronize(c->st.stream));
+  return 0;
+}
+
+int uvaia_gpu_db_word_counts_export(uvaia_gpu_ctx *c, size_t n_tiles, uint32_t *wcnt)
+{
+  if (!c || !wcnt) return UVAIA_GPU_EINVAL;
+  if (int rc = derived_export_ready(c, n_tiles)) return rc;
+  if (n_tiles) HIPCHK(c, hipMemcpy(wcnt, c->db.wcnt, n_tiles * (size_t)c->W4 * 64 * sizeof(uint2), hipMemcpyDeviceToHost));
+  return 0;
+}
+
+int uvaia_gpu_db_derived_export(uvaia_gpu_ctx *c, size_t n_tiles, void *e, uint32_t *grp, void *poly, int *tot)
+{
+  if (!c || !e || !grp || !poly || !tot) return UVAIA_GPU_EINVAL;
+  if (int rc = derived_export_ready(c, n_tiles)) return rc;
+  if (!n_tiles) return 0;
   const size_t W4 = (size_t)c->W4, NG = (size_t)(c->tab.NP4 + c->tab.NR4);
   HIPCHK(c, hipMemcpy2D(e, 1024, c->db.ev, 2048, 1024, n_tiles * W4, hipMemcpyDeviceToHost));
-  HIPCHK(c, hipMemcpy(grp, c->db.grp, n_tiles * W4 * 64 * sizeof(uint32_t), hipMemcpyDeviceToHost));
+  {
+    std::vector<uint2> w(n_tiles * W4 * 64);
+    HIPCHK(c, hipMemcpy(w.data(), c->db.wcnt, w.size() * sizeof(uint2), hipMemcpyDeviceToHost));
+    auto bytes = [](uint32_t x) { return (x & 255u) + ((x >> 8) & 255u) + ((x >> 16) & 255u) + (x >> 24); };
+    for (size_t i = 0; i < w.size(); i++) grp[i] = bytes(w[i].x) | (bytes(w[i].y) << 16);
+  }
   if (NG) HIPCHK(c, hipMemcpy(poly, c->db.poly, n_tiles * NG * 3 * 64 * sizeof(uint4), hipMemcpyDeviceToHost));
   HIPCHK(c, hipMemcpy(tot, c->db.tote, n_tiles * 64 * sizeof(int), hipMemcpyDeviceToHost));
   return 0;
diff --git a/uvaia_amd/csrc/kernels_scan3.inc b/uvaia_amd/csrc/kernels_scan3.inc
--- a/uvaia_amd/csrc/kernels_scan3.inc
+++ b/uvaia_amd/csrc/kernels_scan3.inc
@@ -6,6 +6,7 @@
   const u32x4_nt x = {v.x, v.y, v.z, v.w};
   __builtin_nontemporal_store(x, reinterpret_cast<u32x4_nt *>(p));
 }
+typedef uint32_t u32x2_nt __attribute__((ext_vector_type(2)));
 struct GatherStage { uint32_t bL, bH, bI; int fill, ow; };
 
 template <int NWV>
@@ -24,7 +25,7 @@
 void derive_all_kernel(const uint4 *__restrict__ tiles, long long tile_base, long long dtile_base, int W4,
                        const uint32_t *__restrict__ cls, const uint32_t *__restrict__ rmask,
                        const int *__restrict__ split, int NP4, int NR4,
-                       uint4 *__restrict__ ev, int *__restrict__ tot_e, uint32_t *__restrict__ grp, uint4 *__restrict__ poly)
+                       uint4 *__restrict__ ev, int *__restrict__ tot_e, uint2 *__restrict__ wcnt, uint4 *__restrict__ poly)
 {
   constexpr int P = ACGT ? 3 : 4;
   __shared__ int partial[NWV][64];
@@ -79,7 +80,7 @@
       for (int p = 0; p < P; p++) nxt[p] = ld_stream(t + (size_t)((w4 + 1) * P + p) * 64);
     }
     uint32_t e[4], v[4];
-    int ge = 0, gv = 0;
+    uint32_t ce = 0u, cv = 0u;
 #pragma unroll
     for (int j = 0; j < 4; j++) {
       uint32_t rL, rH, rI, rV;
@@ -93,7 +94,8 @@
       const uint32_t diff = (rL ^ c4[0]) | (rH ^ c4[1]);
       e[j] = rI & c4[2] & (ACGT ? diff : ~diff);
       v[j] = rV;
-      ge += __popc(e[j]); gv += __popc(v[j]);
+      const uint32_t pe = (uint32_t)__popc(e[j]);
+      te += (int)pe; ce |= pe << (8 * j); cv |= (uint32_t)__popc(v[j]) << (8 * j);
       for (uint32_t m = c4[3]; m; m &= m - 1) {
         const int b = __ffs(m) - 1;
         D.bL = take_bit(rL, b, D.fill, D.bL); D.bH = take_bit(rH, b, D.fill, D.bH); D.bI = take_bit(rI, b, D.fill, D.bI);
@@ -105,8 +107,7 @@
         if (++R.fill == 32) push_word(R, 1);
       }
     }
-    te += ge;
-    __builtin_nontemporal_store((uint32_t)ge | ((uint32_t)gv << 16), grp + ((size_t)tile * W4 + w4) * 64 + lane);
+    { const u32x2_nt x = {ce, cv}; __builtin_nontemporal_store(x, reinterpret_cast<u32x2_nt *>(wcnt + ((size_t)tile * W4 + w4) * 64 + lane)); }
     st_stream(o + (size_t)(w4 * 2 + 0) * 64, make_uint4(e[0], e[1], e[2], e[3]));
     if (WRITE_V) st_stream(o + (size_t)(w4 * 2 + 1) * 64, make_uint4(v[0], v[1], v[2], v[3]));
   }
@@ -170,8 +171,8 @@
 
 template <int NW , bool ACGT, int R, int QS = 64 >
 __global__ __launch_bounds__(64 * NW) __attribute__((amdgpu_waves_per_eu(4, 8))) void scan3_kernel(const uint4 *__restrict__ ev, const uint4 *__restrict__ poly, long long tile_first, int n_tiles,
-                                                     int W4, int NP4, int NPT, const uint32_t *__restrict__ qpl, const uint32_t *__restrict__ stream,
-                                                     const uint32_t *__restrict__ sdir, const uint32_t *__restrict__ grp,
+                                                     int W4, int NP4, int NPW, int NPT, const uint32_t *__restrict__ qpl, const uint32_t *__restrict__ stream,
+                                                     const uint32_t *__restrict__ sdir, const uint2 *__restrict__ wcnt,
                                                      const int *__restrict__ tot_e, const int *__restrict__ tot_v,
                                                      uint32_t *__restrict__ out, int ppad, int n_stiles, int2 *__restrict__ tmin, int r_lo, int r_hi,
                                                      int stile_first)
@@ -208,29 +209,47 @@
 #pragma unroll
       for (int rr = 0; rr < R; rr++) t[rr] = poly + (size_t)(tile_first + trel[rr]) * NPT * 3 * 64 + lane;
       const size_t qstride = (size_t)NP4 * 16;
-      const uint32_t *qb = qpl + (size_t)q0 * qstride;
+      typedef __attribute__((address_space(4))) const uint32_t cst_qw;
+      const cst_qw *qb = (const cst_qw *)(qpl + (size_t)q0 * qstride);
+      const int nw_last = NPW - 4 * (NP4 - 1);
       for (int p4 = 0; p4 < NP4; p4++) {
         uint4 pL[R], pH[R], pI[R];
 #pragma unroll
         for (int rr = 0; rr < R; rr++) { pL[rr] = t[rr][(size_t)(p4 * 3 + 0) * 64]; pH[rr] = t[rr][(size_t)(p4 * 3 + 1) * 64]; pI[rr] = t[rr][(size_t)(p4 * 3 + 2) * 64]; }
-        const uint32_t *s0 = qb + (size_t)p4 * 16;
-        QWords<12> cur, nxt;
-        load_qwords(cur, s0);
-#pragma unroll
-        for (int q = 0; q < QT; q++) {
-          if (q + 1 < QT) load_qwords(nxt, s0 + (size_t)(q + 1) * qstride);
-          __builtin_amdgcn_sched_barrier(0);
-#pragma unroll
-          for (int rr = 0; rr < R; rr++)
-#pragma unroll
-            for (int j = 0; j < 4; j++) {
-              const uint32_t d = u4c(pL[rr], j) ^ cur.v[j];
-              const uint32_t y = B3(u4c(pH[rr], j), cur.v[4 + j], d, (TT_A ^ TT_B) | TT_C);
-              acc[rr][q] = bcnt_acc(ACGT ? B3(y, u4c(pI[rr], j), cur.v[8 + j], TT_A & TT_B & TT_C) : B3(y, u4c(pI[rr], j), cur.v[8 + j], ~(~TT_A & TT_B & TT_C)), acc[rr][q]);
-            }
-          __builtin_amdgcn_sched_barrier(0);
-          if (q + 1 < QT) cur = nxt;
-        }
+#if defined(__HIP_DEVICE_COMPILE__)
+#pragma unroll
+        for (int rr = 0; rr < R; rr++) {
+          asm volatile("" : "+v"(pL[rr].x), "+v"(pL[rr].y), "+v"(pL[rr].z), "+v"(pL[rr].w));
+          asm volatile("" : "+v"(pH[rr].x), "+v"(pH[rr].y), "+v"(pH[rr].z), "+v"(pH[rr].w));
+          asm volatile("" : "+v"(pI[rr].x), "+v"(pI[rr].y), "+v"(pI[rr].z), "+v"(pI[rr].w));
+        }
+#endif
+        const cst_qw *s0 = qb + (size_t)p4 * 16;
+        auto group = [&](auto nj) {
+          constexpr int NJ = decltype(nj)::value;
+          QWords<12> cur, nxt;
+          load_qwords(cur, s0);
+#pragma unroll
+          for (int q = 0; q < QT; q++) {
+            if (q + 1 < QT) load_qwords(nxt, s0 + (size_t)(q + 1) * qstride);
+            __builtin_amdgcn_sched_barrier(0);
+#pragma unroll
+            for (int rr = 0; rr < R; rr++)
+#pragma unroll
+              for (int j = 0; j < NJ; j++) {
+                const uint32_t d = u4c(pL[rr], j) ^ cur.v[j];
+                const uint32_t y = B3(u4c(pH[rr], j), cur.v[4 + j], d, (TT_A ^ TT_B) | TT_C);
+                acc[rr][q] = bcnt_acc(ACGT ? B3(y, u4c(pI[rr], j), cur.v[8 + j], TT_A & TT_B & TT_C) : B3(y, u4c(pI[rr], j), cur.v[8 + j], ~(~TT_A & TT_B & TT_C)), acc[rr][q]);
+              }
+            __builtin_amdgcn_sched_barrier(0);
+            if (q + 1 < QT) cur = nxt;
+          }
+        };
+        const int nw = p4 + 1 < NP4 ? 4 : nw_last;
+        if (nw == 4) group(std::integral_constant<int, 4>());
+        else if (nw == 3) group(std::integral_constant<int, 3>());
+        else if (nw == 2) group(std::integral_constant<int, 2>());
+        else group(std::integral_constant<int, 1>());
       }
     }
 #pragma unroll
@@ -246,9 +265,9 @@
   }
   __syncthreads();
   {
-    const uint4 *t[R]; const uint32_t *gt[R];
-#pragma unroll
-    for (int rr = 0; rr < R; rr++) { t[rr] = ev + (size_t)(tile_first + trel[rr]) * W4 * 2 * 64 + lane; gt[rr] = grp + (size_t)(tile_first + trel[rr]) * W4 * 64 + lane; }
+    const uint4 *t[R]; const uint2 *ct[R];
+#pragma unroll
+    for (int rr = 0; rr < R; rr++) { t[rr] = ev + (size_t)(tile_first + trel[rr]) * W4 * 2 * 64 + lane; ct[rr] = wcnt + (size_t)(tile_first + trel[rr]) * W4 * 64 + lane; }
     typedef __attribute__((address_space(4))) const uint32_t cst_u32;
     const cst_u32 *dir = (const cst_u32 *)(sdir + (size_t)stile * 4 * NW);
     const cst_u32 *sp = (const cst_u32 *)(stream + dir[2 * wave]);
@@ -257,7 +276,7 @@
 #define LDS_SUB(byte_off, val) lds_counter_sub(myc + (byte_off), (val))
 #define TOUCH_ITEM(it) asm volatile("" ::"s"(it.v[0]), "s"(it.v[1]), "s"(it.v[2]), "s"(it.v[3]), "s"(it.v[4]), "s"(it.v[5]), "s"(it.v[6]), "s"(it.v[7]), "s"(it.v[8]))
 #define TOUCH4(it) asm volatile("" ::"s"(it.v[0]), "s"(it.v[1]), "s"(it.v[2]), "s"(it.v[3]))
-    struct Planes { uint4 E[R], V[R]; uint32_t g[R]; };
+    struct Planes { uint4 E[R], V[R]; uint2 c[R]; };
     Planes PA, PB;
     auto request = [&](Planes &P, uint32_t h0) {
 #pragma unroll
@@ -265,7 +284,7 @@
         const char *tg = reinterpret_cast<const char *>(t[rr]) + (h0 & ~1023u);
         P.E[rr] = *reinterpret_cast<const uint4 *>(tg);
         P.V[rr] = *reinterpret_cast<const uint4 *>(tg + 1024);
-        P.g[rr] = *reinterpret_cast<const uint32_t *>(reinterpret_cast<const char *>(gt[rr]) + ((h0 & ~1023u) >> 3));
+        P.c[rr] = *reinterpret_cast<const uint2 *>(reinterpret_cast<const char *>(ct[rr]) + ((h0 & ~1023u) >> 2));
       }
     };
     QWords<4> h, hn, hnn;
@@ -288,7 +307,9 @@
       load_qwords(a, ip);                                                                                                         \
       load_qwords(it, wp);                                                                                                        \
       if (n_full4) {     \
-        const acc_t gg = pack_acc(P.g);                                                                                           \
+        uint32_t g_[R];                                                                                                           \
+        _Pragma("unroll") for (int rr = 0; rr < R; rr++) g_[rr] = __builtin_amdgcn_sad_u8(P.c[rr].x, 0u, 0u) | (__builtin_amdgcn_sad_u8(P.c[rr].y, 0u, 0u) << 16); \
+        const acc_t gg = pack_acc(g_);                                                                                            \
         _Pragma("unroll 1") for (uint32_t k = 0; k < n_full4; k++, sp += 4) {       \
           QWords<4> o;                                                                                                            \
           load_qwords(o, sp);                                                                                                     \
@@ -323,13 +344,7 @@
       if (n_words) {     \
                                                    \
         uint32_t wE[R], wV[R];       \
-        _Pragma("unroll") for (int rr = 0; rr < R; rr++) { wE[rr] = 0u; wV[rr] = 0u; }                                            \
-        if (h.v[0] & 1u) {                                                                                                        \
-          _Pragma("unroll") for (int rr = 0; rr < R; rr++) {                                                                      \
-            wE[rr] = (uint32_t)bcnt_acc(P.E[rr].x, 0) | (uint32_t)bcnt_acc(P.E[rr].y, 0) << 8 | (uint32_t)bcnt_acc(P.E[rr].z, 0) << 16 | (uint32_t)bcnt_acc(P.E[rr].w, 0) << 24; \
-            wV[rr] = (uint32_t)bcnt_acc(P.V[rr].x, 0) | (uint32_t)bcnt_acc(P.V[rr].y, 0) << 8 | (uint32_t)bcnt_acc(P.V[rr].z, 0) << 16 | (uint32_t)bcnt_acc(P.V[rr].w, 0) << 24; \
-          }                                                                                                                       \
-        }                                                                                                                         \
+        _Pragma("unroll") for (int rr = 0; rr < R; rr++) { wE[rr] = P.c[rr].x; wV[rr] = P.c[rr].y; }                              \
         TOUCH4(it);                                                                                                               \
         WORD_ITEMS(P, 0) WORD_ITEMS(P, 1) WORD_ITEMS(P, 2) WORD_ITEMS(P, 3)                                                       \
       }                                                                                                                           \
@@ -466,7 +481,7 @@
     for (int rr = 0; rr < R; rr++) {
       if (!live[rr]) continue;
       const uint32_t pk = acc_part(pkk, rr);
-      const int c0 = (ACGT ? te[rr] : te[rr] + NP4 * 128) - ((int)(pk & 0xFFFFu) - (int)RARE_BIAS), c1 = tv[rr] - (int)(pk >> 16);
+      const int c0 = (ACGT ? te[rr] : te[rr] + NPW * 32) - ((int)(pk & 0xFFFFu) - (int)RARE_BIAS), c1 = tv[rr] - (int)(pk >> 16);
       out[(size_t)(q0 + q) * ppad + r[rr]] = (uint32_t)c0 | ((uint32_t)c1 << 16);
       const int mm = ACGT ? c0 : c1 - c0, kk = ACGT ? c1 - c0 : c0;
       const uint32_t mx_m = wave_max_dpp(in_batch[rr] ? 65536u - (uint32_t)mm : 0u), mx_k = wave_max_dpp(in_batch[rr] ? (uint32_t)kk + 1u : 0u);
diff --git a/uvaia_amd/csrc/uvaia_gpu.hip b/uvaia_amd/csrc/uvaia_gpu.hip
--- a/uvaia_amd/csrc/uvaia_gpu.hip
+++ b/uvaia_amd/csrc/uvaia_gpu.hip
@@ -12,6 +12,7 @@
 #include <mutex>
 #include <string>
 #include <thread>
+#include <type_traits>
 #include <vector>
 
 #include "../../include/uvaia_gpu.h"
```

After: 34.57 million. 0.989x the previous value.
